# yanqinJiang/Animate3D

Hardware: AMD Instinct MI355X
Metric: UNet denoise-steps/sec, 4view×16frame×512² MV-VDM @1/2/4/8 GPU (higher is better)
Workload: dtype bf16; 1 GPU; BASELINE config 2: 4 views x 16 frames x 512^2 px (64x64 latent), CFG-doubled batch V=8 videos, one MVUNetMotionModel.forward per step, SD1.5 MV-VDM UNet 1.53 B params, seeded synthetic weights; parallelism=single GPU

## Files before the change

### animate3d_amd/csrc/gemm_common.h

```cpp
#pragma once
#include "common.h"

struct GemmParams {
  const uint16_t* X; int64_t ldx;
  const uint16_t* W; int64_t ldw;
  const float* bias;
  const uint16_t* rowbias; int64_t rb_div;
  const uint16_t* R; int64_t ldr;
  uint16_t* Y; int64_t ldy;
  int64_t M, N, K;
  float alpha, beta;
  int vec16;
  int out_f32;
  int B, H, Wd, Cin, Ho, Wo, stride, up, He, We;
  int64_t tiles_n, tiles_m;
  int ksplit, nk_item;
  float* ws; int64_t ws_bytes;
  const uint16_t* X2; int64_t ldx2; int64_t K1;
};

constexpr int EPI_LINEAR = 0, EPI_GEGLU = 1;

static inline int a3d_gemm_kernel_of(int flags) { return flags & A3D_GEMM_KERNEL_MASK; }
static inline int a3d_gemm_reserved_cus_of(int flags) { return flags & A3D_GEMM_RESERVED_CUS_MASK; }

A3D_DEV float epi_scale(float v, float alpha) { return __fmul_rn(v, alpha); }
A3D_DEV float epi_axpy(float v, float beta, float r) { return __fmaf_rn(beta, r, v); }

A3D_DEV float gelu_erf(float gte) {
  const float x = fabsf(gte) * 0.70710678118654752f;
  const float t = __builtin_amdgcn_rcpf(fmaf(0.3275911f, x, 1.0f));
  float poly = fmaf(1.061405429f, t, -1.453152027f);
  poly = fmaf(poly, t, 1.421413741f);
  poly = fmaf(poly, t, -0.284496736f);
  poly = fmaf(poly, t, 0.254829592f);
  poly *= t;
  const float e = __builtin_amdgcn_exp2f(-x * x * 1.4426950408889634f);
  const float erfx = fmaf(-poly, e, 1.0f);
  const float hg = __fmul_rn(0.5f, gte);
  return __fmaf_rn(fabsf(hg), erfx, hg);
}

A3D_DEV f32x2_t splat2(float v) { return f32x2_t{v, v}; }
A3D_DEV f32x2_t gelu_erf2(f32x2_t g) {
  const f32x2_t x = __builtin_elementwise_abs(g) * 0.70710678118654752f;
  const f32x2_t den = __builtin_elementwise_fma(splat2(0.3275911f), x, splat2(1.0f));
  const f32x2_t t = {__builtin_amdgcn_rcpf(den[0]), __builtin_amdgcn_rcpf(den[1])};
  f32x2_t poly = __builtin_elementwise_fma(splat2(1.061405429f), t, splat2(-1.453152027f));
  poly = __builtin_elementwise_fma(poly, t, splat2(1.421413741f));
  poly = __builtin_elementwise_fma(poly, t, splat2(-0.284496736f));
  poly = __builtin_elementwise_fma(poly, t, splat2(0.254829592f));
  poly = poly * t;
  const f32x2_t a = (-x) * x * 1.4426950408889634f;
  const f32x2_t e = {__builtin_amdgcn_exp2f(a[0]), __builtin_amdgcn_exp2f(a[1])};
  const f32x2_t erfx = __builtin_elementwise_fma(-poly, e, splat2(1.0f));
  const f32x2_t hg = g * 0.5f;
  return __builtin_elementwise_fma(__builtin_elementwise_abs(hg), erfx, hg);
}
A3D_DEV void geglu8(const float (&hv)[8], const float (&gv)[8], const float (&bh)[8], const float (&bg)[8], float (&y)[8]) {
#pragma unroll
  for (int e = 0; e < 4; ++e) {
    const f32x2_t gg = f32x2_t{gv[2 * e], gv[2 * e + 1]} + f32x2_t{bg[2 * e], bg[2 * e + 1]};
    const f32x2_t hh = f32x2_t{hv[2 * e], hv[2 * e + 1]} + f32x2_t{bh[2 * e], bh[2 * e + 1]};
    const f32x2_t yy = hh * gelu_erf2(gg);
    y[2 * e] = yy[0]; y[2 * e + 1] = yy[1];
  }
}

static __device__ u32x4_t g_zero_page[4];

A3D_DEV uint32_t lds_addr(const void* p) {
  return (uint32_t)(uintptr_t)(__attribute__((address_space(3))) const void*)p;
}
A3D_DEV void glds16_v(const void* gsrc, uint32_t lds_dst) {
  unsigned keep;
  asm volatile("s_mov_b32 %0, m0\n\ts_mov_b32 m0, %2\n\ts_nop 0\n\tglobal_load_lds_dwordx4 %1, off\n\ts_mov_b32 m0, %0"
               : "=&s"(keep) : "v"(gsrc), "s"(__builtin_amdgcn_readfirstlane(lds_dst)) : "memory");
}
A3D_DEV void glds16_s(uint32_t voff, const void* sbase, uint32_t lds_dst) {
  unsigned keep;
  asm volatile("s_mov_b32 %0, m0\n\ts_mov_b32 m0, %3\n\ts_nop 0\n\tglobal_load_lds_dwordx4 %1, %2\n\ts_mov_b32 m0, %0"
               : "=&s"(keep) : "v"(voff), "s"(sbase), "s"(__builtin_amdgcn_readfirstlane(lds_dst)) : "memory");
}
A3D_DEV const uint16_t* scalar_ptr(const uint16_t* ptr) {
  const uint64_t a = (uint64_t)(uintptr_t)ptr;
  return (const uint16_t*)(uintptr_t)(((uint64_t)(uint32_t)__builtin_amdgcn_readfirstlane((int)(a >> 32)) << 32) |
                                      (uint32_t)__builtin_amdgcn_readfirstlane((int)(uint32_t)a));
}
A3D_DEV u32x4_t lds_vload128(const void* p) {
  return *(const volatile __attribute__((address_space(3))) u32x4_t*)(uintptr_t)lds_addr(p);
}
A3D_DEV u32x2_t lds_vload64(const void* p) {
  return *(const volatile __attribute__((address_space(3))) u32x2_t*)(uintptr_t)lds_addr(p);
}
A3D_DEV void wave_lds_fence() {
  __builtin_amdgcn_fence(__ATOMIC_RELEASE, "wavefront");
  __builtin_amdgcn_wave_barrier();
  __builtin_amdgcn_fence(__ATOMIC_ACQUIRE, "wavefront");
}

A3D_DEV void tile_barrier() {
  asm volatile("s_barrier" ::: "memory");
  __builtin_amdgcn_sched_barrier(0);
}

template <int NB> struct WaveCols {
  static constexpr int PASSES = (NB + 1) / 2;
  int first, last;
  __device__ __forceinline__ explicit WaveCols(int wn) : first(NB == 5 ? wn * 4 : wn * NB), last(NB == 5 ? 8 + wn : wn * NB + NB - 1) {}
  __device__ __forceinline__ int block(int tn) const { return tn < NB - 1 ? first + tn : last; }
  A3D_DEV int pass_width(int ps) { return 2 * ps + 1 < NB ? 64 : 32; }
  __device__ __forceinline__ int pass_col0(int ps) const { return block(2 * ps) * 32; }
};

constexpr int BIAS_IMG_STRIDE = 2048;
constexpr int BIAS_IMG_ROWBIAS = 1280;
constexpr int BIAS_IMG_DMA = 1024;
A3D_DEV const float* bias_image(const char* img, int par) { return reinterpret_cast<const float*>(img + par * BIAS_IMG_STRIDE); }
A3D_DEV const uint16_t* rowbias_image(const char* img, int par) {
  return reinterpret_cast<const uint16_t*>(img + par * BIAS_IMG_STRIDE + BIAS_IMG_ROWBIAS);
}
template <int THREADS> A3D_DEV void zero_absent_bias_images(char* img, const float* bias, const uint16_t* rowbias, int tid) {
  if (!bias || !rowbias) {
    uint32_t* const bz = reinterpret_cast<uint32_t*>(img);
    for (int i = tid; i < 2 * BIAS_IMG_STRIDE / 4; i += THREADS) {
      const int o = (i * 4) % BIAS_IMG_STRIDE;
      if ((o < BIAS_IMG_ROWBIAS && !bias) || (o >= BIAS_IMG_ROWBIAS && !rowbias)) bz[i] = 0u;
    }
    asm volatile("s_waitcnt lgkmcnt(0)" ::: "memory");
    tile_barrier();
  }
}

template <int NB> A3D_DEV void read_frags(const char* stage, uint32_t xrd, uint32_t wrd, uint32_t wrd_last, uint32_t ko, u32x4_t (&fx)[2],
                                          u32x4_t (&fw)[NB]) {
  const char* xs = stage + xrd;
  const char* ws = stage + wrd;
  const char* wl = stage + wrd_last;
#pragma unroll
  for (int tm = 0; tm < 2; ++tm) fx[tm] = *reinterpret_cast<const u32x4_t*>(xs + tm * 4096 + ko);
#pragma unroll
  for (int tn = 0; tn < NB - 1; ++tn) fw[tn] = *reinterpret_cast<const u32x4_t*>(ws + tn * 4096 + ko);
  fw[NB - 1] = *reinterpret_cast<const u32x4_t*>(wl + ko);
}

template <int EPI, int NB>
A3D_DEV void epilogue_rounded(const GemmParams& p, f32x16_t (&acc)[NB][2], float* const stg, const float* const bias_lds,
                              const uint16_t* const rowbias_lds, const int64_t m0, const int64_t n0, const int wm, const WaveCols<NB> wc,
                              const int lane) {
  const int wblk = wc.first, wblk_last = wc.last;
  auto pass_cols = [&](int ps) { return (2 * ps + 1 < NB) ? 64 : 32; };
  auto pass_col0 = [&](int ps) { return ((2 * ps + 1 < NB) ? wblk + 2 * ps : wblk_last) * 32; };
  const int l31 = lane & 31, g = lane >> 5;
  constexpr int NP = (NB + 1) / 2;
  constexpr int RS = (EPI == EPI_GEGLU) ? 64 : 128;
  char* const stg16 = reinterpret_cast<char*>(stg);
  const int wsw = (EPI == EPI_GEGLU) ? ((l31 >> 1) & 3) : (l31 & 7);
  const int whalf = 8 * (g ^ ((l31 >> 3) & 1));
  auto unswap = [](u32x4_t o, int row) {
    const bool sw = row & 8;
    u32x4_t r;
    r[0] = sw ? o[2] : o[0]; r[1] = sw ? o[3] : o[1]; r[2] = sw ? o[0] : o[2]; r[3] = sw ? o[1] : o[3];
    return r;
  };
  constexpr int BUF2 = 32 * RS;
#pragma unroll
  for (int pi = 0; pi < 2 * NP; ++pi) {
    const int tm = pi / NP, ps = pi % NP;
    const int ncol = pass_cols(ps);
    const int64_t mbase = m0 + wm * 64 + tm * 32;
    const int64_t nbase = n0 + pass_col0(ps);
    char* const sb = stg16 + (pi & 1) * BUF2;
    if constexpr (EPI == EPI_GEGLU) {
      u32x4_t bq[2][4];
      auto fetch = [&](int q2, int slot) __attribute__((always_inline)) {
#pragma unroll
        for (int h = 0; h < 2; ++h) {
          const int c0 = 8 * (2 * q2 + h) + 4 * g;
          bq[slot][2 * h] = lds_vload128(bias_lds + pass_col0(ps) + c0);
          bq[slot][2 * h + 1] = lds_vload128(bias_lds + pass_col0(ps) + 32 + c0);
        }
      };
      fetch(0, 0);
#pragma unroll
      for (int q2 = 0; q2 < 2; ++q2) {
        if (q2 + 1 < 2) fetch(q2 + 1, (q2 + 1) & 1);
        __builtin_amdgcn_sched_barrier(0);
        float hv[8], gv[8], bh[8], bg[8], y[8];
#pragma unroll
        for (int h = 0; h < 2; ++h) {
          const u32x4_t b0 = bq[q2 & 1][2 * h], b1 = bq[q2 & 1][2 * h + 1];
#pragma unroll
          for (int j = 0; j < 4; ++j) { bh[4 * h + j] = __uint_as_float(b0[j]); bg[4 * h + j] = __uint_as_float(b1[j]); }
#pragma unroll
          for (int j = 0; j < 4; ++j) { hv[4 * h + j] = acc[2 * ps][tm][4 * (2 * q2 + h) + j]; gv[4 * h + j] = acc[2 * ps + 1][tm][4 * (2 * q2 + h) + j]; }
        }
        geglu8(hv, gv, bh, bg, y);
#pragma unroll
        for (int h = 0; h < 2; ++h) {
          u32x2_t o;
          o[0] = pack16(y[4 * h], y[4 * h + 1]);
          o[1] = pack16(y[4 * h + 2], y[4 * h + 3]);
          *reinterpret_cast<u32x2_t*>(sb + l31 * RS + 16 * ((2 * q2 + h) ^ wsw) + whalf) = o;
        }
      }
      wave_lds_fence();
      const int cc = lane & 3;
      const int64_t oc = nbase / 2 + 8 * cc;
      u32x4_t ob[2];
#pragma unroll
      for (int j = 0; j < 2; ++j) {
        const int row = 16 * j + (lane >> 2);
        ob[j] = *reinterpret_cast<const u32x4_t*>(sb + row * RS + 16 * (cc ^ ((row >> 1) & 3)));
      }
#pragma unroll
      for (int j = 0; j < 2; ++j) {
        const int row = 16 * j + (lane >> 2);
        const int64_t m = mbase + row;
        const u32x4_t o = unswap(ob[j], row);
        *reinterpret_cast<u32x4_t*>(p.Y + m * p.ldy + oc) = o;
      }
    } else {
      constexpr int NQ = 8;
      const int nq = (2 * ps + 1 < NB) ? 8 : 4;
      u32x4_t bq[3];
      u32x2_t tq[3];
      auto fetch = [&](int idx, int slot) __attribute__((always_inline)) {
        const int c0 = (idx >> 2) * 32 + 8 * (idx & 3) + 4 * g;
        bq[slot] = lds_vload128(bias_lds + pass_col0(ps) + c0);
        tq[slot] = lds_vload64(rowbias_lds + pass_col0(ps) + c0);
      };
      auto quads = [&](auto with_c) __attribute__((always_inline)) {
        constexpr bool WITH = decltype(with_c)::value;
        if constexpr (WITH) { fetch(0, 0); fetch(1, 1); }
#pragma unroll
        for (int idx = 0; idx < NQ; ++idx) {
          if (idx >= nq) continue;
          const int tl = idx >> 2, q = idx & 3;
          const int tn = 2 * ps + tl;
          if constexpr (WITH) {
            if (idx + 2 < nq) fetch(idx + 2, (idx + 2) % 3);
            __builtin_amdgcn_sched_barrier(0);
          }
          float v[4] = {acc[tn][tm][4 * q], acc[tn][tm][4 * q + 1], acc[tn][tm][4 * q + 2], acc[tn][tm][4 * q + 3]};
          if constexpr (WITH) {
            const u32x4_t b = bq[idx % 3];
            v[0] += __uint_as_float(b[0]); v[1] += __uint_as_float(b[1]); v[2] += __uint_as_float(b[2]); v[3] += __uint_as_float(b[3]);
            const u32x2_t tb = tq[idx % 3];
            v[0] += lo16(tb[0]); v[1] += hi16(tb[0]); v[2] += lo16(tb[1]); v[3] += hi16(tb[1]);
          }
#pragma unroll
          for (int e = 0; e < 4; ++e) v[e] = epi_scale(v[e], p.alpha);
          u32x2_t o;
          o[0] = pack16(v[0], v[1]);
          o[1] = pack16(v[2], v[3]);
          *reinterpret_cast<u32x2_t*>(sb + l31 * RS + 16 * ((4 * tl + q) ^ wsw) + whalf) = o;
          if constexpr (WITH) __builtin_amdgcn_sched_barrier(0);
        }
      };
      if (p.bias || p.rowbias) quads(std::true_type{});
      else quads(std::false_type{});
      wave_lds_fence();
      const int lpr = ncol / 8;
      const int cc = lane & (lpr - 1);
      u32x4_t ob[4];
#pragma unroll
      for (int j = 0; j < 4; ++j) {
        if (j * (64 / lpr) >= 32) continue;
        const int row = (64 / lpr) * j + lane / lpr;
        ob[j] = *reinterpret_cast<const u32x4_t*>(sb + row * RS + 16 * (cc ^ (row & 7)));
      }
#pragma unroll
      for (int j = 0; j < 4; ++j) {
        if (j * (64 / lpr) >= 32) continue;
        const int row = (64 / lpr) * j + lane / lpr;
        const int64_t m = mbase + row;
        const u32x4_t o = unswap(ob[j], row);
        *reinterpret_cast<u32x4_t*>(p.Y + m * p.ldy + nbase + 8 * cc) = o;
      }
    }
  }
}

template <int NB>
A3D_DEV void epilogue_residual(const GemmParams& p, f32x16_t (&acc)[NB][2], float* const stg, const float* const bias_lds,
                               const uint16_t* const rowbias_lds, const int64_t m0, const int64_t n0, const int wm, const WaveCols<NB> wc,
                               const int lane) {
  const int l31 = lane & 31, g = lane >> 5;
  constexpr int SROW = 68;
  constexpr int NP = WaveCols<NB>::PASSES;
  u32x4_t rres[2][4];
  auto load_res = [&](int pi, int slot) {
    const int tm = pi / NP, ps = pi % NP;
    const int64_t mbase = m0 + wm * 64 + tm * 32;
    const int64_t nbase = n0 + wc.pass_col0(ps);
    if (WaveCols<NB>::pass_width(ps) == 64) {
#pragma unroll
      for (int j = 0; j < 4; ++j) {
        const int64_t m = mbase + 8 * j + (lane >> 3);
        rres[slot][j] = *reinterpret_cast<const u32x4_t*>(p.R + m * p.ldr + nbase + 8 * (lane & 7));
      }
    } else {
#pragma unroll
      for (int j = 0; j < 2; ++j) {
        const int64_t m = mbase + 16 * j + (lane >> 2);
        rres[slot][j] = *reinterpret_cast<const u32x4_t*>(p.R + m * p.ldr + nbase + 8 * (lane & 3));
      }
    }
  };
  load_res(0, 0);
#pragma unroll
  for (int pi = 0; pi < 2 * NP; ++pi) {
    const int tm = pi / NP, ps = pi % NP;
    const int ncol = WaveCols<NB>::pass_width(ps);
    if (pi + 1 < 2 * NP) load_res(pi + 1, (pi + 1) & 1);
#pragma unroll
    for (int tl = 0; tl < 2; ++tl) {
      const int tn = 2 * ps + tl;
      if (tn < NB) {
#pragma unroll
        for (int q = 0; q < 4; ++q) {
          float4 v;
          v.x = acc[tn][tm][4 * q]; v.y = acc[tn][tm][4 * q + 1]; v.z = acc[tn][tm][4 * q + 2]; v.w = acc[tn][tm][4 * q + 3];
          *reinterpret_cast<float4*>(stg + l31 * SROW + tl * 32 + 8 * q + 4 * g) = v;
        }
      }
    }
    wave_lds_fence();
    const int64_t mbase = m0 + wm * 64 + tm * 32;
    const int64_t nbase = n0 + wc.pass_col0(ps);

    const int lpr = ncol / 8;
    const int cc = lane & (lpr - 1);
    const int64_t n = nbase + 8 * cc;
    const int ncl = wc.pass_col0(ps) + 8 * cc;
    float bv[8];
#pragma unroll
    for (int e = 0; e < 8; ++e) bv[e] = bias_lds[ncl + e];
    const u32x4_t tb = *reinterpret_cast<const u32x4_t*>(rowbias_lds + ncl);
#pragma unroll
    for (int j = 0; j < 4; ++j) {
      if (j * (64 / lpr) >= 32) continue;
      const int row = (64 / lpr) * j + lane / lpr;
      const int64_t m = mbase + row;
      const float4 a0 = *reinterpret_cast<const float4*>(stg + row * SROW + 8 * cc);
      const float4 a1 = *reinterpret_cast<const float4*>(stg + row * SROW + 8 * cc + 4);
      float v[8] = {a0.x, a0.y, a0.z, a0.w, a1.x, a1.y, a1.z, a1.w};
#pragma unroll
      for (int e = 0; e < 8; ++e) v[e] += bv[e];
#pragma unroll
      for (int e = 0; e < 4; ++e) { v[2 * e] += lo16(tb[e]); v[2 * e + 1] += hi16(tb[e]); }
#pragma unroll
      for (int e = 0; e < 8; ++e) v[e] = epi_scale(v[e], p.alpha);
      const u32x4_t tr = rres[pi & 1][j];
#pragma unroll
      for (int e = 0; e < 4; ++e) { v[2 * e] = epi_axpy(v[2 * e], p.beta, lo16(tr[e])); v[2 * e + 1] = epi_axpy(v[2 * e + 1], p.beta, hi16(tr[e])); }
      u32x4_t o;
#pragma unroll
      for (int e = 0; e < 4; ++e) o[e] = pack16(v[2 * e], v[2 * e + 1]);
      *reinterpret_cast<u32x4_t*>(p.Y + m * p.ldy + n) = o;
    }
    wave_lds_fence();
  }
}


__attribute__((visibility("hidden"))) int A3D_FN(a3d_launch_gemm_pp)(int conv, int epi, int nb, hipStream_t stream, const GemmParams& p, int cus);
__attribute__((visibility("hidden"))) int A3D_FN(a3d_launch_gemm_ring)(int nb, hipStream_t stream, const GemmParams& p, int cus);
```

### animate3d_amd/csrc/gemm_conv.hip

```cpp
#include "gemm_common.h"

namespace {

constexpr int BM = 128, BN = 128;
template <int BKT> struct TileCfg {
  static constexpr int LROW = BKT + 8;
  static constexpr int TILE_ELEMS = 128 * LROW;
  static constexpr int STAGE_BYTES = 2 * 2 * TILE_ELEMS * 2;
  static constexpr int EPI_BYTES = 4 * 32 * 68 * 4;
  static constexpr int SMEM_BYTES = STAGE_BYTES > EPI_BYTES ? STAGE_BYTES : EPI_BYTES;
  static constexpr int CPR = BKT / 8;
  static constexpr int RPT = 256 / CPR;
  static constexpr int NPASS = 128 / RPT;
};



template <int CONV, int EPI, int BKT, bool RES>
__global__ __launch_bounds__(256, (BKT == 64 ? 2 : 3)) void gemm_kernel(const GemmParams p) {
  using TC = TileCfg<BKT>;
  constexpr int LROW = TC::LROW, TILE_ELEMS = TC::TILE_ELEMS, NPASS = TC::NPASS, RPT = TC::RPT, BK = BKT;
  extern __shared__ __attribute__((aligned(16))) uint16_t smem[];
  const int tid = threadIdx.x;
  const int lane = tid & 63, wid = tid >> 6;
  const int wm = wid >> 1, wn = wid & 1;
  const int l31 = lane & 31, g = lane >> 5;

  const int64_t nblk = p.tiles_n * p.tiles_m;
  const int64_t lid = xcd_remap(blockIdx.x, nblk);
  const int64_t tile_n = lid % p.tiles_n, tile_m = lid / p.tiles_n;
  const int64_t m0 = tile_m * BM, n0 = tile_n * BN;

  const int kc = tid % TC::CPR;
  const int srow = tid / TC::CPR;

  const uint16_t* a_ptr[NPASS];
  int a_b[CONV == 2 ? NPASS : 1], a_y[CONV == 2 ? NPASS : 1], a_x[CONV == 2 ? NPASS : 1];
  bool a_ok[NPASS];
  int a_mask[NPASS];
#pragma unroll
  for (int i = 0; i < NPASS; ++i) {
    int64_t m = m0 + srow + RPT * i;
    a_ok[i] = m < p.M;
    if (m >= p.M) m = p.M - 1;
    if constexpr (CONV != 0) {
      const int hw = p.Ho * p.Wo;
      const int b = (int)(m / hw);
      const int rem = (int)(m - (int64_t)b * hw);
      const int oy = rem / p.Wo, ox = rem - oy * p.Wo;
      if constexpr (CONV == 2) {
        a_b[i] = b; a_y[i] = oy; a_x[i] = ox;
        a_ptr[i] = nullptr; a_mask[i] = 0;
      } else {
        const int y0 = oy * p.stride - 1, x0 = ox * p.stride - 1;
        a_ptr[i] = p.X + (((int64_t)b * p.H + y0) * p.Wd + x0) * p.Cin + kc * 8;
        int mask = 0;
#pragma unroll
        for (int t = 0; t < 9; ++t) {
          const int yy = y0 + t / 3, xx = x0 + t % 3;
          if (a_ok[i] && yy >= 0 && yy < p.H && xx >= 0 && xx < p.Wd) mask |= 1 << t;
        }
        a_mask[i] = mask;
      }
    } else {
      a_ptr[i] = p.X + m * p.ldx + kc * 8;
      a_mask[i] = 0;
    }
  }
  const uint16_t* w_ptr[NPASS];
#pragma unroll
  for (int i = 0; i < NPASS; ++i) {
    int64_t n = n0 + srow + RPT * i;
    if (n >= p.N) n = p.N - 1;
    w_ptr[i] = p.W + n * p.ldw + kc * 8;
  }

  struct RegTile { u32x4_t a[NPASS], w[NPASS]; };
  RegTile rt0, rt1;
  auto load_tile = [&](int64_t k0, RegTile& rt) {
    u32x4_t (&ra)[NPASS] = rt.a; u32x4_t (&rw)[NPASS] = rt.w;
    if constexpr (CONV != 0) {
      {
        const int kt64 = (int)(k0 >> 6);
        const int c64 = kt64 / 9, t = kt64 - 9 * c64;
        k0 = (int64_t)t * p.Cin + c64 * 64 + (k0 & 63);
      }
      const int tap = (int)(k0 / p.Cin);
      const int ci0 = (int)(k0 - (int64_t)tap * p.Cin);
      const int ky = tap / 3, kx = tap - ky * 3;
      if constexpr (CONV == 1) {
        const int64_t toff = ((int64_t)ky * p.Wd + kx) * p.Cin + ci0;
#pragma unroll
        for (int i = 0; i < NPASS; ++i) {
          if ((a_mask[i] >> tap) & 1) ra[i] = *reinterpret_cast<const u32x4_t*>(a_ptr[i] + toff);
          else ra[i] = u32x4_t{0u, 0u, 0u, 0u};
        }
      } else {
        const int He = p.He, We = p.We;
#pragma unroll
        for (int i = 0; i < NPASS; ++i) {
          const int yy = a_y[i] + ky - 1, xx = a_x[i] + kx - 1;
          const bool ok = a_ok[i] && yy >= 0 && yy < He && xx >= 0 && xx < We;
          if (ok) {
            const uint16_t* src = p.X + (((int64_t)a_b[i] * p.H + (yy >> 1)) * p.Wd + (xx >> 1)) * p.Cin + ci0 + kc * 8;
            ra[i] = *reinterpret_cast<const u32x4_t*>(src);
          } else {
            ra[i] = u32x4_t{0u, 0u, 0u, 0u};
          }
        }
      }
    } else {
#pragma unroll
      for (int i = 0; i < NPASS; ++i) ra[i] = *reinterpret_cast<const u32x4_t*>(a_ptr[i] + k0);
    }
#pragma unroll
    for (int i = 0; i < NPASS; ++i) rw[i] = *reinterpret_cast<const u32x4_t*>(w_ptr[i] + k0);
  };
  auto store_tile = [&](int buf, const RegTile& rt) {
    const u32x4_t (&ra)[NPASS] = rt.a; const u32x4_t (&rw)[NPASS] = rt.w;
    uint16_t* As = smem + (buf * 2 + 0) * TILE_ELEMS;
    uint16_t* Ws = smem + (buf * 2 + 1) * TILE_ELEMS;
#pragma unroll
    for (int i = 0; i < NPASS; ++i) {
      *reinterpret_cast<u32x4_t*>(As + (srow + RPT * i) * LROW + kc * 8) = ra[i];
      *reinterpret_cast<u32x4_t*>(Ws + (srow + RPT * i) * LROW + kc * 8) = rw[i];
    }
  };

  f32x16_t acc[2][2];
#pragma unroll
  for (int a = 0; a < 2; ++a)
#pragma unroll
    for (int b = 0; b < 2; ++b)
#pragma unroll
      for (int r = 0; r < 16; ++r) acc[a][b][r] = 0.f;

  u32x4_t rres[RES ? 4 : 1];
  const int ecc = lane & 7;
  const int64_t en = n0 + wn * 64 + 8 * ecc;
  const bool epf = RES && (EPI == EPI_LINEAR) && p.R != nullptr && p.vec16 && en + 8 <= p.N;
  auto prefetch_residual = [&](int tm) {
    if constexpr (RES) {
#pragma unroll
      for (int j = 0; j < 4; ++j) {
        int64_t m = m0 + wm * 64 + tm * 32 + 8 * j + (lane >> 3);
        if (m >= p.M) m = p.M - 1;
        rres[j] = *reinterpret_cast<const u32x4_t*>(p.R + m * p.ldr + en);
      }
    }
  };

  const int64_t nk = p.K / BK;
  auto compute = [&](int cur) {
    const uint16_t* As = smem + (cur * 2 + 0) * TILE_ELEMS;
    const uint16_t* Ws = smem + (cur * 2 + 1) * TILE_ELEMS;
    u32x4_t fw[2][2], fa[2][2];
    auto load_frags = [&](int slot, int ks) {
#pragma unroll
      for (int t = 0; t < 2; ++t) {
        fw[slot][t] = *reinterpret_cast<const u32x4_t*>(Ws + (wn * 64 + t * 32 + l31) * LROW + ks * 16 + g * 8);
        fa[slot][t] = *reinterpret_cast<const u32x4_t*>(As + (wm * 64 + t * 32 + l31) * LROW + ks * 16 + g * 8);
      }
    };
    load_frags(0, 0);
#pragma unroll
    for (int ks = 0; ks < BK / 16; ++ks) {
      if (ks + 1 < BK / 16) load_frags((ks + 1) & 1, ks + 1);
#pragma unroll
      for (int tn = 0; tn < 2; ++tn)
#pragma unroll
        for (int tm = 0; tm < 2; ++tm) acc[tn][tm] = mfma32(fw[ks & 1][tn], fa[ks & 1][tm], acc[tn][tm]);
    }
  };

  load_tile(0, rt0);
  store_tile(0, rt0);
  if (nk > 1) load_tile(1 * BK, rt0);
  if (nk > 2) load_tile(2 * BK, rt1);
  __syncthreads();
  for (int64_t kt = 0;;) {
    if (kt + 1 >= nk && epf) prefetch_residual(0);
    compute(0);
    if (kt + 1 < nk) store_tile(1, rt0);
    if (kt + 3 < nk) load_tile((kt + 3) * BK, rt0);
    __syncthreads();
    if (++kt >= nk) break;
    if (kt + 1 >= nk && epf) prefetch_residual(0);
    compute(1);
    if (kt + 1 < nk) store_tile(0, rt1);
    if (kt + 3 < nk) load_tile((kt + 3) * BK, rt1);
    __syncthreads();
    if (++kt >= nk) break;
  }

  constexpr int SROW = 68;
  float* const stg = reinterpret_cast<float*>(smem) + wid * (32 * SROW);
#pragma unroll
  for (int tm = 0; tm < 2; ++tm) {
  if (tm == 1) __syncthreads();
#pragma unroll
  for (int tn = 0; tn < 2; ++tn)
#pragma unroll
    for (int q = 0; q < 4; ++q) {
      float4 v;
      v.x = acc[tn][tm][4 * q]; v.y = acc[tn][tm][4 * q + 1]; v.z = acc[tn][tm][4 * q + 2]; v.w = acc[tn][tm][4 * q + 3];
      *reinterpret_cast<float4*>(stg + l31 * SROW + tn * 32 + 8 * q + 4 * g) = v;
    }
  __syncthreads();
  const int64_t mbase = m0 + wm * 64 + tm * 32;

  if constexpr (EPI == EPI_GEGLU) {
    const int cc = lane & 3;
    const int64_t nh = n0 + wn * 64 + 8 * cc;
    const int64_t oc = (n0 + wn * 64) / 2 + 8 * cc;
    if (nh + 32 < p.N + 0 && oc + 8 <= p.N / 2) {
      float bh[8], bg[8];
#pragma unroll
      for (int e = 0; e < 8; ++e) { bh[e] = p.bias ? p.bias[nh + e] : 0.f; bg[e] = p.bias ? p.bias[nh + 32 + e] : 0.f; }
#pragma unroll
      for (int j = 0; j < 2; ++j) {
        const int row = 16 * j + (lane >> 2);
        const int64_t m = mbase + row;
        if (m >= p.M) continue;
        const float4 h0 = *reinterpret_cast<const float4*>(stg + row * SROW + 8 * cc);
        const float4 h1 = *reinterpret_cast<const float4*>(stg + row * SROW + 8 * cc + 4);
        const float4 g0 = *reinterpret_cast<const float4*>(stg + row * SROW + 32 + 8 * cc);
        const float4 g1 = *reinterpret_cast<const float4*>(stg + row * SROW + 32 + 8 * cc + 4);
        const float hv[8] = {h0.x, h0.y, h0.z, h0.w, h1.x, h1.y, h1.z, h1.w};
        const float gv[8] = {g0.x, g0.y, g0.z, g0.w, g1.x, g1.y, g1.z, g1.w};
        float y[8];
        geglu8(hv, gv, bh, bg, y);
        u32x4_t o;
#pragma unroll
        for (int e = 0; e < 4; ++e) o[e] = pack16(y[2 * e], y[2 * e + 1]);
        *reinterpret_cast<u32x4_t*>(p.Y + m * p.ldy + oc) = o;
      }
    }
  } else {
    const int cc = lane & 7;
    const int64_t n = n0 + wn * 64 + 8 * cc;
    if (n < p.N) {
      const bool full = (n + 8 <= p.N) && p.vec16;
      float bv[8];
#pragma unroll
      for (int e = 0; e < 8; ++e) bv[e] = (p.bias && n + e < p.N) ? p.bias[n + e] : 0.f;
#pragma unroll
      for (int j = 0; j < 4; ++j) {
        const int row = 8 * j + (lane >> 3);
        const int64_t m = mbase + row;
        if (m >= p.M) continue;
        const float4 a0 = *reinterpret_cast<const float4*>(stg + row * SROW + 8 * cc);
        const float4 a1 = *reinterpret_cast<const float4*>(stg + row * SROW + 8 * cc + 4);
        float v[8] = {a0.x, a0.y, a0.z, a0.w, a1.x, a1.y, a1.z, a1.w};
#pragma unroll
        for (int e = 0; e < 8; ++e) v[e] += bv[e];
        const uint16_t* rb = p.rowbias ? p.rowbias + (m / p.rb_div) * p.N + n : nullptr;
        const uint16_t* rr = p.R ? p.R + m * p.ldr + n : nullptr;
        uint16_t* yy = p.Y + m * p.ldy + n;
        if (full) {
          if (rb) {
            const u32x4_t t = *reinterpret_cast<const u32x4_t*>(rb);
#pragma unroll
            for (int e = 0; e < 4; ++e) { v[2 * e] += lo16(t[e]); v[2 * e + 1] += hi16(t[e]); }
          }
#pragma unroll
          for (int e = 0; e < 8; ++e) v[e] = epi_scale(v[e], p.alpha);
          if constexpr (RES) {
            if (rr) {
              const u32x4_t t = rres[j];
#pragma unroll
              for (int e = 0; e < 4; ++e) { v[2 * e] = epi_axpy(v[2 * e], p.beta, lo16(t[e])); v[2 * e + 1] = epi_axpy(v[2 * e + 1], p.beta, hi16(t[e])); }
            }
          }
          if (p.out_f32) {
            float* yf = reinterpret_cast<float*>(p.Y) + m * p.ldy + n;
            *reinterpret_cast<float4*>(yf) = float4{v[0], v[1], v[2], v[3]};
            *reinterpret_cast<float4*>(yf + 4) = float4{v[4], v[5], v[6], v[7]};
          } else {
            u32x4_t o;
#pragma unroll
            for (int e = 0; e < 4; ++e) o[e] = pack16(v[2 * e], v[2 * e + 1]);
            *reinterpret_cast<u32x4_t*>(yy) = o;
          }
        } else {
#pragma unroll
          for (int hh = 0; hh < 2; ++hh) {
            if (n + 4 * hh + 4 > p.N) continue;
            float w[4] = {v[4 * hh], v[4 * hh + 1], v[4 * hh + 2], v[4 * hh + 3]};
            if (rb) {
              const u32x2_t t = *reinterpret_cast<const u32x2_t*>(rb + 4 * hh);
              w[0] += lo16(t[0]); w[1] += hi16(t[0]); w[2] += lo16(t[1]); w[3] += hi16(t[1]);
            }
#pragma unroll
            for (int e = 0; e < 4; ++e) w[e] = epi_scale(w[e], p.alpha);
            if (rr) {
              const u32x2_t t = *reinterpret_cast<const u32x2_t*>(rr + 4 * hh);
              w[0] = epi_axpy(w[0], p.beta, lo16(t[0])); w[1] = epi_axpy(w[1], p.beta, hi16(t[0]));
              w[2] = epi_axpy(w[2], p.beta, lo16(t[1])); w[3] = epi_axpy(w[3], p.beta, hi16(t[1]));
            }
            u32x2_t o;
            o[0] = pack16(w[0], w[1]);
            o[1] = pack16(w[2], w[3]);
            *reinterpret_cast<u32x2_t*>(yy + 4 * hh) = o;
          }
        }
      }
    }
  }
  if (tm == 0 && epf) prefetch_residual(1);
  }
}


constexpr int PBM = 256;
constexpr int NOT_ELIGIBLE = -1000;

inline bool gemm_flags_ok(int flags) {
  return !(flags & ~(A3D_GEMM_RESERVED_CUS_MASK | A3D_GEMM_KERNEL_MASK)) && a3d_gemm_kernel_of(flags) <= A3D_GEMM_RING;
}

inline int device_cus() {
  static int cus_of[64] = {0};
  const int dev = a3d_current_device();
  if (cus_of[dev] == 0) {
    int n = 0;
    if (hipDeviceGetAttribute(&n, hipDeviceAttributeMultiprocessorCount, dev) != hipSuccess) return 0;
    cus_of[dev] = n > 0 ? n : 256;
  }
  return cus_of[dev];
}

constexpr int PERSIST_MIN_FILL = 50;
struct PPPlan { int nb, S, cus; int64_t tiles_m, tiles_n; };
constexpr int SPLITK_MAX = 16;
constexpr int SPLITK_MINK = 9;
template <int CONV, int EPI>
bool plan_persist(const GemmParams& p, int flags, bool allow_split, PPPlan& out) {
  if (a3d_gemm_kernel_of(flags) == A3D_GEMM_TILE128 || p.out_f32) return false;
  const int cus_dev = device_cus();
  if (cus_dev == 0) return false;
  const int reserved = a3d_gemm_reserved_cus_of(flags);
  const int cus = cus_dev - reserved > 32 ? cus_dev - reserved : 32;
  if (!p.vec16 || p.K % 64 != 0 || p.M % PBM != 0 || (p.rowbias && p.rb_div % PBM != 0)) return false;
  if (p.ldw % 64 != 0 || (CONV == 0 && p.ldx % 64 != 0)) return false;
  if (CONV == 0 && (uint64_t)p.ldx * 16u >= (1ull << 31)) return false;
  if ((uint64_t)p.ldw * 16u >= (1ull << 31)) return false;
  if (CONV != 0 && ((uint64_t)p.B * p.H * p.Wd + 2u * p.Wd + 2u) * (uint64_t)p.Cin * 2u >= (1ull << 32)) return false;
  const int64_t tm = (p.M + PBM - 1) / PBM;
  const int nk = (int)(p.K / 64);
  const int unit = CONV ? 9 : 1;
  const int cus_plan = cus_dev;
  constexpr int OVH = 12;
  int64_t best = -1, best1 = -1;
  int bnb = 0, bS = 1, bnb1 = 0;
  for (int nb = 5; nb >= 4; --nb) {
    if (EPI == EPI_GEGLU && nb == 5) continue;
    if (p.N % (nb * 64) != 0) continue;
    const int64_t tiles = tm * (p.N / (nb * 64));
    for (int S = 1; S <= (allow_split && EPI == EPI_LINEAR ? SPLITK_MAX : 1); ++S) {
      if ((nk / unit) % S != 0 || (S > 1 && nk / S < SPLITK_MINK)) continue;
      const int64_t items = tiles * S;
      const int64_t rounds = (items + cus_plan - 1) / cus_plan;
      if (items * 100 < rounds * cus_plan * PERSIST_MIN_FILL) continue;
      if (S > 1 && p.ws != nullptr && items * nb * 65536 > p.ws_bytes) continue;
      const int64_t cost = rounds * (nk / S + OVH) * nb * (nb == 4 ? 108 : 100) + (S > 1 ? 100 * nb : 0);
      if (S == 1 && (best1 < 0 || cost < best1)) { best1 = cost; bnb1 = nb; }
      if (best < 0 || cost < best) { best = cost; bnb = nb; bS = S; }
    }
  }
  if (best < 0) return false;
  if (bS > 1 && best1 >= 0 && best * 100 > best1 * 85) { bnb = bnb1; bS = 1; }
  out.nb = bnb; out.S = bS; out.cus = cus;
  out.tiles_m = tm; out.tiles_n = p.N / (bnb * 64);
  return true;
}

struct RingPlan { int nb, cus, cus_plan; int64_t cost; };
constexpr int RING_VS_PP_PCT = 75;
inline bool plan_ring(const GemmParams& p, int flags, RingPlan& out) {
  if (a3d_gemm_kernel_of(flags) == A3D_GEMM_TILE128 || p.out_f32 || !p.vec16 || p.X2 != nullptr) return false;
  if (p.M % 128 != 0 || p.K % 64 != 0 || p.K < 256 || p.ldx % 64 != 0 || p.ldw % 64 != 0) return false;
  if ((uint64_t)p.ldx * 64u >= (1ull << 32) || (uint64_t)p.ldw * 256u >= (1ull << 32)) return false;
  if (p.rowbias && p.rb_div % 128 != 0) return false;
  const int n = device_cus() ? device_cus() : 256;
  const int reserved = a3d_gemm_reserved_cus_of(flags);
  out.cus_plan = n;
  out.cus = n - reserved > 32 ? n - reserved : 32;
  out.nb = 0; out.cost = 0;
  for (int nb : {5, 4, 2}) {
    if (p.N % (64 * nb) != 0) continue;
    const int64_t tiles = (p.M / 128) * (p.N / (64 * nb));
    const int64_t rounds = (tiles + out.cus - 1) / out.cus;
    const int64_t cost = rounds * (128 + 64 * nb);
    if (out.nb == 0 || cost < out.cost) { out.nb = nb; out.cost = cost; }
  }
  return out.nb != 0;
}

template <int CONV, int EPI>
int try_launch_persist(hipStream_t stream, GemmParams& p, int flags) {
  PPPlan pl;
  if (!plan_persist<CONV, EPI>(p, flags, p.ws != nullptr, pl)) return NOT_ELIGIBLE;
  p.tiles_m = pl.tiles_m; p.tiles_n = pl.tiles_n;
  p.ksplit = pl.S; p.nk_item = (int)(p.K / 64) / pl.S;
  return A3D_FN(a3d_launch_gemm_pp)(CONV, EPI, pl.nb, stream, p, pl.cus);
}


template <int CONV, int EPI, int BKT, bool RES>
int launch_res(hipStream_t stream, GemmParams& p, int64_t nblk) {
  using TC = TileCfg<BKT>;
  static uint64_t attr_done = 0;
  if (int rc = a3d_once_per_device(attr_done, [] {
        return (int)hipFuncSetAttribute(reinterpret_cast<const void*>(&gemm_kernel<CONV, EPI, BKT, RES>),
                                        hipFuncAttributeMaxDynamicSharedMemorySize, TC::SMEM_BYTES); })) return rc;
  gemm_kernel<CONV, EPI, BKT, RES><<<dim3((unsigned)nblk), dim3(256), TC::SMEM_BYTES, stream>>>(p);
  return a3d_launch_status();
}

template <int CONV, int EPI, int BKT>
int launch_bk(hipStream_t stream, GemmParams& p, int64_t nblk) {
  if constexpr (EPI == EPI_LINEAR) {
    if (p.R != nullptr) return launch_res<CONV, EPI, BKT, true>(stream, p, nblk);
  }
  return launch_res<CONV, EPI, BKT, false>(stream, p, nblk);
}

template <int CONV, int EPI = EPI_LINEAR>
int launch(hipStream_t stream, GemmParams& p, int flags) {
  if (!gemm_flags_ok(flags)) return A3D_EINVAL;
  if constexpr (CONV == 0 && EPI == EPI_LINEAR) {
    RingPlan rp;
    if (plan_ring(p, flags, rp)) {
      PPPlan pl;
      bool ring = true;
      if (a3d_gemm_kernel_of(flags) != A3D_GEMM_RING && plan_persist<CONV, EPI>(p, flags, p.ws != nullptr, pl)) {
        const int64_t tiles = pl.tiles_m * pl.tiles_n * pl.S;
        const int64_t pp_cost = ((tiles + rp.cus_plan - 1) / rp.cus_plan) * (256 + 64 * pl.nb) * RING_VS_PP_PCT;
        ring = pl.S == 1 && rp.cost * 100 < pp_cost;
      }
      if (ring) {
        p.tiles_m = p.M / 128; p.tiles_n = p.N / (64 * rp.nb);
        return A3D_FN(a3d_launch_gemm_ring)(rp.nb, stream, p, rp.cus);
      }
    }
  }
  {
    const int rc = try_launch_persist<CONV, EPI>(stream, p, flags);
    if (rc != NOT_ELIGIBLE) return rc;
  }
  p.tiles_m = (p.M + BM - 1) / BM;
  p.tiles_n = (p.N + BN - 1) / BN;
  const int64_t nblk = p.tiles_m * p.tiles_n;
  if (nblk <= 0 || nblk > 0x7fffffffLL) return A3D_EINVAL;
  const bool small = (CONV == 0 && p.K <= 640) || nblk < 768;
  if (small) return launch_bk<CONV, EPI, 32>(stream, p, nblk);
  return launch_bk<CONV, EPI, 64>(stream, p, nblk);
}

template <int CONV>
int64_t splitk_ws_bytes(const GemmParams& p, int flags) {
  PPPlan pl;
  GemmParams q = p;
  q.ws = nullptr; q.ws_bytes = 0;
  if (!gemm_flags_ok(flags)) return 0;
  if (!plan_persist<CONV, EPI_LINEAR>(q, flags, true, pl) || pl.S <= 1) return 0;
  return pl.tiles_m * pl.tiles_n * pl.S * pl.nb * 65536;
}

void attach_workspace(GemmParams& p, void* ws, int64_t ws_bytes) {
  if (ws && ws_bytes > 0 && a3d_aligned(16, ws)) { p.ws = (float*)ws; p.ws_bytes = ws_bytes; }
}

GemmParams dense_params(const void* X, int64_t ldx, const void* W, int64_t ldw, const float* bias, const void* rowbias, int64_t rb_div,
                        const void* R, int64_t ldr, void* Y, int64_t ldy, int64_t M, int64_t N, int64_t K, float alpha, float beta,
                        bool out_f32 = false) {
  GemmParams p{};
  p.X = (const uint16_t*)X; p.ldx = ldx; p.W = (const uint16_t*)W; p.ldw = ldw;
  p.bias = bias; p.rowbias = (const uint16_t*)rowbias; p.rb_div = rowbias ? rb_div : 1;
  p.R = (const uint16_t*)R; p.ldr = ldr; p.Y = (uint16_t*)Y; p.ldy = ldy;
  p.M = M; p.N = N; p.K = K; p.alpha = alpha; p.beta = beta; p.out_f32 = out_f32;
  p.vec16 = (ldy * (out_f32 ? 4 : 2) % 16 == 0) && a3d_aligned(16, Y) && (!R || (ldr % 8 == 0 && a3d_aligned(16, R))) &&
            (!rowbias || (N % 8 == 0 && a3d_aligned(16, rowbias)));
  return p;
}

bool dense_args_ok(const GemmParams& p, uintptr_t y_align, int n_div, int ldy_div) {
  if (!p.X || !p.W || !p.Y || p.M <= 0 || p.N <= 0 || p.K <= 0) return false;
  if (p.K % 64 != 0 || p.N % n_div != 0) return false;
  if (p.ldx % 8 != 0 || p.ldw % 8 != 0 || p.ldy % ldy_div != 0 || (p.R && p.ldr % 4 != 0)) return false;
  if (!a3d_aligned(16, p.X, p.W) || !a3d_aligned(16, p.bias) || !a3d_aligned(y_align, p.Y) || !a3d_aligned(8, p.R, p.rowbias)) return false;
  return !p.rowbias || p.rb_div > 0;
}

int gemm_entry(a3d_stream_t stream, const void* X, int64_t ldx, const void* W, int64_t ldw,
               const float* bias, const void* rowbias, int64_t rb_div, const void* R, int64_t ldr,
               void* Y, int64_t ldy, int64_t M, int64_t N, int64_t K, float alpha, float beta, int flags,
               void* ws, int64_t ws_bytes, int64_t* ws_needed) {
  GemmParams p = dense_params(X, ldx, W, ldw, bias, rowbias, rb_div, R, ldr, Y, ldy, M, N, K, alpha, beta);
  if (!dense_args_ok(p, 8, 4, 4)) return A3D_EINVAL;
  if (ws_needed) { *ws_needed = splitk_ws_bytes<0>(p, flags); return 0; }
  attach_workspace(p, ws, ws_bytes);
  return launch<0>((hipStream_t)stream, p, flags);
}

}

extern "C" int A3D_FN(a3d_gemm)(a3d_stream_t stream, const void* X, int64_t ldx, const void* W, int64_t ldw,
                             const float* bias, const void* rowbias, int64_t rb_div, const void* R, int64_t ldr,
                             void* Y, int64_t ldy, int64_t M, int64_t N, int64_t K, float alpha, float beta, int flags) {
  return gemm_entry(stream, X, ldx, W, ldw, bias, rowbias, rb_div, R, ldr, Y, ldy, M, N, K, alpha, beta, flags, nullptr, 0, nullptr);
}

extern "C" int A3D_FN(a3d_gemm_ws)(a3d_stream_t stream, const void* X, int64_t ldx, const void* W, int64_t ldw,
                                const float* bias, const void* rowbias, int64_t rb_div, const void* R, int64_t ldr,
                                void* Y, int64_t ldy, int64_t M, int64_t N, int64_t K, float alpha, float beta, int flags,
                                void* ws, int64_t ws_bytes, int64_t* ws_needed) {
  return gemm_entry(stream, X, ldx, W, ldw, bias, rowbias, rb_div, R, ldr, Y, ldy, M, N, K, alpha, beta, flags, ws, ws_bytes, ws_needed);
}

extern "C" int A3D_FN(a3d_gemm2)(a3d_stream_t stream, const void* X, int64_t ldx, const void* X2, int64_t ldx2, int64_t K1,
                              const void* W, int64_t ldw, const float* bias, void* Y, int64_t ldy, int64_t M, int64_t N, int64_t K, int flags) {
  GemmParams p = dense_params(X, ldx, W, ldw, bias, nullptr, 1, nullptr, 0, Y, ldy, M, N, K, 1.f, 0.f);
  p.X2 = (const uint16_t*)X2; p.ldx2 = ldx2; p.K1 = K1;
  if (!dense_args_ok(p, 16, 8, 8) || !X2 || K1 <= 0 || K1 >= K || K1 % 64 != 0 || ldx2 % 8 != 0 || !a3d_aligned(16, X2)) return A3D_EINVAL;
  if (!gemm_flags_ok(flags)) return A3D_EINVAL;
  if (ldx2 % 64 != 0 || (uint64_t)ldx2 * 16u >= (1ull << 31)) return A3D_EUNSUPPORTED;
  const int rc = try_launch_persist<0, EPI_LINEAR>((hipStream_t)stream, p, flags);
  return rc == NOT_ELIGIBLE ? A3D_EUNSUPPORTED : rc;
}

extern "C" int A3D_FN(a3d_gemm_f32out)(a3d_stream_t stream, const void* X, int64_t ldx, const void* W, int64_t ldw,
                                    const float* bias, float* Y, int64_t ldy, int64_t M, int64_t N, int64_t K, float alpha) {
  GemmParams p = dense_params(X, ldx, W, ldw, bias, nullptr, 1, nullptr, 0, Y, ldy, M, N, K, alpha, 0.f, true);
  if (!dense_args_ok(p, 16, 8, 4)) return A3D_EINVAL;
  return launch<0>((hipStream_t)stream, p, 0);
}

static int conv_entry(a3d_stream_t stream, const void* X, const void* Wp, const float* bias,
                      const void* rowbias, int64_t rb_div, const void* R, void* Y,
                      int B, int H, int W, int Cin, int Cout, int stride, int up2x, int flags,
                      void* ws, int64_t ws_bytes, int64_t* ws_needed) {
  if (!X || !Wp || !Y || B <= 0 || H <= 0 || W <= 0) return A3D_EINVAL;
  if (Cin % 64 != 0 || Cout % 4 != 0 || (stride != 1 && stride != 2)) return A3D_EINVAL;
  if (up2x < 0 || up2x > 7 || (up2x > 1 && !(up2x & 1)) || (up2x && stride != 1)) return A3D_EINVAL;
  if (!a3d_aligned(16, X, Wp) || !a3d_aligned(16, bias) || !a3d_aligned(8, Y)) return A3D_EINVAL;
  if (rowbias && rb_div <= 0) return A3D_EINVAL;
  const int He = up2x ? 2 * H - ((up2x >> 1) & 1) : H, We = up2x ? 2 * W - ((up2x >> 2) & 1) : W;
  if (He <= 0 || We <= 0) return A3D_EINVAL;
  GemmParams p{};
  p.X = (const uint16_t*)X; p.ldx = Cin; p.W = (const uint16_t*)Wp; p.ldw = (int64_t)9 * Cin;
  p.bias = bias; p.rowbias = (const uint16_t*)rowbias; p.rb_div = rowbias ? rb_div : 1;
  p.R = (const uint16_t*)R; p.ldr = Cout; p.Y = (uint16_t*)Y; p.ldy = Cout;
  p.B = B; p.H = H; p.Wd = W; p.Cin = Cin; p.stride = stride; p.up = up2x ? 1 : 0; p.He = He; p.We = We;
  p.Ho = (He + 2 - 3) / stride + 1; p.Wo = (We + 2 - 3) / stride + 1;
  p.M = (int64_t)B * p.Ho * p.Wo; p.N = Cout; p.K = (int64_t)9 * Cin;
  p.alpha = 1.f; p.beta = 1.f;
  p.vec16 = (Cout % 8 == 0) && a3d_aligned(16, Y, R, rowbias);
  if (ws_needed) { *ws_needed = up2x ? splitk_ws_bytes<2>(p, flags) : splitk_ws_bytes<1>(p, flags); return 0; }
  attach_workspace(p, ws, ws_bytes);
  return up2x ? launch<2>((hipStream_t)stream, p, flags) : launch<1>((hipStream_t)stream, p, flags);
}

extern "C" int A3D_FN(a3d_conv3x3)(a3d_stream_t stream, const void* X, const void* Wp, const float* bias,
                                const void* rowbias, int64_t rb_div, const void* R, void* Y,
                                int B, int H, int W, int Cin, int Cout, int stride, int up2x, int flags) {
  return conv_entry(stream, X, Wp, bias, rowbias, rb_div, R, Y, B, H, W, Cin, Cout, stride, up2x, flags, nullptr, 0, nullptr);
}

extern "C" int A3D_FN(a3d_conv3x3_ws)(a3d_stream_t stream, const void* X, const void* Wp, const float* bias,
                                   const void* rowbias, int64_t rb_div, const void* R, void* Y,
                                   int B, int H, int W, int Cin, int Cout, int stride, int up2x, int flags,
                                   void* ws, int64_t ws_bytes, int64_t* ws_needed) {
  return conv_entry(stream, X, Wp, bias, rowbias, rb_div, R, Y, B, H, W, Cin, Cout, stride, up2x, flags, ws, ws_bytes, ws_needed);
}

extern "C" int A3D_FN(a3d_gemm_geglu)(a3d_stream_t stream, const void* X, int64_t ldx, const void* W, int64_t ldw,
                                   const float* bias, void* Y, int64_t ldy, int64_t M, int64_t N2, int64_t K, int flags) {
  GemmParams p = dense_params(X, ldx, W, ldw, bias, nullptr, 1, nullptr, 0, Y, ldy, M, N2, K, 1.f, 0.f);
  if (!dense_args_ok(p, 16, 64, 8)) return A3D_EINVAL;
  return launch<0, EPI_GEGLU>((hipStream_t)stream, p, flags);
}
```

### animate3d_amd/csrc/gemm_pp.hip

```cpp
#include "gemm_common.h"

namespace {

constexpr int PBM = 256;
template <int NB> struct PPCfg {
  static constexpr int BN = NB * 64;
  static constexpr int XBYTES = PBM * 128;
  static constexpr int WBYTES = BN * 128;
  static constexpr int EPI_BYTES = 8 * 32 * 68 * 4;
  static constexpr int STAGE = (XBYTES + WBYTES) > EPI_BYTES ? (XBYTES + WBYTES) : EPI_BYTES;
  static constexpr int BIAS_OFF = 2 * STAGE;
  static constexpr int SMEM = BIAS_OFF + 2 * BIAS_IMG_STRIDE;
};

constexpr int PP_GM = 8;
A3D_DEV void pp_tile_coords(int64_t t, int64_t tiles_m, int64_t tiles_n, int64_t& tile_m, int64_t& tile_n) {
  const int64_t gsz = PP_GM * tiles_n;
  const int64_t blk = t / gsz;
  const int64_t first = blk * PP_GM;
  const int64_t gm = tiles_m - first < PP_GM ? tiles_m - first : PP_GM;
  const int64_t within = t - blk * gsz;
  tile_n = within / gm;
  tile_m = first + (within - tile_n * gm);
}

template <int CONV, int EPI, int NB, bool RES, bool SPLIT = false, bool TWO = false>
__global__ __launch_bounds__(512, 1) void gemm_pp_kernel(const GemmParams p) {
  static_assert(!TWO || CONV == 0, "the two-source A operand is a dense-GEMM feature");
  using PC = PPCfg<NB>;
  constexpr int PH = 1, NPH = 4;
  constexpr int NP = 4 + NB;
  extern __shared__ __attribute__((aligned(16))) uint16_t smem[];
  char* const smem_b = reinterpret_cast<char*>(smem);
  const int tid = threadIdx.x, lane = tid & 63;
  const int wid = __builtin_amdgcn_readfirstlane(tid >> 6);
  const int wm = wid >> 1, wn = wid & 1;
  const int grp = wid >> 2;
  const int l31 = lane & 31, g = lane >> 5;
  const int lr = lane >> 3, pos = lane & 7;
  const uint32_t lds0 = lds_addr(smem);

  const int S = SPLIT ? p.ksplit : 1;
  const int64_t ntiles = p.tiles_m * p.tiles_n * S;
  const int64_t G = gridDim.x;
  int64_t t = xcd_remap(blockIdx.x, G);
  if (t >= ntiles) return;
  const int nk = SPLIT ? p.nk_item : (int)(p.K / 64);

  const uint32_t koff0 = (uint32_t)((g ^ ((l31 >> 1) & 7)) << 4);
  const uint32_t xrd = (uint32_t)(wm * 64 + l31) * 128u;
  const WaveCols<NB> wc(wn);
  const uint32_t wrd = (uint32_t)PC::XBYTES + (uint32_t)(wc.first * 32 + l31) * 128u;
  const uint32_t wrd_last = (uint32_t)PC::XBYTES + (uint32_t)(wc.last * 32 + l31) * 128u;

  const uint32_t vx0 = (uint32_t)(lr * p.ldx * 2 + ((pos ^ (lr >> 1)) << 4));
  const uint32_t vw0 = (uint32_t)(lr * p.ldw * 2 + ((pos ^ (lr >> 1)) << 4));
  uint32_t aoff[CONV ? 4 : 1];
  uint32_t amask[CONV ? 2 : 1];
  uint32_t sok[CONV ? 2 : 1];
  const int64_t cbias = CONV ? ((int64_t)p.Wd + 1) * p.Cin : 0;
  int64_t ld_m0 = 0, ld_n0 = 0;
  int ld_par = 0;
  int ik0 = 0, itap = 0, ikx = 0, iky = 0;
  uint64_t xck = 0;
  uint64_t zpage = 0;
  if constexpr (CONV != 0) {
    zpage = (uint64_t)(uintptr_t)g_zero_page;
    asm volatile("" : "+s"(zpage));
  }
  uint64_t xk = 0, wk = 0, rbk = 0;
  const uint32_t sx8 = (uint32_t)(p.ldx * 16), sw8 = (uint32_t)(p.ldw * 16);
  uint64_t xk2 = 0;
  const uint32_t vx0b = TWO ? (uint32_t)(lr * p.ldx2 * 2 + ((pos ^ (lr >> 1)) << 4)) : 0u;
  const uint32_t sx8b = TWO ? (uint32_t)(p.ldx2 * 16) : 0u;
  auto setup_tile = [&](int64_t tt) {
    int64_t tile_n, tile_m;
    const int64_t tile_id = SPLIT ? (int64_t)((uint32_t)tt / (uint32_t)S) : tt;
    const int64_t kofs = SPLIT ? (CONV ? ((int64_t)(tt - tile_id * S) * nk / 9) * 64 : (int64_t)(tt - tile_id * S) * nk * 64) : 0;
    pp_tile_coords(tile_id, p.tiles_m, p.tiles_n, tile_m, tile_n);
    ld_m0 = tile_m * PBM; ld_n0 = tile_n * PC::BN;
    ik0 = 0; itap = 0; ikx = 0; iky = 0;
    ld_par ^= 1;
    if constexpr (CONV != 0) xck = (uint64_t)(uintptr_t)p.X - (uint64_t)cbias * 2u + (uint64_t)kofs * 2u;
    if constexpr (CONV == 0) xk = (uint64_t)(uintptr_t)(p.X + (ld_m0 + wid * 32) * p.ldx + kofs);
    if constexpr (TWO) xk2 = (uint64_t)(uintptr_t)(p.X2 + (ld_m0 + wid * 32) * p.ldx2);
    wk = (uint64_t)(uintptr_t)(p.W + (ld_n0 + wid * (NB * 8)) * p.ldw + kofs);
    if (EPI == EPI_LINEAR && p.rowbias) rbk = (uint64_t)(uintptr_t)(p.rowbias + (ld_m0 / p.rb_div) * p.N + ld_n0);
    if constexpr (CONV != 0) {
      amask[0] = 0; amask[1] = 0;
#pragma unroll
      for (int i = 0; i < 4; ++i) {
        const int r = (wid * 4 + i) * 8 + lr;
        const int slot = pos ^ ((r >> 1) & 7);
        const uint32_t m = (uint32_t)ld_m0 + (uint32_t)r;
        const uint32_t hw = (uint32_t)(p.Ho * p.Wo);
        const int b = (int)(m / hw);
        const int rem = (int)(m - (uint32_t)b * hw);
        const int oy = (int)((uint32_t)rem / (uint32_t)p.Wo), ox = rem - oy * p.Wo;
        uint32_t mask = 0;
        if constexpr (CONV == 2) {
          const int sy0 = (oy - 1) >> 1, sx0 = (ox - 1) >> 1;
          aoff[i] = (uint32_t)(((((int64_t)b * p.H + sy0) * p.Wd + sx0) * p.Cin + cbias) * 2 + slot * 16);
#pragma unroll
          for (int tp = 0; tp < 9; ++tp) {
            const int yy = oy + tp / 3 - 1, xx = ox + tp % 3 - 1;
            if (yy >= 0 && yy < p.He && xx >= 0 && xx < p.We) mask |= 1u << tp;
          }
          amask[i >> 1] |= (mask << (9 * (i & 1))) | ((uint32_t)(~oy & 1) << (18 + 2 * (i & 1))) | ((uint32_t)(~ox & 1) << (19 + 2 * (i & 1)));
        } else {
          const int y0 = oy * p.stride - 1, x0 = ox * p.stride - 1;
          aoff[i] = (uint32_t)(((((int64_t)b * p.H + y0) * p.Wd + x0) * p.Cin + cbias) * 2 + slot * 16);
#pragma unroll
          for (int tp = 0; tp < 9; ++tp) {
            const int yy = y0 + tp / 3, xx = x0 + tp % 3;
            if (yy >= 0 && yy < p.H && xx >= 0 && xx < p.Wd) mask |= 1u << tp;
          }
          amask[i >> 1] |= mask << (9 * (i & 1));
        }
      }
      sok[0] = 0; sok[1] = 0;
#pragma unroll
      for (int bit = 0; bit < 18; ++bit) {
        if (__builtin_amdgcn_ballot_w64(((amask[0] >> bit) & 1u) != 0u) == ~0ull) sok[0] |= 1u << bit;
        if (__builtin_amdgcn_ballot_w64(((amask[1] >> bit) & 1u) != 0u) == ~0ull) sok[1] |= 1u << bit;
      }
    }
  };
  auto issue_pieces = [&](int buf, auto a_c, auto b_c) __attribute__((always_inline)) {
    constexpr int A = decltype(a_c)::value, B = decltype(b_c)::value;
    if constexpr (A >= B) return;
    const uint32_t dst = lds0 + (uint32_t)buf * PC::STAGE;
    if constexpr (A == 0) {
      if (ik0 == 0) {
        const uint32_t bdst = lds0 + (uint32_t)PC::BIAS_OFF + (uint32_t)ld_par * BIAS_IMG_STRIDE;
        if (p.bias) {
          if (wid == 0) glds16_s((uint32_t)lane * 16u, p.bias + ld_n0, bdst);
          if (NB == 5 && wid == 1) { if (lane < 16) glds16_s((uint32_t)lane * 16u, p.bias + ld_n0 + BIAS_IMG_DMA / 4, bdst + (uint32_t)BIAS_IMG_DMA); }
        }
        if (EPI == EPI_LINEAR && p.rowbias && wid == 2) {
          if (lane < PC::BN / 8) glds16_s((uint32_t)lane * 16u, (const void*)(uintptr_t)rbk, bdst + (uint32_t)BIAS_IMG_ROWBIAS);
        }
      }
    }
    if constexpr (CONV != 0) {
      const int ky = iky, kx = ikx;
      const uint32_t rowb = (uint32_t)(p.Wd * p.Cin * 2), colb = (uint32_t)(p.Cin * 2);
      const uint32_t yE = (uint32_t)((ky + 1) >> 1) * rowb, yO = (uint32_t)(ky >> 1) * rowb;
      const uint32_t xE = (uint32_t)((kx + 1) >> 1) * colb, xO = (uint32_t)(kx >> 1) * colb;
#pragma unroll
      for (int i = 0; i < 4; ++i) {
        if (i < A || i >= B) continue;
        const uint32_t d = dst + (uint32_t)(wid * 4 + i) * 1024u;
        const uint32_t mk = amask[i >> 1];
        uint32_t vo = aoff[i];
        if constexpr (CONV == 2) vo += (((mk >> (18 + 2 * (i & 1))) & 1u) ? yE : yO) + (((mk >> (19 + 2 * (i & 1))) & 1u) ? xE : xO);
        const int bit = itap + 9 * (i & 1);
        if ((sok[i >> 1] >> bit) & 1u) {
          glds16_s(vo, (const void*)(uintptr_t)xck, d);
        } else {
          const uint64_t src = ((mk >> bit) & 1u) ? xck + vo : zpage;
          glds16_v((const void*)(uintptr_t)src, d);
        }
      }
    } else {
      const bool sec = TWO && ik0 >= (int)p.K1;
      const uint32_t vxs = sec ? vx0b : vx0, sxs = sec ? sx8b : sx8;
      const uint64_t xks = sec ? xk2 : xk;
#pragma unroll
      for (int i = 0; i < 4; ++i) {
        if (i < A || i >= B) continue;
        const int pc = wid * 4 + i;
        glds16_s(vxs ^ (uint32_t)((i & 1) << 6), (const void*)(uintptr_t)(xks + (uint64_t)(uint32_t)(i * sxs)), dst + (uint32_t)pc * 1024u);
      }
    }
#pragma unroll
    for (int i = 0; i < NB; ++i) {
      if (4 + i < A || 4 + i >= B) continue;
      const int pc = wid * NB + i;
      glds16_s(vw0 ^ (uint32_t)((pc & 1) << 6), (const void*)(uintptr_t)(wk + (uint64_t)(uint32_t)(i * sw8)), dst + (uint32_t)PC::XBYTES + (uint32_t)pc * 1024u);
    }
    if constexpr (B == NP) {
      if constexpr (CONV != 0) {
        const uint64_t cin2 = (uint64_t)(uint32_t)p.Cin * 2u;
        wk += cin2;
        ++itap;
        if (++ikx == 3) { ikx = 0; ++iky; }
        if (itap == 9) {
          itap = 0; iky = 0; wk -= 9u * cin2 - 128u;
          if constexpr (CONV == 1) xck -= (2u * (uint64_t)(uint32_t)p.Wd + 2u) * cin2;
          xck += 128u;
        } else if constexpr (CONV == 1) {
          xck += ikx == 0 ? ((uint64_t)(uint32_t)p.Wd - 2u) * cin2 : cin2;
        }
      } else {
        if (TWO && ik0 >= (int)p.K1) xk2 += 128; else xk += 128;
        wk += 128;
      }
      ik0 += 64;
    }
  };
  auto issue_phase = [&](int buf, auto ph_c, bool late) __attribute__((always_inline)) {
    constexpr int ph = decltype(ph_c)::value;
    using I0 = std::integral_constant<int, 0>;
    using I3 = std::integral_constant<int, 3>;
    using I5 = std::integral_constant<int, 5>;
    using I6 = std::integral_constant<int, 6>;
    using IN = std::integral_constant<int, NP>;
    if (!late) {
      if constexpr (ph == 0) issue_pieces(buf, I0{}, I3{});
      if constexpr (ph == 1) issue_pieces(buf, I3{}, I6{});
      if constexpr (ph == 2) issue_pieces(buf, I6{}, IN{});
    } else {
      if constexpr (ph == 1) issue_pieces(buf, I0{}, I5{});
      if constexpr (ph == 2) issue_pieces(buf, I5{}, IN{});
    }
  };

  f32x16_t acc[NB][2];
  u32x4_t fx[PH][2], fw[PH][NB];
  auto load_frags = [&](int buf, int ks0) __attribute__((always_inline)) {
#pragma unroll
    for (int s = 0; s < PH; ++s) read_frags<NB>(smem_b + buf * PC::STAGE, xrd, wrd, wrd_last, koff0 ^ (uint32_t)((ks0 + s) << 5), fx[s], fw[s]);
  };
  auto mfma_phase = [&]() __attribute__((always_inline)) {
#pragma unroll
    for (int s = 0; s < PH; ++s)
#pragma unroll
      for (int tn = 0; tn < NB; ++tn)
#pragma unroll
        for (int tm = 0; tm < 2; ++tm) acc[tn][tm] = mfma32(fw[s][tn], fx[s][tm], acc[tn][tm]);
  };

  zero_absent_bias_images<512>(smem_b + PC::BIAS_OFF, p.bias, EPI == EPI_LINEAR ? p.rowbias : nullptr, tid);
  setup_tile(t);
  issue_pieces(0, std::integral_constant<int, 0>{}, std::integral_constant<int, NP>{});
  asm volatile("s_waitcnt vmcnt(0)" ::: "memory");
  tile_barrier();
  int buf = 0;
  for (;;) {
    int64_t tile_n, tile_m;
    pp_tile_coords(SPLIT ? (int64_t)((uint32_t)t / (uint32_t)S) : t, p.tiles_m, p.tiles_n, tile_m, tile_n);
    const int64_t m0 = tile_m * PBM, n0 = tile_n * PC::BN;
    const int64_t tnext = t + G;
#pragma unroll
    for (int a = 0; a < NB; ++a)
#pragma unroll
      for (int b = 0; b < 2; ++b)
#pragma unroll
        for (int r = 0; r < 16; ++r) acc[a][b][r] = 0.f;
    const int cur_par = ld_par;
    if (grp) tile_barrier();
    for (int kt = 0; kt < nk; ++kt) {
      const bool last = kt + 1 >= nk;
      const bool more = !last || tnext < ntiles;
      const bool late = kt == 0;
      static_for<NPH>([&](auto ph_c) __attribute__((always_inline)) {
        constexpr int ph = decltype(ph_c)::value;
        load_frags(buf, ph * PH);
        if (more) {
          if constexpr (ph == 0 || ph == 1) {
            if (last && (late ? ph == 1 : ph == 0)) setup_tile(tnext);
          }
          issue_phase(buf ^ 1, ph_c, late);
          if constexpr (ph == NPH - 1) { if (grp) asm volatile("s_waitcnt vmcnt(0)" ::: "memory"); }
        }
        asm volatile("s_waitcnt lgkmcnt(0)" ::: "memory");
        tile_barrier();
        __builtin_amdgcn_s_setprio(1);
        mfma_phase();
        __builtin_amdgcn_s_setprio(0);
        __builtin_amdgcn_sched_barrier(0);
        if constexpr (ph == NPH - 1) { if (more && !grp) asm volatile("s_waitcnt vmcnt(0)" ::: "memory"); }
        tile_barrier();
      });
      buf ^= 1;
    }
    if (!grp) tile_barrier();

    if constexpr (SPLIT) {
      float* const wsi = p.ws + ((t * 8 + wid) * (NB * 8)) * 256 + lane * 4;
#pragma unroll
      for (int tn = 0; tn < NB; ++tn)
#pragma unroll
        for (int tm = 0; tm < 2; ++tm)
#pragma unroll
          for (int q = 0; q < 4; ++q)
            *reinterpret_cast<float4*>(wsi + ((tn * 2 + tm) * 4 + q) * 256) =
                float4{acc[tn][tm][4 * q], acc[tn][tm][4 * q + 1], acc[tn][tm][4 * q + 2], acc[tn][tm][4 * q + 3]};
    } else {
      float* const stg = reinterpret_cast<float*>(smem_b + (buf ^ 1) * PC::STAGE) + wid * (32 * 68);
      const float* const bias_lds = bias_image(smem_b + PC::BIAS_OFF, cur_par);
      const uint16_t* const rowbias_lds = rowbias_image(smem_b + PC::BIAS_OFF, cur_par);
      if constexpr (EPI == EPI_GEGLU || !RES) epilogue_rounded<EPI, NB>(p, acc, stg, bias_lds, rowbias_lds, m0, n0, wm, wc, lane);
      else epilogue_residual<NB>(p, acc, stg, bias_lds, rowbias_lds, m0, n0, wm, wc, lane);
    }
    if (tnext >= ntiles) break;
    t = tnext;
  }
}

template <int NB>
__global__ __launch_bounds__(512) void splitk_reduce_kernel(const GemmParams p) {
  using PC = PPCfg<NB>;
  const int tid = threadIdx.x, lane = tid & 63, wid = tid >> 6;
  const int wm = wid >> 1, wn = wid & 1, l31 = lane & 31, g = lane >> 5;
  const WaveCols<NB> wc(wn);
  const int S = p.ksplit;
  int64_t tile_n, tile_m;
  pp_tile_coords(blockIdx.x, p.tiles_m, p.tiles_n, tile_m, tile_n);
  const int64_t m0 = tile_m * PBM, n0 = tile_n * PC::BN;
  const float* const w0 = p.ws + (((int64_t)blockIdx.x * S * 8 + wid) * (NB * 8)) * 256 + lane * 4;
  const int64_t item_stride = (int64_t)8 * NB * 8 * 256;
  const int tn = blockIdx.y;
#pragma unroll
    for (int tm = 0; tm < 2; ++tm) {
      const int64_t m = m0 + wm * 64 + tm * 32 + l31;
      const int64_t nb0 = n0 + wc.block(tn) * 32 + 4 * g;
#pragma unroll
      for (int q = 0; q < 4; ++q) {
        const float* src = w0 + ((tn * 2 + tm) * 4 + q) * 256;
        float4 a = *reinterpret_cast<const float4*>(src);
        for (int s = 1; s < S; ++s) {
          const float4 b = *reinterpret_cast<const float4*>(src + s * item_stride);
          a.x += b.x; a.y += b.y; a.z += b.z; a.w += b.w;
        }
        const int64_t n = nb0 + 8 * q;
        float v[4] = {a.x, a.y, a.z, a.w};
        if (p.bias) {
          const float4 b = *reinterpret_cast<const float4*>(p.bias + n);
          v[0] += b.x; v[1] += b.y; v[2] += b.z; v[3] += b.w;
        }
        if (p.rowbias) {
          const u32x2_t tb = *reinterpret_cast<const u32x2_t*>(p.rowbias + (m / p.rb_div) * p.N + n);
          v[0] += lo16(tb[0]); v[1] += hi16(tb[0]); v[2] += lo16(tb[1]); v[3] += hi16(tb[1]);
        }
#pragma unroll
        for (int e = 0; e < 4; ++e) v[e] = epi_scale(v[e], p.alpha);
        if (p.R) {
          const u32x2_t tr = *reinterpret_cast<const u32x2_t*>(p.R + m * p.ldr + n);
          v[0] = epi_axpy(v[0], p.beta, lo16(tr[0])); v[1] = epi_axpy(v[1], p.beta, hi16(tr[0]));
          v[2] = epi_axpy(v[2], p.beta, lo16(tr[1])); v[3] = epi_axpy(v[3], p.beta, hi16(tr[1]));
        }
        u32x2_t o;
        o[0] = pack16(v[0], v[1]);
        o[1] = pack16(v[2], v[3]);
        *reinterpret_cast<u32x2_t*>(p.Y + m * p.ldy + n) = o;
      }
    }
}

template <int CONV, int EPI, int NB, bool RES, bool SPLIT = false, bool TWO = false>
int launch_pp(hipStream_t stream, const GemmParams& p, int cus) {
  using PC = PPCfg<NB>;
  static uint64_t attr_done = 0;
  if (int rc = a3d_once_per_device(attr_done, [] {
        return (int)hipFuncSetAttribute(reinterpret_cast<const void*>(&gemm_pp_kernel<CONV, EPI, NB, RES, SPLIT, TWO>),
                                        hipFuncAttributeMaxDynamicSharedMemorySize, PC::SMEM); })) return rc;
  const int64_t ntiles = p.tiles_m * p.tiles_n * (SPLIT ? p.ksplit : 1);
  const unsigned grid = (unsigned)(ntiles < cus ? ntiles : cus);
  gemm_pp_kernel<CONV, EPI, NB, RES, SPLIT, TWO><<<dim3(grid), dim3(512), PC::SMEM, stream>>>(p);
  if (int rc = a3d_launch_status()) return rc;
  if constexpr (SPLIT) {
    splitk_reduce_kernel<NB><<<dim3((unsigned)(p.tiles_m * p.tiles_n), NB), dim3(512), 0, stream>>>(p);
    return a3d_launch_status();
  }
  return 0;
}

template <int CONV>
int launch_pp_conv(int epi, int nb, hipStream_t stream, const GemmParams& p, int cus) {
  if (epi == EPI_GEGLU) {
    if constexpr (CONV == 0) { if (nb == 4) return launch_pp<0, EPI_GEGLU, 4, false>(stream, p, cus); }
    return A3D_EUNSUPPORTED;
  }
  if constexpr (CONV == 0) {
    if (p.X2 != nullptr) {
      if (p.R || p.ksplit > 1) return A3D_EUNSUPPORTED;
      if (nb == 5) return launch_pp<0, EPI_LINEAR, 5, false, false, true>(stream, p, cus);
      if (nb == 4) return launch_pp<0, EPI_LINEAR, 4, false, false, true>(stream, p, cus);
      return A3D_EUNSUPPORTED;
    }
  }
  if (p.ksplit > 1) {
    if (nb == 5) return launch_pp<CONV, EPI_LINEAR, 5, false, true>(stream, p, cus);
    if (nb == 4) return launch_pp<CONV, EPI_LINEAR, 4, false, true>(stream, p, cus);
    return A3D_EUNSUPPORTED;
  }
  if (nb == 5) return p.R ? launch_pp<CONV, EPI_LINEAR, 5, true>(stream, p, cus) : launch_pp<CONV, EPI_LINEAR, 5, false>(stream, p, cus);
  if (nb == 4) return p.R ? launch_pp<CONV, EPI_LINEAR, 4, true>(stream, p, cus) : launch_pp<CONV, EPI_LINEAR, 4, false>(stream, p, cus);
  return A3D_EUNSUPPORTED;
}

}

int A3D_FN(a3d_launch_gemm_pp)(int conv, int epi, int nb, hipStream_t stream, const GemmParams& p, int cus) {
  if (conv == 0) return launch_pp_conv<0>(epi, nb, stream, p, cus);
  if (conv == 1) return launch_pp_conv<1>(epi, nb, stream, p, cus);
  return launch_pp_conv<2>(epi, nb, stream, p, cus);
}
```

### animate3d_amd/hip_ops.py

```python
from __future__ import annotations

import ctypes
import os
from dataclasses import dataclass
from typing import Optional

import torch

_LIB_PATH = os.path.join(os.path.dirname(os.path.abspath(__file__)), "lib", "libanimate3d_hip.so")
_lib = None

c_i64, c_int, c_f32, c_f64, c_vp = ctypes.c_int64, ctypes.c_int, ctypes.c_float, ctypes.c_double, ctypes.c_void_p


class _RowMapC(ctypes.Structure):
    _fields_ = [("gdiv", c_i64), ("ga", c_i64), ("gb", c_i64), ("seg_len", c_i64), ("seg_stride", c_i64), ("ld", c_i64)]


@dataclass(frozen=True)
class RowMap:
    gdiv: int
    ga: int
    gb: int
    seg_len: int
    seg_stride: int

    def c(self, ld: int) -> _RowMapC:
        return _RowMapC(self.gdiv, self.ga, self.gb, self.seg_len, self.seg_stride, ld)


def rowmap_rows(m: RowMap, groups: int, step: int, length: int, device="cpu") -> torch.Tensor:
    g = torch.arange(0, groups, step, device=device).view(-1, 1)
    s = torch.arange(length, device=device).view(1, -1)
    return ((g // m.gdiv) * m.ga + (g % m.gdiv) * m.gb + (s // m.seg_len) * m.seg_stride + s % m.seg_len).reshape(-1)


def rowmap_covers(m: RowMap, groups: int, step: int, length: int, rows: int, device="cpu") -> bool:
    if (groups + step - 1) // step * length != rows:
        return False
    idx = rowmap_rows(m, groups, step, length, device)
    return bool(int(idx.min()) >= 0 and int(idx.max()) < rows and torch.unique(idx).numel() == rows)


_SIGNATURES = {
    "a3d_version": (ctypes.c_char_p, []),
    "a3d_gemm_bf16": (c_int, [c_vp, c_vp, c_i64, c_vp, c_i64, c_vp, c_vp, c_i64, c_vp, c_i64, c_vp, c_i64, c_i64, c_i64, c_i64, c_f32, c_f32, c_int]),
    "a3d_gemm_ws_bf16": (c_int, [c_vp, c_vp, c_i64, c_vp, c_i64, c_vp, c_vp, c_i64, c_vp, c_i64, c_vp, c_i64, c_i64, c_i64, c_i64, c_f32, c_f32, c_int,
                                 c_vp, c_i64, ctypes.POINTER(c_i64)]),
    "a3d_gemm2_bf16": (c_int, [c_vp, c_vp, c_i64, c_vp, c_i64, c_i64, c_vp, c_i64, c_vp, c_vp, c_i64, c_i64, c_i64, c_i64, c_int]),
    "a3d_gemm_geglu_bf16": (c_int, [c_vp, c_vp, c_i64, c_vp, c_i64, c_vp, c_vp, c_i64, c_i64, c_i64, c_i64, c_int]),
    "a3d_conv3x3_bf16": (c_int, [c_vp, c_vp, c_vp, c_vp, c_vp, c_i64, c_vp, c_vp, c_int, c_int, c_int, c_int, c_int, c_int, c_int, c_int]),
    "a3d_conv3x3_ws_bf16": (c_int, [c_vp, c_vp, c_vp, c_vp, c_vp, c_i64, c_vp, c_vp, c_int, c_int, c_int, c_int, c_int, c_int, c_int, c_int,
                                    c_vp, c_i64, ctypes.POINTER(c_i64)]),
    "a3d_flash_attn_bf16": (c_int, [c_vp, c_vp, c_vp, c_vp, c_vp, ctypes.POINTER(_RowMapC), ctypes.POINTER(_RowMapC), ctypes.POINTER(_RowMapC),
                                    c_int, c_int, c_int, c_i64, c_i64, c_f32, c_f32, c_int]),
    "a3d_flash_attn_counted_bf16": (c_int, [c_vp, c_vp, c_vp, c_vp, c_vp, ctypes.POINTER(_RowMapC), ctypes.POINTER(_RowMapC), ctypes.POINTER(_RowMapC),
                                            c_int, c_int, c_int, c_i64, c_i64, c_f32, c_f32, c_int, c_vp]),
    "a3d_flash_attn2_bf16": (c_int, [c_vp, c_vp, c_vp, c_vp, c_vp, c_vp, c_vp, ctypes.POINTER(_RowMapC), ctypes.POINTER(_RowMapC), ctypes.POINTER(_RowMapC),
                                     ctypes.POINTER(_RowMapC), c_int, c_int, c_int, c_i64, c_i64, c_i64, c_f32, c_f32, c_f32, c_int]),
    "a3d_temporal_attn_bf16": (c_int, [c_vp, c_vp, c_vp, c_vp, c_i64, c_vp, c_i64, c_int, c_int, c_i64, c_int, c_int, c_f32]),
    "a3d_temporal_attn_sharded_bf16": (c_int, [c_vp, c_vp, c_i64, c_vp, c_vp, c_i64, c_vp, c_i64, c_int, c_int, c_i64, c_int, c_int, c_f32,
                                               c_int, c_int, c_int, c_i64]),
    "a3d_group_norm_ws_floats": (c_i64, [c_int, c_i64, c_int]),
    "a3d_group_norm_plan": (c_int, [c_i64, c_int, c_int, ctypes.POINTER(c_int)]),
    "a3d_group_norm_bf16": (c_int, [c_vp, c_vp, c_vp, c_vp, c_vp, c_vp, c_int, c_i64, c_int, c_int, c_f32, c_int]),
    "a3d_group_norm2_bf16": (c_int, [c_vp, c_vp, c_int, c_vp, c_int, c_vp, c_vp, c_vp, c_vp, c_int, c_i64, c_int, c_f32, c_int]),
    "a3d_group_norm_sums_bf16": (c_int, [c_vp, c_vp, c_vp, c_vp, c_int, c_i64, c_int, c_int]),
    "a3d_group_norm_apply_bf16": (c_int, [c_vp, c_vp, c_vp, c_vp, c_vp, c_vp, c_int, c_i64, c_int, c_int, c_int]),
    "a3d_layer_norm_bf16": (c_int, [c_vp, c_vp, c_vp, c_vp, c_vp, c_vp, c_i64, c_int, c_f32, c_vp, c_i64, c_i64, c_vp, c_i64, c_i64]),
    "a3d_geglu_bf16": (c_int, [c_vp, c_vp, c_i64, c_vp, c_i64, c_i64, c_i64]),
    "a3d_silu_bf16": (c_int, [c_vp, c_vp, c_vp, c_i64]),
    "a3d_activation_bf16": (c_int, [c_vp, c_vp, c_vp, c_i64, c_int]),
    "a3d_concat_bf16": (c_int, [c_vp, c_vp, c_i64, c_vp, c_i64, c_vp, c_i64]),
    "a3d_timestep_embed_bf16": (c_int, [c_vp, c_vp, c_vp, c_int, c_int]),
    "a3d_im2col_in": (c_int, [c_vp, c_vp, c_int, c_vp, c_int, c_int, c_int, c_int, c_int]),
    "a3d_unpack_out": (c_int, [c_vp, c_vp, c_vp, c_int, c_int, c_int, c_int, c_int, c_int]),
    "a3d_gemm_f32out_bf16": (c_int, [c_vp, c_vp, c_i64, c_vp, c_i64, c_vp, c_vp, c_i64, c_i64, c_i64, c_i64, c_f32]),
    "a3d_softmax_rows_f32_bf16": (c_int, [c_vp, c_vp, c_i64, c_vp, c_i64, c_i64, c_i64]),
    "a3d_softmax_rows_bwd_bf16": (c_int, [c_vp, c_vp, c_i64, c_vp, c_i64, c_vp, c_i64, c_i64, c_i64, c_f32]),
    "a3d_im2col_in_bwd": (c_int, [c_vp, c_vp, c_vp, c_int, c_int, c_int, c_int, c_int, c_f32]),
    "a3d_channel_mix_f32": (c_int, [c_vp, c_vp, c_vp, c_vp, c_vp, c_int, c_int, c_int, c_i64, c_f32]),
    "a3d_cfg_ddim_step_f32": (c_int, [c_vp, c_vp, c_vp, c_vp, c_vp, c_i64, c_int, c_int, c_i64, c_f32, c_f32, c_f32]),
    "a3d_flash_attn_bwd_bf16": (c_int, [c_vp, c_vp, c_vp, c_vp, c_vp, c_vp, c_vp, c_vp, c_vp, c_vp,
                                        ctypes.POINTER(_RowMapC), ctypes.POINTER(_RowMapC), ctypes.POINTER(_RowMapC), ctypes.POINTER(_RowMapC),
                                        ctypes.POINTER(_RowMapC), c_int, c_int, c_int, c_i64, c_i64, c_int, c_f32, c_f32, c_int]),
    "a3d_flash_attn_lse_bf16": (c_int, [c_vp, c_vp, c_vp, c_vp, c_vp, ctypes.POINTER(_RowMapC), ctypes.POINTER(_RowMapC), ctypes.POINTER(_RowMapC),
                                        c_int, c_int, c_int, c_i64, c_i64, c_f32, c_f32, c_int, c_vp]),
    "a3d_attn_delta_bf16": (c_int, [c_vp, c_vp, c_vp, ctypes.POINTER(_RowMapC), ctypes.POINTER(_RowMapC), c_vp, c_int, c_int, c_int, c_i64]),
    "a3d_temporal_attn_bwd_bf16": (c_int, [c_vp, c_vp, c_vp, c_vp, c_i64, c_vp, c_i64, c_vp, c_vp, c_vp, c_i64, c_int, c_int, c_i64, c_int, c_int, c_f32]),
    "a3d_layer_norm_bwd_bf16": (c_int, [c_vp, c_vp, c_vp, c_vp, c_vp, c_vp, c_vp, c_i64, c_int, c_f32, c_int]),
    "a3d_group_norm_bwd_bf16": (c_int, [c_vp, c_vp, c_vp, c_vp, c_vp, c_vp, c_vp, c_vp, c_vp, c_vp, c_int, c_i64, c_int, c_int, c_int]),
    "a3d_geglu_bwd_bf16": (c_int, [c_vp, c_vp, c_i64, c_vp, c_i64, c_vp, c_i64, c_i64, c_i64]),
    "a3d_transpose_bf16": (c_int, [c_vp, c_vp, c_i64, c_vp, c_i64, c_i64, c_i64, c_i64]),
    "a3d_wgrad_ws_floats": (c_i64, [c_i64, c_i64, c_i64]),
    "a3d_wgrad_bf16": (c_int, [c_vp, c_vp, c_i64, c_vp, c_i64, c_vp, c_i64, c_vp, c_i64, c_i64, c_i64, c_f32, c_int]),
    "a3d_colsum_bf16": (c_int, [c_vp, c_vp, c_i64, c_i64, c_i64, c_vp, c_f32, c_int]),
    "a3d_axpby_bf16": (c_int, [c_vp, c_vp, c_vp, c_i64, c_f32, c_f32]),
    "a3d_zero_insert2x_bf16": (c_int, [c_vp, c_vp, c_vp, c_int, c_int, c_int, c_int]),
    "a3d_upsample2x_bwd_bf16": (c_int, [c_vp, c_vp, c_vp, c_int, c_int, c_int, c_int, c_int, c_int]),
    "a3d_sqnorm_f32": (c_int, [c_vp, c_vp, c_i64, c_vp, c_int]),
    "a3d_clip_ctrl_f32": (c_int, [c_vp, c_vp, c_f32, c_f32, c_vp]),
    "a3d_adamw_f32": (c_int, [c_vp, c_vp, c_vp, c_vp, c_vp, c_i64, c_f32, c_f32, c_f32, c_f32, c_f32, c_f32, c_f32, c_vp]),
    "a3d_gs_preprocess_f32": (c_int, [c_vp, c_int, c_int, c_vp, c_i64, c_vp, c_i64, c_vp, c_i64, c_vp, c_i64, c_vp, c_i64, c_int, c_int, c_vp, c_i64, c_vp, c_vp, c_vp, c_vp, c_vp, c_int, c_int, c_f32, c_vp, c_vp, c_vp, c_vp, c_vp, c_vp, c_vp]),
    "a3d_gs_duplicate_f32": (c_int, [c_vp, c_int, c_int, c_int, c_int, c_vp, c_vp, c_vp, c_vp, c_vp, c_vp]),
    "a3d_gs_tile_ranges_f32": (c_int, [c_vp, c_vp, c_i64, c_vp, c_i64]),
    "a3d_gs_render_f32": (c_int, [c_vp, c_int, c_int, c_int, c_int, c_vp, c_vp, c_vp, c_vp, c_vp, c_vp, c_vp, c_vp, c_vp, c_vp, c_vp, c_vp, c_vp]),
    "a3d_gs_render_bwd_f32": (c_int, [c_vp, c_int, c_int, c_int, c_int, c_vp, c_vp, c_vp, c_vp, c_vp, c_vp, c_vp, c_vp, c_vp, c_vp, c_vp,
                                      c_vp, c_vp, c_vp]),
    "a3d_gs_preprocess_bwd_f32": (c_int, [c_vp, c_int, c_int, c_vp, c_i64, c_vp, c_i64, c_vp, c_i64, c_vp, c_i64, c_vp, c_i64, c_int, c_int, c_vp, c_i64, c_vp, c_vp, c_vp, c_vp, c_vp, c_int, c_int, c_f32, c_vp, c_vp, c_vp, c_vp, c_vp, c_vp, c_vp, c_vp, c_vp, c_vp, c_vp, c_vp]),
    "a3d_gs_sum_batch_f32": (c_int, [c_vp, c_vp, c_vp, c_int, c_i64]),
    "a3d_dg_cells_f32": (c_int, [c_vp, c_int, c_vp, c_vp, c_vp]),
    "a3d_dg_mean_partials": (c_i64, [c_int]),
    "a3d_dg_forward_f32": (c_int, [c_vp, c_int, c_int, c_int, c_vp, c_vp, c_vp, c_vp, c_vp, c_vp, c_vp, c_int, c_vp, c_vp, c_vp, c_vp, c_vp, c_vp,
                                   c_vp, c_vp, c_vp]),
    "a3d_dg_backward_ws_floats": (c_i64, [c_int, c_int, c_vp]),
    "a3d_dg_backward_f32": (c_int, [c_vp, c_int, c_int, c_int, c_vp, c_vp, c_vp, c_vp, c_vp, c_vp, c_vp, c_int, c_vp, c_vp, c_vp, c_vp, c_vp,
                                    c_vp, c_vp, c_vp, c_vp, c_vp, c_vp, c_vp, c_vp, c_vp, c_vp]),
    "a3d_knn_f32": (c_int, [c_vp, c_int, c_vp, c_int, c_int, c_f32, c_vp, c_vp]),
    "a3d_arap_energy_f32": (c_int, [c_vp, c_int, c_int, c_int, c_int, c_vp, c_vp, c_i64, c_vp, c_vp, c_vp, c_vp, c_vp, c_vp, c_vp]),
    "a3d_arap_backward_f32": (c_int, [c_vp, c_int, c_int, c_int, c_int, c_vp, c_vp, c_i64, c_vp, c_vp, c_vp, c_vp, c_vp, c_vp, c_vp, c_vp, c_vp]),
    "a3d_mesh_sample_neighbours": (c_int, [c_vp, c_int, c_int, c_vp, c_vp, c_int, c_vp, c_vp]),
    "a3d_mesh_vertex_gaussians_f32": (c_int, [c_vp, c_int, c_int, c_int, c_vp, c_vp, c_vp, c_vp, c_vp, c_vp, c_vp, c_vp, c_int, c_int, c_vp,
                                              c_int, c_vp, c_vp, c_f64, c_f64, c_vp, c_vp, c_vp, c_vp, c_vp, c_vp]),
    "a3d_gaussians_rigid_f32": (c_int, [c_vp, c_int, c_vp, c_vp, c_vp, c_vp, c_vp, c_f64, c_vp, c_vp, c_vp]),
    "a3d_recon_loss_f32": (c_int, [c_vp, c_int, c_int, c_int, c_vp, c_vp, c_vp, c_vp, c_vp, c_f32, c_f64, c_f64, c_vp, c_i64, c_vp]),
    "a3d_recon_loss_bwd_f32": (c_int, [c_vp, c_int, c_int, c_int, c_vp, c_vp, c_vp, c_vp, c_vp, c_f32, c_f32, c_f32, c_vp, c_vp, c_vp]),
    "a3d_image_reg_f32": (c_int, [c_vp, c_int, c_int, c_int, c_vp, c_vp, c_vp, c_f64, c_f64, c_f64, c_vp, c_i64, c_vp]),
    "a3d_image_reg_bwd_f32": (c_int, [c_vp, c_int, c_int, c_int, c_vp, c_vp, c_vp, c_f32, c_f32, c_f32, c_f32, c_f32, c_vp, c_vp, c_vp, c_vp]),
    "a3d_gaussian_reg_f32": (c_int, [c_vp, c_int, c_int, c_vp, c_vp, c_i64, c_vp, c_vp, c_f64, c_f64, c_f64, c_vp, c_i64, c_vp]),
    "a3d_gaussian_reg_bwd_f32": (c_int, [c_vp, c_int, c_int, c_vp, c_vp, c_f32, c_f32, c_f32, c_vp, c_vp, c_vp, c_vp]),
    "a3d_clip_preprocess_lds_limit": (c_i64, []),
    "a3d_clip_preprocess": (c_int, [c_vp, c_vp, c_int, c_int, c_int, c_i64, c_i64, c_i64, c_i64, c_vp, c_int, c_int, c_vp, c_vp, c_int, c_int,
                                    c_vp, c_vp, c_int, c_int, c_int, c_int, c_vp, c_int, c_vp, c_vp, c_int, c_int, c_vp]),
}
_UNSUFFIXED_TWINS = ("a3d_im2col_in", "a3d_unpack_out", "a3d_im2col_in_bwd")
for _name in list(_SIGNATURES):
    if _name.endswith("_bf16"):
        _SIGNATURES[_name[:-5] + "_f16"] = _SIGNATURES[_name]
    elif _name in _UNSUFFIXED_TWINS:
        _SIGNATURES[_name + "_f16"] = _SIGNATURES[_name]
EXPORTED_SYMBOLS = tuple(_SIGNATURES)

_DTYPE_CODE = {torch.float32: 0, torch.bfloat16: 1, torch.float16: 2}
A3D_EUNSUPPORTED = -2


def lib_path() -> str:
    return _LIB_PATH


def load_library():
    global _lib
    if _lib is None:
        if not os.path.exists(_LIB_PATH):
            raise RuntimeError(f"{_LIB_PATH} is missing: run `python -m animate3d_amd.build` (or __graft_entry__.build()). "
                               "There is no CPU fallback for the MI355X kernels.")
        lib = ctypes.CDLL(_LIB_PATH)
        for name, (res, args) in _SIGNATURES.items():
            fn = getattr(lib, name)
            fn.restype, fn.argtypes = res, args
        _lib = lib
    return _lib


GN_PLAN_FIELDS = ("fused", "sg", "nx", "ny", "threads", "rmax", "stream")


def group_norm_plan(rows: int, C: int, groups: int) -> dict:
    out = (c_int * len(GN_PLAN_FIELDS))()
    _check(load_library().a3d_group_norm_plan(rows, C, groups, out), f"a3d_group_norm_plan rows={rows} C={C} groups={groups}")
    plan = dict(zip(GN_PLAN_FIELDS, out))
    plan["iters"] = -(-rows // plan["ny"]) if plan["fused"] else 0
    return plan


def _check(rc: int, what: str):
    if rc != 0:
        kind = {-1: "A3D_EINVAL (shape/alignment precondition)", -2: "A3D_EUNSUPPORTED"}.get(rc, f"hipError {rc}")
        raise RuntimeError(f"{what} failed: {kind}")


def _p(t: Optional[torch.Tensor]):
    return None if t is None else t.data_ptr()


def on_model_device(method):
    import functools

    @functools.wraps(method)
    def wrapper(self, *args, **kwargs):
        dev = self.device
        if dev.type == "cuda" and torch.cuda.current_device() != (dev.index if dev.index is not None else torch.cuda.current_device()):
            with torch.cuda.device(dev):
                return method(self, *args, **kwargs)
        return method(self, *args, **kwargs)
    return wrapper


class _Entry:

    def __init__(self, lib, f16: bool):
        self._lib, self._f16 = lib, f16

    def __getattr__(self, name):
        if self._f16:
            if name.endswith("_bf16"):
                name = name[:-5] + "_f16"
            elif name in _UNSUFFIXED_TWINS:
                name = name + "_f16"
        return getattr(self._lib, name)


class HipOps:

    has_attn_lse = True

    def __init__(self, device: Optional[torch.device] = None, act_dtype: torch.dtype = torch.bfloat16, split_k: bool = True):
        if not torch.cuda.is_available():
            raise RuntimeError("HipOps needs a visible MI355X (torch.cuda.is_available() is False); no CPU fallback exists")
        if act_dtype not in (torch.bfloat16, torch.float16):
            raise ValueError(f"storage type {act_dtype} is not supported (bfloat16 or float16)")
        self.raw_lib = load_library()
        self._kv_row_cache = {}
        self._kv_cover_cache = {}
        self.act_dtype = act_dtype
        self.lib = _Entry(self.raw_lib, act_dtype == torch.float16)
        self.device = torch.device(device) if device is not None else torch.device("cuda", torch.cuda.current_device())
        self.reserved_cus = 0
        self.split_k = bool(split_k)
        self.split_k_gemm = False
        self.attn_counters = None
        self._ws_plan = {}
        self._ws_bufs = {}

    def _workspace(self, need: int) -> torch.Tensor:
        if torch.cuda.is_current_stream_capturing():
            return torch.empty(max(need, 1 << 20), dtype=torch.uint8, device=self.device)
        stream = self._stream()
        buf = self._ws_bufs.get(stream)
        if buf is None or buf.numel() < need:
            buf = self._ws_bufs[stream] = torch.empty(max(need, 1 << 20), dtype=torch.uint8, device=self.device)
        return buf

    def _gemm_flags(self, tile128: bool, ring: bool = False) -> int:
        r = int(self.reserved_cus)
        if not 0 <= r <= 0xFF:
            raise ValueError(f"reserved_cus = {self.reserved_cus}: the flags word of a3d_gemm / a3d_conv3x3 carries 0..255 reserved compute units")
        return r | (0x100 if tile128 else (0x200 if ring else 0))

    def _stream(self):
        return torch.cuda.current_stream(self.device).cuda_stream

    def _act(self, t: torch.Tensor, name: str):
        if t.dtype != self.act_dtype or not t.is_cuda or t.dim() != 2 or t.stride(1) != 1:
            raise RuntimeError(f"{name}: expected a 2-D {self.act_dtype} CUDA tensor with contiguous rows, got {t.dtype} {tuple(t.shape)} {t.device} strides {t.stride()}")
        return t

    def split_cols(self, x, *bounds):
        return tuple(x[:, a:b] for a, b in zip(bounds[:-1], bounds[1:]))

    def empty(self, rows: int, cols: int) -> torch.Tensor:
        return torch.empty((rows, cols), dtype=self.act_dtype, device=self.device)

    def gemm(self, x, w, bias=None, *, residual=None, alpha: float = 1.0, beta: float = 1.0, rowbias=None, rb_div: int = 1, out=None,
             tile128: bool = False, ring: bool = False):
        x, w = self._act(x, "gemm.x"), self._act(w, "gemm.w")
        M, K = x.shape
        N = w.shape[0]
        assert w.shape[1] == K, (x.shape, w.shape)
        y = out if out is not None else self.empty(M, N)
        self._act(y, "gemm.out")
        if residual is not None:
            self._act(residual, "gemm.residual")
            assert residual.shape == (M, N)
        if rowbias is not None:
            self._act(rowbias, "gemm.rowbias")
            assert rowbias.is_contiguous() and rowbias.shape[1] == N
        if bias is not None:
            assert bias.dtype == torch.float32 and bias.numel() == N
        flags = self._gemm_flags(tile128, ring)
        args = (self._stream(), _p(x), x.stride(0), _p(w), w.stride(0), _p(bias), _p(rowbias), rb_div,
                _p(residual), residual.stride(0) if residual is not None else 0, _p(y), y.stride(0), M, N, K, alpha, beta, flags)
        if self.split_k and self.split_k_gemm and not tile128 and M <= 32768 and K >= 1152:
            key = ("gemm", M, N, K, x.stride(0), w.stride(0), y.stride(0), rb_div if rowbias is not None else 0, flags)
            need = self._ws_plan.get(key)
            if need is None:
                q = c_i64(0)
                _check(self.lib.a3d_gemm_ws_bf16(*args, None, 0, ctypes.byref(q)), f"a3d_gemm_ws_bf16 (query) M={M} N={N} K={K}")
                need = self._ws_plan[key] = int(q.value)
            if need > 0:
                ws = self._workspace(need)
                _check(self.lib.a3d_gemm_ws_bf16(*args, _p(ws), need, None), f"a3d_gemm_ws_bf16 M={M} N={N} K={K}")
                return y
        rc = self.lib.a3d_gemm_bf16(*args)
        _check(rc, f"a3d_gemm_bf16 M={M} N={N} K={K}")
        return y

    def gemm2(self, xa, xb, w, bias=None):
        xa, xb, w = self._act(xa, "gemm2.xa"), self._act(xb, "gemm2.xb"), self._act(w, "gemm2.w")
        M, K1 = xa.shape
        K = K1 + xb.shape[1]
        N = w.shape[0]
        assert xb.shape[0] == M and w.shape[1] == K
        if K1 % 64 or K % 64 or N % 8:
            return None
        y = self.empty(M, N)
        rc = self.lib.a3d_gemm2_bf16(self._stream(), _p(xa), xa.stride(0), _p(xb), xb.stride(0), K1, _p(w), w.stride(0), _p(bias), _p(y), y.stride(0),
                                     M, N, K, self._gemm_flags(False))
        if rc == A3D_EUNSUPPORTED:
            return None
        _check(rc, f"a3d_gemm2_bf16 M={M} N={N} K={K1}+{K - K1}")
        return y

    @staticmethod
    def interleave_geglu(w: torch.Tensor) -> torch.Tensor:
        n = w.shape[0] // 2
        assert n % 32 == 0
        h, g = w[:n].reshape(n // 32, 32, *w.shape[1:]), w[n:].reshape(n // 32, 32, *w.shape[1:])
        return torch.stack([h, g], dim=1).reshape(w.shape).contiguous()

    def gemm_geglu(self, x, w_il, bias_il, *, tile128: bool = False):
        x, w_il = self._act(x, "geglu.x"), self._act(w_il, "geglu.w")
        M, K = x.shape
        N2 = w_il.shape[0]
        y = self.empty(M, N2 // 2)
        rc = self.lib.a3d_gemm_geglu_bf16(self._stream(), _p(x), x.stride(0), _p(w_il), w_il.stride(0), _p(bias_il), _p(y), y.stride(0), M, N2, K,
                                          self._gemm_flags(tile128))
        _check(rc, f"a3d_gemm_geglu_bf16 M={M} N2={N2} K={K}")
        return y

    def conv3x3(self, x, B: int, H: int, W: int, w, bias, *, stride: int = 1, up2x: bool = False, rowbias=None, rb_div: int = 1, residual=None,
                up_size=None, tile128: bool = False):
        x, w = self._act(x, "conv.x"), self._act(w, "conv.w")
        Cin = x.shape[1]
        Cout = w.shape[0]
        assert x.is_contiguous() and w.is_contiguous() and x.shape[0] == B * H * W and w.shape[1] == 9 * Cin
        He, We = (2 * H, 2 * W) if up2x else (H, W)
        up_code = 1 if up2x else 0
        if up_size is not None:
            if not up2x or up_size[0] not in (2 * H, 2 * H - 1) or up_size[1] not in (2 * W, 2 * W - 1):
                raise ValueError(f"forced upsample size {tuple(up_size)} is not reachable from {(H, W)} (2x or 2x - 1 per axis)")
            He, We = int(up_size[0]), int(up_size[1])
            up_code |= (2 if He == 2 * H - 1 else 0) | (4 if We == 2 * W - 1 else 0)
        Ho, Wo = (He - 1) // stride + 1, (We - 1) // stride + 1
        y = self.empty(B * Ho * Wo, Cout)
        if residual is not None:
            assert residual.is_contiguous() and residual.shape == y.shape
        if rowbias is not None:
            assert rowbias.is_contiguous() and rowbias.shape[1] == Cout
        flags = self._gemm_flags(tile128)
        args = (self._stream(), _p(x), _p(w), _p(bias), _p(rowbias), rb_div, _p(residual), _p(y), B, H, W, Cin, Cout, stride, up_code, flags)
        if self.split_k and not tile128 and B * Ho * Wo <= 32768:
            key = ("conv", B, H, W, Cin, Cout, stride, up_code, rb_div if rowbias is not None else 0, flags)
            need = self._ws_plan.get(key)
            if need is None:
                q = c_i64(0)
                _check(self.lib.a3d_conv3x3_ws_bf16(*args, None, 0, ctypes.byref(q)), f"a3d_conv3x3_ws_bf16 (query) B={B} H={H} W={W} Cin={Cin} Cout={Cout}")
                need = self._ws_plan[key] = int(q.value)
            if need > 0:
                ws = self._workspace(need)
                _check(self.lib.a3d_conv3x3_ws_bf16(*args, _p(ws), need, None), f"a3d_conv3x3_ws_bf16 B={B} H={H} W={W} Cin={Cin} Cout={Cout}")
                return y, Ho, Wo
        rc = self.lib.a3d_conv3x3_bf16(*args)
        _check(rc, f"a3d_conv3x3_bf16 B={B} H={H} W={W} Cin={Cin} Cout={Cout} stride={stride} up={up2x}")
        return y, Ho, Wo

    def flash_attn(self, q, k, v, qmap: RowMap, kmap: RowMap, groups: int, heads: int, q_len: int, kv_len: int, *,
                   out=None, out_scale: float = 1.0, accumulate: bool = False, causal: bool = False, with_lse: bool = False,
                   accumulation_target: bool = False, exact: bool = False, plain: bool = False):
        q, k, v = self._act(q, "attn.q"), self._act(k, "attn.k"), self._act(v, "attn.v")
        C = q.shape[1]
        D = C // heads
        assert k.stride(0) == v.stride(0)
        o = out if out is not None else self.empty(q.shape[0], C)
        qm, km, om = qmap.c(q.stride(0)), kmap.c(k.stride(0)), qmap.c(o.stride(0))
        flags = (1 if accumulate else 0) | (2 if causal else 0) | (4 if exact else 0) | (8 if plain else 0)
        if with_lse:
            lse = torch.empty((groups, heads, q_len), dtype=torch.float32, device=self.device)
            rc = self.lib.a3d_flash_attn_lse_bf16(self._stream(), _p(q), _p(k), _p(v), _p(o), ctypes.byref(qm), ctypes.byref(km), ctypes.byref(om),
                                                  groups, heads, D, q_len, kv_len, float(D) ** -0.5, out_scale,
                                                  flags, _p(lse))
            _check(rc, f"a3d_flash_attn_lse_bf16 groups={groups} heads={heads} D={D} q_len={q_len} kv_len={kv_len}")
            return o, lse
        if self.attn_counters is not None:
            cnt = self.attn_counters
            assert cnt.dtype == torch.int32 and cnt.is_cuda and cnt.numel() >= 3 and cnt.is_contiguous()
            rc = self.lib.a3d_flash_attn_counted_bf16(self._stream(), _p(q), _p(k), _p(v), _p(o), ctypes.byref(qm), ctypes.byref(km), ctypes.byref(om),
                                                      groups, heads, D, q_len, kv_len, float(D) ** -0.5, out_scale, flags, _p(cnt))
            _check(rc, f"a3d_flash_attn_counted_bf16 groups={groups} heads={heads} D={D} q_len={q_len} kv_len={kv_len}")
            return o
        rc = self.lib.a3d_flash_attn_bf16(self._stream(), _p(q), _p(k), _p(v), _p(o), ctypes.byref(qm), ctypes.byref(km), ctypes.byref(om),
                                          groups, heads, D, q_len, kv_len, float(D) ** -0.5, out_scale, flags)
        _check(rc, f"a3d_flash_attn_bf16 groups={groups} heads={heads} D={D} q_len={q_len} kv_len={kv_len}")
        return o

    def flash_attn2(self, q, k, v, k2, v2, qmap: RowMap, kmap: RowMap, kmap2: RowMap, groups: int, heads: int, q_len: int, kv_len: int,
                    kv_len2: int, *, out_scale2: float = 1.0):
        D = q.shape[1] // heads
        if D not in (40, 80):
            return None
        q, k, v, k2, v2 = self._act(q, "attn.q"), self._act(k, "attn.k"), self._act(v, "attn.v"), self._act(k2, "attn.k2"), self._act(v2, "attn.v2")
        assert k.stride(0) == v.stride(0) and k2.stride(0) == v2.stride(0)
        o = self.empty(q.shape[0], q.shape[1])
        qm, km, km2, om = qmap.c(q.stride(0)), kmap.c(k.stride(0)), kmap2.c(k2.stride(0)), qmap.c(o.stride(0))
        rc = self.lib.a3d_flash_attn2_bf16(self._stream(), _p(q), _p(k), _p(v), _p(k2), _p(v2), _p(o), ctypes.byref(qm), ctypes.byref(km),
                                           ctypes.byref(km2), ctypes.byref(om), groups, heads, D, q_len, kv_len, kv_len2, float(D) ** -0.5,
                                           1.0, out_scale2, 0)
        _check(rc, f"a3d_flash_attn2_bf16 groups={groups} heads={heads} D={D} q_len={q_len} kv_len={kv_len} kv_len2={kv_len2}")
        return o

    def temporal_attn(self, q, k, v, videos: int, frames: int, L: int, heads: int, *, q_f0: int = 0, q_frames: Optional[int] = None,
                      out=None):
        q, k, v = self._act(q, "tattn.q"), self._act(k, "tattn.k"), self._act(v, "tattn.v")
        C = q.shape[1]
        D = C // heads
        assert k.stride(0) == v.stride(0)
        o = self._act(out, "tattn.out") if out is not None else self.empty(q.shape[0], C)
        assert o.shape == (q.shape[0], C)
        if q_frames is None or q_frames == frames:
            assert q.stride(0) == k.stride(0)
            rc = self.lib.a3d_temporal_attn_bf16(self._stream(), _p(q), _p(k), _p(v), q.stride(0), _p(o), o.stride(0),
                                                 videos, frames, L, heads, D, float(D) ** -0.5)
        else:
            assert q.shape[0] == videos * q_frames * L and k.shape[0] == videos * frames * L
            rc = self.lib.a3d_temporal_attn_sharded_bf16(self._stream(), _p(q), q.stride(0), _p(k), _p(v), k.stride(0), _p(o), o.stride(0),
                                                         videos, frames, L, heads, D, float(D) ** -0.5, q_f0, q_frames, q_frames,
                                                         videos * q_frames * L)
        _check(rc, f"a3d_temporal_attn_bf16 videos={videos} frames={frames} L={L} D={D} q_f0={q_f0} q_frames={q_frames}")
        return o

    def group_norm(self, x, B: int, rows: int, gamma, beta, groups: int, eps: float, silu: bool):
        x = self._act(x, "gn.x")
        assert x.is_contiguous() and x.shape[0] == B * rows
        C = x.shape[1]
        y = self.empty(x.shape[0], C)
        ws = torch.empty(int(self.lib.a3d_group_norm_ws_floats(B, rows, groups)), dtype=torch.float32, device=self.device)
        rc = self.lib.a3d_group_norm_bf16(self._stream(), _p(x), _p(y), _p(gamma), _p(beta), _p(ws), B, rows, C, groups, eps, 1 if silu else 0)
        _check(rc, f"a3d_group_norm_bf16 B={B} rows={rows} C={C}")
        return y

    def group_norm2(self, xa, xb, B: int, rows: int, gamma, beta, groups: int, eps: float, silu: bool):
        xa, xb = self._act(xa, "gn2.xa"), self._act(xb, "gn2.xb")
        assert xa.is_contiguous() and xb.is_contiguous() and xa.shape[0] == B * rows == xb.shape[0]
        Ca, Cb = xa.shape[1], xb.shape[1]
        y = self.empty(xa.shape[0], Ca + Cb)
        ws = torch.empty(int(self.lib.a3d_group_norm_ws_floats(B, rows, groups)), dtype=torch.float32, device=self.device)
        rc = self.lib.a3d_group_norm2_bf16(self._stream(), _p(xa), Ca, _p(xb), Cb, _p(y), _p(gamma), _p(beta), _p(ws), B, rows, groups, eps, 1 if silu else 0)
        _check(rc, f"a3d_group_norm2_bf16 B={B} rows={rows} C={Ca}+{Cb}")
        return y

    def group_norm_sums(self, x, B: int, rows: int, groups: int) -> torch.Tensor:
        x = self._act(x, "gn.x")
        assert x.is_contiguous() and x.shape[0] == B * rows
        ws = torch.empty(int(self.lib.a3d_group_norm_ws_floats(B, rows, groups)), dtype=torch.float32, device=self.device)
        sums = torch.empty((B, groups, 2), dtype=torch.float64, device=self.device)
        _check(self.lib.a3d_group_norm_sums_bf16(self._stream(), _p(x), _p(ws), _p(sums), B, rows, x.shape[1], groups),
               f"a3d_group_norm_sums_bf16 B={B} rows={rows} C={x.shape[1]}")
        return sums

    def group_norm_apply(self, x, B: int, rows: int, gamma, beta, groups: int, stats: torch.Tensor, silu: bool):
        x = self._act(x, "gn.x")
        assert x.is_contiguous() and x.shape[0] == B * rows
        assert stats.dtype == torch.float32 and stats.is_contiguous() and stats.shape == (B, groups, 2)
        y = self.empty(x.shape[0], x.shape[1])
        _check(self.lib.a3d_group_norm_apply_bf16(self._stream(), _p(x), _p(y), _p(gamma), _p(beta), _p(stats), B, rows, x.shape[1], groups,
                                                  1 if silu else 0), f"a3d_group_norm_apply_bf16 B={B} rows={rows} C={x.shape[1]}")
        return y

    def layer_norm(self, x, gamma, beta, eps: float, pe1=None, pe1_div: int = 1, pe2=None, pe2_div: int = 1, two: bool = False):
        x = self._act(x, "ln.x")
        assert x.is_contiguous()
        M, C = x.shape
        y1 = self.empty(M, C)
        y2 = self.empty(M, C) if two else None
        for pe in (pe1, pe2):
            if pe is not None:
                self._act(pe, "ln.pe")
                assert pe.is_contiguous() and pe.shape[1] == C
        rc = self.lib.a3d_layer_norm_bf16(self._stream(), _p(x), _p(y1), _p(y2), _p(gamma), _p(beta), M, C, eps,
                                          _p(pe1), pe1_div, pe1.shape[0] if pe1 is not None else 1,
                                          _p(pe2), pe2_div, pe2.shape[0] if pe2 is not None else 1)
        _check(rc, f"a3d_layer_norm_bf16 M={M} C={C}")
        return (y1, y2) if two else y1

    def geglu(self, x):
        x = self._act(x, "geglu.x")
        M, N2 = x.shape
        y = self.empty(M, N2 // 2)
        _check(self.lib.a3d_geglu_bf16(self._stream(), _p(x), x.stride(0), _p(y), y.stride(0), M, N2 // 2), "a3d_geglu_bf16")
# ... 286 lines not shown
```

### animate3d_amd/unet.py

```python
from __future__ import annotations

import math
import os
import re
from types import SimpleNamespace
from typing import Any, Dict, Optional, Tuple, Union

import torch
import torch.nn as nn

from . import modules as M
from .config import UNetConfig
from .embeddings import sine_pos_2d, sinusoidal_pos_1d
from .hip_ops import RowMap, on_model_device


class UNet3DConditionOutput:

    def __init__(self, sample: torch.Tensor):
        self.sample = sample

    def __getitem__(self, i):
        return (self.sample,)[i]

# ... 300 lines not shown
        return self

    def _invalidate(self):
        self._packed = None
        self._packed_frozen = None
        if self._train_ops is not None:
            self._train_ops._persistent.clear()

    @property
    def ops(self):
        if self._active_ops is not None:
            return self._active_ops
        return self._base_ops()

    def _base_ops(self):
        if self._ops is None:
            from .hip_ops import HipOps
            self._ops = HipOps(self.device, torch.float16 if self.dtype == torch.float16 else torch.bfloat16)
            self._ops_auto = True
        return self._ops

    def _d(self, t: torch.Tensor) -> torch.Tensor:
        return t if (self._pack_grad and t.requires_grad) else t.detach()

    def _w(self, t: torch.Tensor) -> torch.Tensor:
        if self._pack_grad and t.requires_grad and t.is_leaf:
            return self._wcat([t])
        return self._d(t).to(self.ops.act_dtype).contiguous()

    def _wcat(self, ws, interleave: bool = False) -> torch.Tensor:
        if self._pack_grad and any(w.requires_grad for w in ws):
            from .autograd_ops import pack_weight
            return pack_weight(self.ops.act_dtype, list(ws), interleave)
        w = ws[0].detach() if len(ws) == 1 else torch.cat([w.detach() for w in ws], 0)
        if interleave:
            w = self.ops.interleave_geglu(w)
        return w.to(self.ops.act_dtype).contiguous()

    def _f(self, t: Optional[torch.Tensor]) -> Optional[torch.Tensor]:
        return None if t is None else self._d(t).float().contiguous()

    def _conv_w(self, conv: nn.Conv2d) -> torch.Tensor:
        w = self._d(conv.weight)
        return self._w(w.permute(0, 2, 3, 1).reshape(w.shape[0], -1))

    def _fold(self, a: torch.Tensor, b_t: torch.Tensor) -> torch.Tensor:
        ops = self._base_ops()
        dt = ops.act_dtype
        a, b_t = a.detach().float().contiguous(), b_t.detach().float().contiguous()
        ah, bh = a.to(dt), b_t.to(dt)
        al, bl = (a - ah.float()).to(dt), (b_t - bh.float()).to(dt)
        return ops.gemm_f32out(ah, bh) + ops.gemm_f32out(ah, bl) + ops.gemm_f32out(al, bh)

    def _pack_resnet(self, r: M.ResnetBlock2D):
        return SimpleNamespace(
            n1=(self._f(r.norm1.weight), self._f(r.norm1.bias)), eps=r.norm1.eps,
            c1=(self._conv_w(r.conv1), self._f(r.conv1.bias)),
            temb=(self._w(r.time_emb_proj.weight), self._f(r.time_emb_proj.bias)),
            n2=(self._f(r.norm2.weight), self._f(r.norm2.bias)),
            c2=(self._conv_w(r.conv2), self._f(r.conv2.bias)),
            sc=None if r.conv_shortcut is None else (self._conv_w(r.conv_shortcut), self._f(r.conv_shortcut.bias)))

    def _pack_ff(self, tb):
        return SimpleNamespace(n3=(self._f(tb.norm3.weight), self._f(tb.norm3.bias)),
                               ff1=(self._wcat([tb.ff.net[0].proj.weight], interleave=True),
                                    self._f(self.ops.interleave_geglu(self._d(tb.ff.net[0].proj.bias)))),
                               ff2=(self._w(tb.ff.net[2].weight), self._f(tb.ff.net[2].bias)))

    def _pack_t2d(self, t: M.Transformer2DModel):
        tb = t.transformer_blocks[0]
        a1, a2 = tb.attn1, tb.attn2
        p1, p2 = a1.processor, a2.processor
        if p1.kind not in ("mvdream", "mvdream_i2v") or p2.kind != "ip_adapter":
            raise TypeError("Transformer2D layers need a MVDream(I2V) processor on attn1 and an IPAdapter processor on attn2")
        qkv = [a1.to_k.weight, a1.to_v.weight, a1.to_q.weight]
        i2v = p1.kind == "mvdream_i2v"
        if i2v:
            qkv.append(p1.to_q_i2v.weight)
        out = SimpleNamespace(
            heads=a1.heads, i2v=i2v,
            norm=(self._f(t.norm.weight), self._f(t.norm.bias)),
            pin=(self._conv_w(t.proj_in), self._f(t.proj_in.bias)),
            n1=(self._f(tb.norm1.weight), self._f(tb.norm1.bias)),
            qkv=self._wcat(qkv),
            oi2v=(self._w(p1.to_out_i2v.weight), self._f(p1.to_out_i2v.bias)) if i2v else None,
            o1=(self._w(a1.to_out[0].weight), self._f(a1.to_out[0].bias)),
            n2=(self._f(tb.norm2.weight), self._f(tb.norm2.bias)),
            q2=self._w(a2.to_q.weight),
            kv_text=self._wcat([a2.to_k.weight, a2.to_v.weight]),
            kv_ip=[self._wcat([k.weight, v.weight]) for k, v in zip(p2.to_k_ip, p2.to_v_ip)],
            ip_scale=list(p2.scale), ip_tokens=list(p2.num_tokens),
            o2=(self._w(a2.to_out[0].weight), self._f(a2.to_out[0].bias)),
            pout=(self._conv_w(t.proj_out), self._f(t.proj_out.bias)))
        out.o1m = None
        if i2v and not self._pack_grad:
            wo, wi = a1.to_out[0].weight.detach().float(), p1.to_out_i2v.weight.detach().float()
            bias = a1.to_out[0].bias.detach().float()
            if p1.to_out_i2v.bias is not None:
                bias = bias + self._fold(p1.to_out_i2v.bias.detach().float()[None, :], wo)[0]
            out.o1m = (self._w(torch.cat([wo, self._fold(wo, wi.t())], dim=1)), self._f(bias))
        out.ff = self._pack_ff(tb)
        return out

    def _pack_motion(self, m: M.TransformerTemporalModel):
        tb = m.transformer_blocks[0]
        attns = []
        for a, ln in ((tb.attn1, tb.norm1), (tb.attn2, tb.norm2)):
            pr = a.processor
            if pr.kind != "spatio_temporal":
                raise TypeError("motion-module attention layers need a SpatioTemporalI2VAttnProcessor")
            C = a.to_q.weight.shape[0]
            if hasattr(pr, "time_pos_embed"):
                pe = pr.time_pos_embed.pe[0]
            else:
                pe = sinusoidal_pos_1d(C, self.config.motion_max_seq_length)[0].to(a.to_q.weight.device)
            proc_pe = hasattr(pr, "time_pos_embed")
            ct, cs, ci = pr.blend_coefficients_t() if self._pack_grad else pr.blend_coefficients()
            if self._pack_grad:
                self._coef_tensors.extend(c for c in (ct, cs, ci) if torch.is_tensor(c))
            ns = SimpleNamespace(
                heads=a.heads, spatial=pr.use_spatial_attn, image=pr.use_image_attn,
                spatial_pe=pr.use_spatial_attn and pr.use_spatial_encoding, camera_pe=pr.use_spatial_attn and pr.use_camera_encoding,
                n=(self._f(ln.weight), self._f(ln.bias)),
                qkv=self._wcat([a.to_q.weight, a.to_k.weight, a.to_v.weight]),
                o=(self._w(a.to_out[0].weight), self._f(a.to_out[0].bias)),
                pe_t=self._w(pe), coef=(ct, cs, ci), proc=pr,
                block_pe=not proc_pe)
            if pr.use_spatial_attn:
                ns.qkv_sp = self._wcat([pr.to_k_sp.weight, pr.to_v_sp.weight, pr.to_q_sp.weight])
                ns.osp = (self._w(pr.to_out_sp.weight), self._f(pr.to_out_sp.bias))
            if pr.use_image_attn:
                ns.qkv_img = self._wcat([pr.to_k_i2v.weight, pr.to_v_i2v.weight, pr.to_q_i2v.weight])
                ns.oimg = (self._w(pr.to_out_i2v.weight), self._f(pr.to_out_i2v.bias))
            ns.om = None
            if not self._pack_grad and (pr.use_spatial_attn or pr.use_image_attn):
                parts = [(ct, a.to_out[0])]
                if pr.use_spatial_attn:
                    parts.append((cs, pr.to_out_sp))
                if pr.use_image_attn:
                    parts.append((ci, pr.to_out_i2v))
                bias = None
                for c, lin in parts:
                    if lin.bias is not None:
                        bias = float(c) * lin.bias.detach().float() if bias is None else bias + float(c) * lin.bias.detach().float()
                ns.om = (self._w(torch.cat([float(c) * lin.weight.detach().float() for c, lin in parts], dim=1)), self._f(bias))
            attns.append(ns)
        out = SimpleNamespace(norm=(self._f(m.norm.weight), self._f(m.norm.bias)),
                              pin=(self._w(m.proj_in.weight), self._f(m.proj_in.bias)),
                              attns=attns,
                              pout=(self._w(m.proj_out.weight), self._f(m.proj_out.bias)))
        out.ff = self._pack_ff(tb)
        return out

    def _pack_block(self, blk: M.MotionBlock):
        return SimpleNamespace(
            resnets=[self._pack_resnet(r) for r in blk.resnets],
            t2d=[self._pack_t2d(t) for t in blk.attentions] if blk.has_cross_attention else None,
            motion=[self._pack_motion(m) for m in blk.motion_modules],
            down=None if blk.downsamplers is None else (self._conv_w(blk.downsamplers[0].conv), self._f(blk.downsamplers[0].conv.bias)),
            up=None if blk.upsamplers is None else (self._conv_w(blk.upsamplers[0].conv), self._f(blk.upsamplers[0].conv.bias)))

    def _pack(self):
        cfg = self.config
        dev = self.device
        te, P = self.time_embedding, SimpleNamespace()
        P.time = (self._w(te.linear_1.weight), self._f(te.linear_1.bias), self._w(te.linear_2.weight), self._f(te.linear_2.bias))
        P.cam = None
        if cfg.camera_embedding_dim is not None:
            ce = self.camera_embedding
            w1 = torch.zeros(ce.linear_1.weight.shape[0], 64, device=dev, dtype=torch.float32)
            w1[:, : cfg.camera_embedding_dim] = ce.linear_1.weight.detach().float()
            P.cam = (self._w(w1), self._f(ce.linear_1.bias), self._w(ce.linear_2.weight), self._f(ce.linear_2.bias))
        P.ip = None
        if self.encoder_hid_proj is not None:
            ipl = self.encoder_hid_proj.image_projection_layers[0]
            P.ip = (self._w(ipl.image_embeds.weight), self._f(ipl.image_embeds.bias), self._f(ipl.norm.weight), self._f(ipl.norm.bias), ipl.norm.eps)
        wi = self.conv_in.weight.detach().float().permute(0, 2, 3, 1).reshape(self.conv_in.weight.shape[0], -1)
        wpad = torch.zeros(wi.shape[0], 64, device=dev, dtype=torch.float32)
        wpad[:, : wi.shape[1]] = wi
        P.conv_in = (self._w(wpad), self._f(self.conv_in.bias))
        P.down = [self._pack_block(b) for b in self.down_blocks]
        P.mid = self._pack_block(self.mid_block)
        P.up = [self._pack_block(b) for b in self.up_blocks]
        P.norm_out = (self._f(self.conv_norm_out.weight), self._f(self.conv_norm_out.bias))
        P.conv_out = (self._conv_w(self.conv_out), self._f(self.conv_out.bias))
        P.cond = self._pack_conditioning(P)
        self._packed = P
        return P

    def _pack_conditioning(self, P):
        blocks = [*P.down, P.mid, *P.up]
        res = [r for b in blocks for r in b.resnets]
        t2d = [t for b in blocks if b.t2d is not None for t in b.t2d]
        c = SimpleNamespace(temb=None, kv_text=None, kv_ip=None, perm={}, widths=[r.temb[0].shape[0] for r in res])
        if res:
            off = 0
            for r in res:
                r.temb_off = (off, r.temb[0].shape[0])
                off += r.temb[0].shape[0]
            c.temb = (torch.cat([r.temb[0] for r in res], 0).contiguous(), torch.cat([r.temb[1] for r in res], 0).contiguous(), off)
        if t2d:
            off = 0
            for t in t2d:
                t.kv_off = (off, t.kv_text.shape[0])
                off += t.kv_text.shape[0]
            c.kv_text = torch.cat([t.kv_text for t in t2d], 0).contiguous()
            if all(len(t.kv_ip) == 1 and t.kv_ip[0].shape[0] == t.kv_text.shape[0] for t in t2d):
                c.kv_ip = torch.cat([t.kv_ip[0] for t in t2d], 0).contiguous()
        return c

    def _project_conditioning(self, c, semb, text_rows, ip_rows):
        ops = self.ops
        out = SimpleNamespace(tp=None, M=0, kvt=None, kvi=None)
        if c.temb is not None:
            M = semb.shape[0]
            perm = c.perm.get(M)
            if perm is None:
                total = c.temb[2]
                idx = torch.arange(M * total, device=semb.device).view(M, total)
                parts, off = [], 0
                for w in c.widths:
                    parts.append(idx[:, off:off + w].reshape(-1))
                    off += w
                perm = c.perm[M] = torch.cat(parts).contiguous()
            out.tp = ops.gemm(semb, c.temb[0], c.temb[1]).reshape(-1).index_select(0, perm)
            out.M = M
        if c.kv_text is not None:
            out.kvt = ops.gemm(text_rows, c.kv_text)
            if c.kv_ip is not None and len(ip_rows) == 1:
                out.kvi = ops.gemm(ip_rows[0], c.kv_ip)
        return out


    def _pe_spatial(self, C: int, h: int, w: int) -> torch.Tensor:
        key = (C, h, w)
        if key not in self._pe_cache:
            self._pe_cache[key] = sine_pos_2d(C // 2, h, w).to(device=self.device, dtype=self.ops.act_dtype).contiguous()
        return self._pe_cache[key]

    def _pe_spatial_general(self, a, C: int, h: int, w: int, n: int, F: int, view0: int = 0):
        pr = a.proc
        L = h * w
        pe = None
        if self._active_ops is not None:
            learn = ([pr.spatial_pos_embed.row_embed.weight, pr.spatial_pos_embed.col_embed.weight]
                     if a.spatial_pe and pr.spatial_encoding_type == "learnable" else [])
            learn += [pr.camera_embed.embedding_table.weight] if a.camera_pe and pr.camera_encoding_type == "learnable" else []
            if any(t.requires_grad for t in learn):
                raise NotImplementedError("learnable positional / camera-encoding tables are not trainable on this path (the reference's "
                                          "training configuration uses the sinusoid encodings); freeze them (requires_grad_(False))")
        if a.spatial_pe:
            if pr.spatial_encoding_type == "learnable":
                sp = pr.spatial_pos_embed
                if h > sp.row_embed.weight.shape[0] or w > sp.col_embed.weight.shape[0]:
                    raise ValueError(f"feature map {(h, w)} exceeds the learnable positional tables "
                                     f"({sp.row_embed.weight.shape[0]} x {sp.col_embed.weight.shape[0]})")
                xe = sp.col_embed.weight.detach().float()[:w][None, :, :].expand(h, w, -1)
                ye = sp.row_embed.weight.detach().float()[:h][:, None, :].expand(h, w, -1)
                pe = torch.cat([xe, ye], dim=-1).reshape(L, C).to(self.device)
            else:
                pe = sine_pos_2d(C // 2, h, w).to(self.device)
        if not a.camera_pe:
            return pe.to(self.ops.act_dtype).contiguous(), 1
        cam = pr.camera_embed.embedding_table.weight if pr.camera_encoding_type == "learnable" else pr.camera_embed.pe[0]
        cam = cam.detach().float().to(self.device)[view0:view0 + n]
        if cam.shape[0] != n:
            raise ValueError(f"camera encoding holds {pr.camera_embed} vectors, the call has views {view0}..{view0 + n}")
        tab = cam[:, None, None, :].expand(n, F, L, C)
        if pe is not None:
            tab = tab + pe[None, None, :, :]
        return tab.reshape(n * F * L, C).to(self.ops.act_dtype).contiguous(), 1

    def _resnet(self, x, B2, H, W, pk, semb, rb_rows):
        ops, g = self.ops, self.config.norm_num_groups
        L = H * W
        sc = None
        if isinstance(x, tuple):
            xa, xb = x
            sc = ops.gemm2(xa, xb, pk.sc[0], pk.sc[1]) if pk.sc is not None else None
            if sc is None:
                x = ops.concat(xa, xb)
                h = ops.group_norm(x, B2, L, pk.n1[0], pk.n1[1], g, pk.eps, True)
            else:
                h = ops.group_norm2(xa, xb, B2, L, pk.n1[0], pk.n1[1], g, pk.eps, True)
        else:
            h = ops.group_norm(x, B2, L, pk.n1[0], pk.n1[1], g, pk.eps, True)
        c = self._cond
        if c is not None and c.tp is not None and hasattr(pk, "temb_off"):
            o, N = pk.temb_off
            tp = c.tp[c.M * o: c.M * (o + N)].view(c.M, N)
        else:
            tp = ops.gemm(semb, pk.temb[0], pk.temb[1])
        h, _, _ = ops.conv3x3(h, B2, H, W, pk.c1[0], pk.c1[1], rowbias=tp, rb_div=rb_rows * L)
        h = ops.group_norm(h, B2, L, pk.n2[0], pk.n2[1], g, pk.eps, True)
        if sc is None:
            sc = x if pk.sc is None else ops.gemm(x, pk.sc[0], pk.sc[1])
        out, _, _ = ops.conv3x3(h, B2, H, W, pk.c2[0], pk.c2[1], residual=sc)
        return out

    def _ff(self, h, pk):
        ops = self.ops
        n3 = ops.layer_norm(h, pk.n3[0], pk.n3[1], 1e-5)
        u = ops.gemm_geglu(n3, pk.ff1[0], pk.ff1[1])
        return ops.gemm(u, pk.ff2[0], pk.ff2[1], residual=h)

    def _mv_maps(self, n, F, L):
        qm = RowMap(gdiv=F, ga=n * F * L, gb=L, seg_len=L, seg_stride=F * L)
        k0 = RowMap(gdiv=F, ga=n * F * L, gb=0, seg_len=L, seg_stride=F * L)
        return qm, k0

    def _mv_attention(self, x, w_kvq, C, V, n, F, L, heads, i2v, overlap=None, out_a=None, out_ai=None):
        ops, par = self.ops, self.parallel
        if par is not None and par.world == 1:
# ... 334 lines not shown

    def _forward_impl(self, sample, timestep, encoder_hidden_states, *, packed, timestep_cond, attention_mask, cross_attention_kwargs,
                      added_cond_kwargs, down_block_additional_residuals, mid_block_additional_residual, return_dict, camera, num_views,
                      i2v_cond_time_zero):
        assert sample.shape[0] % num_views == 0, "[UNet] input batch size must be dividable by num_views!"
        if timestep_cond is not None:
            raise ValueError("timestep_cond needs a time_embedding.cond_proj, which this UNet (time_cond_proj_dim = None) does not have")
        if attention_mask is not None:
            self._reject_attention_mask(attention_mask, sample, num_views)
        if cross_attention_kwargs:
            extra = set(cross_attention_kwargs) - {"scale"}
            if extra:
                raise NotImplementedError(f"cross_attention_kwargs {sorted(extra)} are not supported (only the LoRA `scale`, a no-op here)")
        residuals = down_block_additional_residuals is not None or mid_block_additional_residual is not None
        if residuals and (torch.is_grad_enabled() and getattr(self, "_training_enabled", False)):
            raise NotImplementedError("ControlNet residuals are an inference input (:787-796, 816-817); the training path does not differentiate them")
        if residuals and self.parallel is not None and self.parallel.world > 1:
            raise NotImplementedError("ControlNet residuals with a sharded (shard_unet) model are not supported")
        cfg, ops = self.config, self.ops
        V, _, F, H, W = sample.shape
        n = self.num_views or num_views
        if V % n != 0:
            raise AssertionError("[UNet] input batch size must be dividable by the processors' num_views!")
        nlev = len(cfg.block_out_channels)
        if min(H, W) < (1 << (nlev - 1)):
            raise ValueError(f"latent size {(H, W)} is smaller than the {1 << (nlev - 1)}x total down-sampling")
        if F > cfg.motion_max_seq_length:
            raise ValueError(f"num_frames {F} exceeds motion_max_seq_length {cfg.motion_max_seq_length}")
        P = packed if packed is not None else (self._packed if self._packed is not None else self._pack())
        dev, adt = sample.device, ops.act_dtype
        img_embeds = None if added_cond_kwargs is None else added_cond_kwargs.get("image_embeds")
        if torch.is_tensor(timestep) and timestep.numel() not in (1, V):
            raise ValueError(f"timestep must be a scalar or have one entry per video, got {tuple(timestep.shape)}")
        par = self.parallel if (self.parallel is not None and self.parallel.world > 1) else None
        V_full, n_full, F_full, f0 = V, n, F, 0
        if par is not None:
            par.configure(V // n, n, F)
            idx = par.local_videos_on(V, n, dev)
            f0, F = par.frame_range(F)
            sample = sample.index_select(0, idx)[:, :, f0:f0 + F]
            encoder_hidden_states = encoder_hidden_states.to(dev).index_select(0, idx)
            camera = None if camera is None else camera.to(dev).index_select(0, idx)
            img_embeds = None if img_embeds is None else img_embeds.to(dev).index_select(0, idx)
            if torch.is_tensor(timestep) and timestep.numel() == V:
                timestep = timestep.to(dev).reshape(-1).index_select(0, idx)
            V, n = idx.numel(), n // par.view_shards
        self._frames = (F_full, f0)
        B2 = V * F

        if not torch.is_tensor(timestep):
            t = torch.full((V,), float(timestep), dtype=torch.float32, device=dev)
        else:
            t = timestep.to(device=dev, dtype=torch.float32).reshape(-1).expand(V).contiguous()

        def time_mlp(tt):
            e = ops.gemm(ops.timestep_embed(tt, cfg.block_out_channels[0]), P.time[0], P.time[1])
            return ops.gemm(ops.silu(e), P.time[2], P.time[3])

        emb = time_mlp(t)
        cond_emb = time_mlp(torch.zeros_like(t)) if i2v_cond_time_zero else None
        if camera is not None:
            assert camera.shape[0] == V
            if P.cam is None:
                raise ValueError("camera passed but the model has no camera_embedding")
            cam = torch.zeros((V, 64), dtype=adt, device=dev)
            cam[:, : camera.shape[1]] = camera.to(device=dev, dtype=adt)
            c1 = ops.silu(ops.gemm(cam, P.cam[0], P.cam[1]))
            emb = ops.gemm(c1, P.cam[2], P.cam[3], residual=emb)
            if cond_emb is not None:
                cond_emb = ops.gemm(c1, P.cam[2], P.cam[3], residual=cond_emb)
        if cond_emb is None:
            semb, rb_rows = ops.silu(emb), F
        else:
            per_img = emb[:, None, :].repeat(1, F, 1)
            if f0 == 0:
                per_img[:, 0] = cond_emb
            semb, rb_rows = ops.silu(per_img.reshape(B2, -1).contiguous()), 1

        T = encoder_hidden_states.shape[1]
        text_rows = encoder_hidden_states.to(device=dev, dtype=adt).reshape(V * T, -1).contiguous()
        ip_rows = []
        if self.encoder_hid_proj is not None and cfg.encoder_hid_dim_type == "ip_image_proj":
            if img_embeds is None:
                raise ValueError(f"{self.__class__} has the config param `encoder_hid_dim_type` set to 'ip_image_proj' which requires the "
                                 "keyword argument `image_embeds` to be passed in  `added_conditions`")
            img = img_embeds.to(device=dev, dtype=adt).reshape(V, -1).contiguous()
            pr = ops.gemm(img, P.ip[0], P.ip[1]).reshape(V * cfg.ip_num_tokens, cfg.cross_attention_dim)
            ip_rows.append(ops.layer_norm(pr, P.ip[2], P.ip[3], P.ip[4]))

        self._cond = None
        if self.stack_conditioning and self._active_ops is None and getattr(P, "cond", None) is not None and P is self._packed:
            self._cond = self._project_conditioning(P.cond, semb, text_rows, ip_rows)

        x = ops.gemm(ops.im2col_in(sample), P.conv_in[0], P.conv_in[1])
        h_, w_ = H, W
        skips = [x]
        sizes = [(H, W)]
        ckpt = bool(getattr(self, "_gradient_checkpointing", False)) and torch.is_grad_enabled() and self._active_ops is not None

        def layer(x_in, rp, tp, mp, hh, ww):
            aops = self._active_ops
            def run(xx):
                prev, self._active_ops = self._active_ops, aops
                try:
                    xx = self._resnet(xx, B2, hh, ww, rp, semb, rb_rows)
                    if tp is not None:
                        xx = self._t2d(xx, V, n, F, hh, ww, tp, text_rows, ip_rows, T)
                    return self._motion(xx, V, n, F, hh, ww, mp)
                finally:
                    self._active_ops = prev
            if ckpt:
                from torch.utils.checkpoint import checkpoint
                return checkpoint(run, x_in, use_reentrant=False, preserve_rng_state=False)
            return run(x_in)

        for pk in P.down:
            for j, rp in enumerate(pk.resnets):
                x = layer(x, rp, pk.t2d[j] if pk.t2d is not None else None, pk.motion[j], h_, w_)
                skips.append(x)
            if pk.down is not None:
                x, h_, w_ = ops.conv3x3(x, B2, h_, w_, pk.down[0], pk.down[1], stride=2)
                skips.append(x)
                sizes.append((h_, w_))
        def plus(x_rows, res, hh, ww):
            C = x_rows.shape[1]
            if tuple(res.shape) != (B2, C, hh, ww):
                raise ValueError(f"additional residual of shape {tuple(res.shape)}, expected {(B2, C, hh, ww)}")
            r = ops.empty(B2 * hh * ww, C)
            r.copy_(res.to(device=dev).permute(0, 2, 3, 1).reshape(B2 * hh * ww, C))
            return ops.axpby_(x_rows, r, 1.0, 1.0)

        if down_block_additional_residuals is not None:
            if len(down_block_additional_residuals) != len(skips):
                raise ValueError(f"{len(down_block_additional_residuals)} down-block residuals for {len(skips)} skip connections")
            geo = [sizes[0]]
            for bi, pkd in enumerate(P.down):
                geo += [sizes[bi]] * len(pkd.resnets) + ([sizes[bi + 1]] if pkd.down is not None else [])
            skips = [plus(s_, r_, *g_) for s_, r_, g_ in zip(skips, down_block_additional_residuals, geo)]
        pk = P.mid
        x = layer(x, pk.resnets[0], pk.t2d[0], pk.motion[0], h_, w_)
        x = self._resnet(x, B2, h_, w_, pk.resnets[1], semb, rb_rows)
        if mid_block_additional_residual is not None:
            x = plus(x, mid_block_additional_residual, h_, w_)
        lvl = len(sizes) - 1
        for bi, (blk, pk) in enumerate(zip(self.up_blocks, P.up)):
            for j, rp in enumerate(pk.resnets):
                skip = skips.pop()
                if getattr(self, "_freeu_factors", None) is not None:
                    x, skip = self._freeu(bi, x, skip, B2, h_, w_)
                pair = self._active_ops is None and hasattr(ops, "gemm2") and hasattr(ops, "group_norm2")
                x = layer((x, skip) if pair else ops.concat(x, skip), rp, pk.t2d[j] if pk.t2d is not None else None, pk.motion[j], h_, w_)
            if pk.up is not None:
                lvl -= 1
                x, h_, w_ = ops.conv3x3(x, B2, h_, w_, pk.up[0], pk.up[1], up2x=True, up_size=sizes[lvl])
        x = ops.group_norm(x, B2, h_ * w_, P.norm_out[0], P.norm_out[1], cfg.norm_num_groups, cfg.norm_eps, True)
        x, _, _ = ops.conv3x3(x, B2, h_, w_, P.conv_out[0], P.conv_out[1])
        out_dtype = sample.dtype if sample.dtype in (torch.float32, torch.bfloat16, torch.float16) else torch.float32
        out = ops.unpack_out(x, V, cfg.out_channels, F, H, W, out_dtype)
        if par is not None:
            out = par.all_gather_output(out, V_full, n_full, F_full)
        if not return_dict:
            return (out,)
        return UNet3DConditionOutput(sample=out)
```

### animate3d_amd/vae.py

```python
from __future__ import annotations

from dataclasses import dataclass
from types import SimpleNamespace
from typing import Optional, Tuple, Union

import torch
import torch.nn as nn

from .autograd_ops import AutogradOps
from .denoise import randn_like_reference
from .hip_ops import on_model_device


@dataclass
class VAEConfig:
    block_out_channels: Tuple[int, ...] = (128, 256, 512, 512)
    layers_per_block: int = 2
    norm_num_groups: int = 32
    latent_channels: int = 4
    out_channels: int = 3
    scaling_factor: float = 0.18215
    attention_head_dim: int = 512


# ... 68 lines not shown
    def __init__(self, cfg: VAEConfig):
        super().__init__()
        boc, g = cfg.block_out_channels, cfg.norm_num_groups
        self.conv_in = nn.Conv2d(cfg.out_channels, boc[0], 3, padding=1)
        self.down_blocks = nn.ModuleList()
        cout = boc[0]
        for i, c in enumerate(boc):
            cin, cout = cout, c
            self.down_blocks.append(_DownBlock(cin, cout, cfg.layers_per_block, g, downsample=i != len(boc) - 1))
        self.mid_block = _Mid(boc[-1], g)
        self.conv_norm_out = nn.GroupNorm(g, boc[-1], eps=1e-6)
        self.conv_out = nn.Conv2d(boc[-1], 2 * cfg.latent_channels, 3, padding=1)


def mid_attention(ops, x, B: int, L: int, pk, groups: int, keep: bool = False):
    C = x.shape[1]
    t = ops.group_norm(x, B, L, pk.gn[0], pk.gn[1], groups, 1e-6, False)
    q = ops.gemm(t, pk.q[0], pk.q[1])
    k = ops.gemm(t, pk.k[0], pk.k[1])
    a = ops.empty(B * L, C)
    Lp = -(-L // 64) * 64
    if Lp != L:
        p_pad, vt_pad = ops.empty(L, Lp).zero_(), ops.empty(C, Lp).zero_()
    for b in range(B):
        rows = slice(b * L, (b + 1) * L)
        s = ops.gemm_f32out(q[rows], k[rows], alpha=C ** -0.5)
        if Lp == L:
            p = ops.softmax_rows(s)
            vt = ops.gemm(pk.v[0], t[rows])
        else:
            ops.softmax_rows(s, out=p_pad[:, :L])
            ops.gemm(pk.v[0], t[rows], out=vt_pad[:, :L])
            p, vt = p_pad, vt_pad
        ops.gemm(p, vt, pk.v[1], out=a[rows])
    out = ops.gemm(a, pk.o[0], pk.o[1], residual=x)
    return (out, t, q, k) if keep else out


class _VAEHalf(nn.Module):

    def __init__(self, config: Optional[VAEConfig], ops):
        super().__init__()
        cfg = config or VAEConfig()
        if cfg.block_out_channels[-1] // cfg.attention_head_dim > 1:
            raise ValueError("only the single-head mid-block attention of the SD VAE is implemented")
        self.config = cfg
        self._ops = ops
        self._ops_auto = False
        self._packed = None

    @property
    def device(self):
        return next(self.parameters()).device

    @property
    def dtype(self):
        return next(self.parameters()).dtype

    @property
    def ops(self):
        if self._ops is None:
            from .hip_ops import HipOps
            self._ops = HipOps(self.device, torch.float16 if self.dtype == torch.float16 else torch.bfloat16)
            self._ops_auto = True
        return self._ops

    def load_state_dict(self, state_dict, strict: bool = True, **kw):
        self._packed = None
        return super().load_state_dict(state_dict, strict=strict, **kw)

    def _apply(self, fn, *a, **kw):
        self._packed = None
        if getattr(self, "_ops_auto", False):
            self._ops, self._ops_auto = None, False
        return super()._apply(fn, *a, **kw)

    def init_synthetic(self, seed: int = 0):
        g = torch.Generator(device=self.device).manual_seed(seed)
        with torch.no_grad():
            for name, p in self.named_parameters():
                if p.dim() >= 2:
                    p.copy_(((torch.rand(p.shape, generator=g, device=p.device) * 2 - 1) * p[0].numel() ** -0.5).to(p.dtype))
                elif "norm" in name and name.endswith("weight"):
                    p.copy_((1 + 0.1 * torch.randn(p.shape, generator=g, device=p.device)).to(p.dtype))
                else:
                    p.copy_((0.05 * torch.randn(p.shape, generator=g, device=p.device)).to(p.dtype))
        self._packed = None
        return self

    def _w(self, t):
        return t.detach().to(self.ops.act_dtype).contiguous()

    def _f(self, t):
        return None if t is None else t.detach().float().contiguous()

    def _conv_w(self, conv, pad_out_to: int = 0):
        w = conv.weight.detach().float().permute(0, 2, 3, 1).reshape(conv.weight.shape[0], -1)
        b = conv.bias.detach().float()
        if pad_out_to > w.shape[0]:
            w = torch.cat([w, w.new_zeros(pad_out_to - w.shape[0], w.shape[1])])
            b = torch.cat([b, b.new_zeros(pad_out_to - b.shape[0])])
        return self._w(w), b.contiguous()

    def _pack_resnet(self, r: _Resnet):
        sc = None
        if r.conv_shortcut is not None:
            sc = (self._w(r.conv_shortcut.weight.detach().reshape(r.conv_shortcut.weight.shape[0], -1)), self._f(r.conv_shortcut.bias))
        return SimpleNamespace(n1=(self._f(r.norm1.weight), self._f(r.norm1.bias)), c1=self._conv_w(r.conv1),
                               n2=(self._f(r.norm2.weight), self._f(r.norm2.bias)), c2=self._conv_w(r.conv2), sc=sc)

    def _resnet(self, x, B, H, W, pk, ops=None):
        ops, g = (self.ops if ops is None else ops), self.config.norm_num_groups
        h = ops.group_norm(x, B, H * W, pk.n1[0], pk.n1[1], g, 1e-6, True)
        h, _, _ = ops.conv3x3(h, B, H, W, pk.c1[0], pk.c1[1])
        h = ops.group_norm(h, B, H * W, pk.n2[0], pk.n2[1], g, 1e-6, True)
        sc = x if pk.sc is None else ops.gemm(x, pk.sc[0], pk.sc[1])
        out, _, _ = ops.conv3x3(h, B, H, W, pk.c2[0], pk.c2[1], residual=sc)
        return out

    def _mid_attention(self, x, B, H, W, pk, ops=None):
        ops = self.ops if ops is None else ops
        differentiable = getattr(ops, "vae_mid_attention", None)
        if differentiable is not None:
            return differentiable(x, B, H * W, pk, self.config.norm_num_groups)
        return mid_attention(ops, x, B, H * W, pk, self.config.norm_num_groups)


class AutoencoderKLDecoder(_VAEHalf):

    def __init__(self, config: Optional[VAEConfig] = None, ops=None, device: Optional[Union[str, torch.device]] = None):
        super().__init__(config, ops)
        cfg = self.config
        with (torch.device(device) if device is not None else torch.device("cpu")):
            self.post_quant_conv = nn.Conv2d(cfg.latent_channels, cfg.latent_channels, 1)
            self.decoder = _Decoder(cfg)

    def _pack(self):
        d, cfg = self.decoder, self.config
        P = SimpleNamespace()
        P.pq = (self.post_quant_conv.weight.detach().float().reshape(cfg.latent_channels, cfg.latent_channels).contiguous(),
                self._f(self.post_quant_conv.bias))
        wi = d.conv_in.weight.detach().float().permute(0, 2, 3, 1).reshape(d.conv_in.weight.shape[0], -1)
        wpad = wi.new_zeros(wi.shape[0], 64)
        wpad[:, : wi.shape[1]] = wi
        P.conv_in = (self._w(wpad), self._f(d.conv_in.bias))
        a = d.mid_block.attentions[0]
        P.mid = SimpleNamespace(
            r0=self._pack_resnet(d.mid_block.resnets[0]), r1=self._pack_resnet(d.mid_block.resnets[1]),
            gn=(self._f(a.group_norm.weight), self._f(a.group_norm.bias)),
            q=(self._w(a.to_q.weight), self._f(a.to_q.bias)), k=(self._w(a.to_k.weight), self._f(a.to_k.bias)),
            v=(self._w(a.to_v.weight), self._f(a.to_v.bias)), o=(self._w(a.to_out[0].weight), self._f(a.to_out[0].bias)))
        P.up = [SimpleNamespace(res=[self._pack_resnet(r) for r in b.resnets],
                                up=None if b.upsamplers is None else self._conv_w(b.upsamplers[0].conv)) for b in d.up_blocks]
        P.norm_out = (self._f(d.conv_norm_out.weight), self._f(d.conv_norm_out.bias))
        P.conv_out = self._conv_w(d.conv_out, pad_out_to=4)
        self._packed = P
        return P

    @torch.no_grad()
    @on_model_device
    def decode(self, z: torch.Tensor, scale: float = 1.0) -> torch.Tensor:
        ops, cfg = self.ops, self.config
        P = self._packed if self._packed is not None else self._pack()
        B, Cz, H, W = z.shape
        z = ops.channel_mix(z.to(device=self.device, dtype=torch.float32).contiguous(), P.pq[0], P.pq[1], scale)
        x = ops.gemm(ops.im2col_in(z.reshape(B, Cz, 1, H, W)), P.conv_in[0], P.conv_in[1])
        x = self._resnet(x, B, H, W, P.mid.r0)
        x = self._mid_attention(x, B, H, W, P.mid)
        x = self._resnet(x, B, H, W, P.mid.r1)
        for blk in P.up:
            for r in blk.res:
                x = self._resnet(x, B, H, W, r)
            if blk.up is not None:
                x, H, W = ops.conv3x3(x, B, H, W, blk.up[0], blk.up[1], up2x=True)
        x = ops.group_norm(x, B, H * W, P.norm_out[0], P.norm_out[1], cfg.norm_num_groups, 1e-6, True)
        x, _, _ = ops.conv3x3(x, B, H, W, P.conv_out[0], P.conv_out[1])
        img = ops.unpack_out(x, B, 4, 1, H, W, torch.float32)
        return img[:, : cfg.out_channels, 0].contiguous()

    @torch.no_grad()
    def decode_latents(self, latents: torch.Tensor) -> torch.Tensor:
        b, c, f, h, w = latents.shape
        z = latents.permute(0, 2, 1, 3, 4).reshape(b * f, c, h, w)
        image = self.decode(z, scale=1.0 / self.config.scaling_factor)
        return image[None, :].reshape((b, f, -1) + image.shape[2:]).permute(0, 2, 1, 3, 4).float()


class AutoencoderKLEncoder(_VAEHalf):

    def __init__(self, config: Optional[VAEConfig] = None, ops=None, device: Optional[Union[str, torch.device]] = None):
        super().__init__(config, ops)
        cfg = self.config
        with (torch.device(device) if device is not None else torch.device("cpu")):
            self.encoder = _Encoder(cfg)
            self.quant_conv = nn.Conv2d(2 * cfg.latent_channels, 2 * cfg.latent_channels, 1)
        self._gops = None

    def _pack(self):
        e, cfg = self.encoder, self.config
        P = SimpleNamespace()
        wi = e.conv_in.weight.detach().float().permute(0, 2, 3, 1).reshape(e.conv_in.weight.shape[0], -1)
        wpad = wi.new_zeros(wi.shape[0], 64)
        wpad[:, : wi.shape[1]] = wi
        P.conv_in = (self._w(wpad), self._f(e.conv_in.bias))
        P.down = []
        for b in e.down_blocks:
            dn = None
            if b.downsamplers is not None:
                conv = b.downsamplers[0].conv
                w = conv.weight.detach().float().flip(2, 3).permute(0, 2, 3, 1).reshape(conv.weight.shape[0], -1)
                dn = (self._w(w), self._f(conv.bias))
            P.down.append(SimpleNamespace(res=[self._pack_resnet(r) for r in b.resnets], down=dn))
        a = e.mid_block.attentions[0]
        P.mid = SimpleNamespace(
            r0=self._pack_resnet(e.mid_block.resnets[0]), r1=self._pack_resnet(e.mid_block.resnets[1]),
            gn=(self._f(a.group_norm.weight), self._f(a.group_norm.bias)),
            q=(self._w(a.to_q.weight), self._f(a.to_q.bias)), k=(self._w(a.to_k.weight), self._f(a.to_k.bias)),
            v=(self._w(a.to_v.weight), self._f(a.to_v.bias)), o=(self._w(a.to_out[0].weight), self._f(a.to_out[0].bias)))
        P.norm_out = (self._f(e.conv_norm_out.weight), self._f(e.conv_norm_out.bias))
        P.conv_out = self._conv_w(e.conv_out)
        c2 = 2 * cfg.latent_channels
        P.quant = (self.quant_conv.weight.detach().float().reshape(c2, c2).contiguous(), self._f(self.quant_conv.bias))
        self._packed = P
        return P

    def _downsample(self, x, B, H, W, pk, ops):
        if H % 2 or W % 2:
            raise ValueError(f"VAE encoder needs even feature maps at every level, got {H}x{W}")
        C = x.shape[1]
        xf = x.reshape(B, H, W, C).flip(1, 2).reshape(B * H * W, C).contiguous()
        y, Ho, Wo = ops.conv3x3(xf, B, H, W, pk[0], pk[1], stride=2)
        Co = y.shape[1]
        return y.reshape(B, Ho, Wo, Co).flip(1, 2).reshape(B * Ho * Wo, Co).contiguous(), Ho, Wo

    def _check_images(self, images: torch.Tensor):
        cfg = self.config
        B, Ci, H, W = images.shape
        levels = len(cfg.block_out_channels) - 1
        if Ci != cfg.out_channels or H % (1 << levels) or W % (1 << levels):
            raise ValueError(f"images must be [B, {cfg.out_channels}, H, W] with H, W multiples of {1 << levels}")

    def _moments(self, ops, images: torch.Tensor, unit_range: bool = False) -> torch.Tensor:
        cfg = self.config
        self._check_images(images)
        P = self._packed if self._packed is not None else self._pack()
        B, Ci, H, W = images.shape
        if unit_range:
            cols = ops.im2col_images(images, self.device)
        else:
            img = images.to(device=self.device, dtype=torch.float32).contiguous()
            cols = ops.im2col_in(img.reshape(B, Ci, 1, H, W))
        x = ops.gemm(cols, P.conv_in[0], P.conv_in[1])
        for blk in P.down:
            for r in blk.res:
                x = self._resnet(x, B, H, W, r, ops)
            if blk.down is not None:
                x, H, W = self._downsample(x, B, H, W, blk.down, ops)
        x = self._resnet(x, B, H, W, P.mid.r0, ops)
        x = self._mid_attention(x, B, H, W, P.mid, ops)
        x = self._resnet(x, B, H, W, P.mid.r1, ops)
        x = ops.group_norm(x, B, H * W, P.norm_out[0], P.norm_out[1], cfg.norm_num_groups, 1e-6, True)
        x, _, _ = ops.conv3x3(x, B, H, W, P.conv_out[0], P.conv_out[1])
        c2 = 2 * cfg.latent_channels
        moments = ops.unpack_out(x, B, c2, 1, H, W, torch.float32)[:, :, 0].contiguous()
        return ops.channel_mix(moments, P.quant[0], P.quant[1], 1.0)

    def _grad_ops(self):
        from .vae_grad import VaeGradOps
        base = self._plain_ops()
        if self._gops is None or self._gops.base is not base:
            self._gops = VaeGradOps(base)
        return self._gops

    def _plain_ops(self):
        return self.ops.base if isinstance(self.ops, AutogradOps) else self.ops

    @torch.no_grad()
    @on_model_device
    def encode(self, images: torch.Tensor) -> Tuple[torch.Tensor, torch.Tensor]:
        moments = self._moments(self.ops, images)
        lc = self.config.latent_channels
        mean, logvar = moments[:, :lc], moments[:, lc:]
        return mean.contiguous(), logvar.clamp(-30.0, 20.0).contiguous()

    @torch.no_grad()
    def encode_latents(self, images: torch.Tensor, generator: Optional[torch.Generator] = None) -> torch.Tensor:
        mean, logvar = self.encode(images)
        noise = randn_like_reference(mean.shape, generator, mean.device, mean.dtype)
        return (mean + torch.exp(0.5 * logvar) * noise) * self.config.scaling_factor

    @on_model_device
    def encode_images(self, imgs: torch.Tensor, generator: Optional[torch.Generator] = None,
                      noise: Optional[torch.Tensor] = None) -> torch.Tensor:
        if torch.is_grad_enabled() and imgs.requires_grad:
            moments = self._moments(self._grad_ops(), imgs, unit_range=True)
        else:
            with torch.no_grad():
                moments = self._moments(self._plain_ops(), imgs * 2 - 1)
        lc = self.config.latent_channels
        mean, logvar = moments[:, :lc].contiguous(), moments[:, lc:].clamp(-30.0, 20.0).contiguous()
        if noise is None:
            noise = randn_like_reference(mean.shape, generator, mean.device, mean.dtype)
        else:
            noise = noise.to(device=mean.device, dtype=mean.dtype)
        return ((mean + torch.exp(0.5 * logvar) * noise) * self.config.scaling_factor).to(imgs.dtype)
```

### include/animate3d_hip.h

```cpp
#ifndef ANIMATE3D_HIP_H
#define ANIMATE3D_HIP_H

#include <stdint.h>

#ifdef __cplusplus
extern "C" {
#endif

typedef void* a3d_stream_t;

enum {
  A3D_OK = 0,
  A3D_EINVAL = -1,
  A3D_EUNSUPPORTED = -2
};

enum { A3D_F32 = 0, A3D_BF16 = 1, A3D_F16 = 2 };

const char* a3d_version(void);

typedef struct a3d_rowmap {
  int64_t gdiv, ga, gb;
  int64_t seg_len, seg_stride;
  int64_t ld;
} a3d_rowmap;

#define A3D_GEMM_RESERVED_CUS_MASK 0xff
#define A3D_GEMM_KERNEL_MASK 0x300
#define A3D_GEMM_TILE128 0x100
#define A3D_GEMM_RING 0x200
int a3d_gemm_bf16(a3d_stream_t stream, const void* X, int64_t ldx, const void* W, int64_t ldw,
                  const float* bias, const void* rowbias, int64_t rb_div, const void* R, int64_t ldr,
                  void* Y, int64_t ldy, int64_t M, int64_t N, int64_t K, float alpha, float beta, int flags);

int a3d_gemm_ws_bf16(a3d_stream_t stream, const void* X, int64_t ldx, const void* W, int64_t ldw,
                     const float* bias, const void* rowbias, int64_t rb_div, const void* R, int64_t ldr,
                     void* Y, int64_t ldy, int64_t M, int64_t N, int64_t K, float alpha, float beta, int flags,
                     void* ws, int64_t ws_bytes, int64_t* ws_needed);

int a3d_gemm2_bf16(a3d_stream_t stream, const void* X, int64_t ldx, const void* X2, int64_t ldx2, int64_t K1,
                   const void* W, int64_t ldw, const float* bias, void* Y, int64_t ldy, int64_t M, int64_t N, int64_t K, int flags);

int a3d_gemm_f32out_bf16(a3d_stream_t stream, const void* X, int64_t ldx, const void* W, int64_t ldw,
                         const float* bias, float* Y, int64_t ldy, int64_t M, int64_t N, int64_t K, float alpha);

int a3d_gemm_geglu_bf16(a3d_stream_t stream, const void* X, int64_t ldx, const void* W, int64_t ldw,
                        const float* bias, void* Y, int64_t ldy, int64_t M, int64_t N2, int64_t K, int flags);

int a3d_conv3x3_bf16(a3d_stream_t stream, const void* X, const void* Wp, const float* bias,
                     const void* rowbias, int64_t rb_div, const void* R, void* Y,
                     int B, int H, int W, int Cin, int Cout, int stride, int up2x, int flags);

int a3d_conv3x3_ws_bf16(a3d_stream_t stream, const void* X, const void* Wp, const float* bias,
                        const void* rowbias, int64_t rb_div, const void* R, void* Y,
                        int B, int H, int W, int Cin, int Cout, int stride, int up2x, int flags,
                        void* ws, int64_t ws_bytes, int64_t* ws_needed);

#define A3D_ATTN_ACCUMULATE 1
#define A3D_ATTN_CAUSAL 2
#define A3D_ATTN_EXACT 4
#define A3D_ATTN_PLAIN 8
int a3d_flash_attn_bf16(a3d_stream_t stream, const void* Q, const void* K, const void* V, void* O,
                        const a3d_rowmap* qmap, const a3d_rowmap* kmap, const a3d_rowmap* omap,
                        int groups, int heads, int head_dim, int64_t q_len, int64_t kv_len,
                        float scale, float out_scale, int accumulate);

int a3d_flash_attn_counted_bf16(a3d_stream_t stream, const void* Q, const void* K, const void* V, void* O,
                                const a3d_rowmap* qmap, const a3d_rowmap* kmap, const a3d_rowmap* omap,
                                int groups, int heads, int head_dim, int64_t q_len, int64_t kv_len,
                                float scale, float out_scale, int accumulate, unsigned int* counters);

int a3d_flash_attn2_bf16(a3d_stream_t stream, const void* Q, const void* K, const void* V, const void* K2, const void* V2, void* O,
                         const a3d_rowmap* qmap, const a3d_rowmap* kmap, const a3d_rowmap* kmap2, const a3d_rowmap* omap,
                         int groups, int heads, int head_dim, int64_t q_len, int64_t kv_len, int64_t kv_len2,
                         float scale, float out_scale, float out_scale2, int accumulate);

int a3d_temporal_attn_bf16(a3d_stream_t stream, const void* Q, const void* K, const void* V, int64_t ldqkv,
                           void* O, int64_t ldo, int videos, int frames, int64_t L, int heads,
                           int head_dim, float scale);

int a3d_temporal_attn_sharded_bf16(a3d_stream_t stream, const void* Q, int64_t ldq, const void* K, const void* V, int64_t ldkv,
                                   void* O, int64_t ldo, int videos, int frames, int64_t L, int heads,
                                   int head_dim, float scale, int q_f0, int q_frames, int kv_frames_per_block,
                                   int64_t kv_block_stride);

int64_t a3d_group_norm_ws_floats(int B, int64_t rows, int groups);
int a3d_group_norm_bf16(a3d_stream_t stream, const void* X, void* Y, const float* gamma, const float* beta,
                        float* ws, int B, int64_t rows, int C, int groups, float eps, int silu);

int a3d_group_norm_plan(int64_t rows, int C, int groups, int* out);

int a3d_group_norm2_bf16(a3d_stream_t stream, const void* Xa, int Ca, const void* Xb, int Cb, void* Y, const float* gamma,
                         const float* beta, float* ws, int B, int64_t rows, int groups, float eps, int silu);

int a3d_group_norm_sums_bf16(a3d_stream_t stream, const void* X, float* ws, double* sums, int B, int64_t rows, int C, int groups);
int a3d_group_norm_apply_bf16(a3d_stream_t stream, const void* X, void* Y, const float* gamma, const float* beta,
                              const float* stats, int B, int64_t rows, int C, int groups, int silu);

int a3d_layer_norm_bf16(a3d_stream_t stream, const void* X, void* Y1, void* Y2, const float* gamma,
                        const float* beta, int64_t M, int C, float eps,
                        const void* pe1, int64_t pe1_div, int64_t pe1_mod,
                        const void* pe2, int64_t pe2_div, int64_t pe2_mod);

int a3d_geglu_bf16(a3d_stream_t stream, const void* X, int64_t ldx, void* Y, int64_t ldy, int64_t M, int64_t N);

int a3d_silu_bf16(a3d_stream_t stream, const void* X, void* Y, int64_t n);

int a3d_activation_bf16(a3d_stream_t stream, const void* X, void* Y, int64_t n, int mode);

int a3d_concat_bf16(a3d_stream_t stream, const void* A, int64_t Ca, const void* Bsrc, int64_t Cb, void* Y, int64_t M);

int a3d_timestep_embed_bf16(a3d_stream_t stream, const float* t, void* Y, int V, int dim);

int a3d_im2col_in(a3d_stream_t stream, const void* sample, int dtype, void* Y, int V, int C, int F, int H, int W);

int a3d_im2col_in_bwd(a3d_stream_t stream, const void* dCol, float* dX, int V, int C, int F, int H, int W, float scale);

int a3d_unpack_out(a3d_stream_t stream, const void* X, void* Y, int dtype, int V, int C, int F, int H, int W);

int a3d_softmax_rows_f32_bf16(a3d_stream_t stream, const float* X, int64_t ldx, void* Y, int64_t ldy, int64_t M, int64_t N);

int a3d_softmax_rows_bwd_bf16(a3d_stream_t stream, const void* P, int64_t ldp, const float* dP, int64_t lddp, void* dS, int64_t ldds,
                              int64_t M, int64_t N, float alpha);

int a3d_channel_mix_f32(a3d_stream_t stream, const float* X, const float* W, const float* bias, float* Y,
                        int B, int Cin, int Cout, int64_t HW, float scale);

int a3d_cfg_ddim_step_f32(a3d_stream_t stream, const float* eps_pair, const float* x, const float* first_frame,
                          float* x_prev, int64_t n, int C, int F, int64_t HW, float guidance,
                          float alpha_t, float alpha_prev);



int a3d_flash_attn_bwd_bf16(a3d_stream_t stream, const void* Q, const void* K, const void* V, const void* dO,
                            void* dQ, void* dK, void* dV, float* lse2, float* delta,
                            const a3d_rowmap* qmap, const a3d_rowmap* kmap, const a3d_rowmap* domap,
                            const a3d_rowmap* dqmap, const a3d_rowmap* dkmap,
                            int groups, int heads, int head_dim, int64_t q_len, int64_t kv_len, int q_per_kv,
                            float scale, float do_scale, int accumulate);

int a3d_flash_attn_lse_bf16(a3d_stream_t stream, const void* Q, const void* K, const void* V, void* O,
                            const a3d_rowmap* qmap, const a3d_rowmap* kmap, const a3d_rowmap* omap,
                            int groups, int heads, int head_dim, int64_t q_len, int64_t kv_len,
                            float scale, float out_scale, int accumulate, float* lse2);
int a3d_attn_delta_bf16(a3d_stream_t stream, const void* dO, const void* O, const a3d_rowmap* domap, const a3d_rowmap* omap,
                        float* delta, int groups, int heads, int head_dim, int64_t q_len);

int a3d_temporal_attn_bwd_bf16(a3d_stream_t stream, const void* Q, const void* K, const void* V, int64_t ldqkv,
                               const void* dO, int64_t lddo, void* dQ, void* dK, void* dV, int64_t ldd,
                               int videos, int frames, int64_t L, int heads, int head_dim, float scale);

int a3d_layer_norm_bwd_bf16(a3d_stream_t stream, const void* X, const void* dY, const float* gamma, void* dX,
                            float* dgamma, float* dbeta, int64_t M, int C, float eps, int accumulate);

int a3d_group_norm_bwd_bf16(a3d_stream_t stream, const void* X, const void* dY, const float* gamma, const float* beta,
                            const float* stats, void* dX, float* ws, float* dgamma, float* dbeta,
                            int B, int64_t rows, int C, int groups, int silu);

int a3d_geglu_bwd_bf16(a3d_stream_t stream, const void* P, int64_t ldp, const void* dY, int64_t lddy, void* dP, int64_t lddp,
                       int64_t M, int64_t N);

int a3d_transpose_bf16(a3d_stream_t stream, const void* X, int64_t ldx, void* Y, int64_t ldy, int64_t rows, int64_t cols,
                       int64_t rows_pad);

int64_t a3d_wgrad_ws_floats(int64_t M, int64_t N, int64_t K);
int a3d_wgrad_bf16(a3d_stream_t stream, const void* dY, int64_t lddy, const void* X, int64_t ldx, float* dW, int64_t lddw,
                   float* ws, int64_t M, int64_t N, int64_t K, float alpha, int accumulate);

int a3d_colsum_bf16(a3d_stream_t stream, const void* X, int64_t ldx, int64_t rows, int64_t cols, float* out, float alpha, int accumulate);

int a3d_axpby_bf16(a3d_stream_t stream, const void* X, void* Y, int64_t n, float a, float b);

int a3d_zero_insert2x_bf16(a3d_stream_t stream, const void* dY, void* Z, int B, int H, int W, int C);

int a3d_upsample2x_bwd_bf16(a3d_stream_t stream, const void* dU, void* dX, int B, int H, int W, int He, int We, int C);

int a3d_sqnorm_f32(a3d_stream_t stream, const float* g, int64_t n, float* out, int accumulate);
int a3d_clip_ctrl_f32(a3d_stream_t stream, const float* sqnorm, float max_norm, float inv_loss_scale, float* ctrl);
int a3d_adamw_f32(a3d_stream_t stream, float* p, const float* g, float* m, float* v, int64_t n, float lr, float beta1, float beta2,
                  float eps, float weight_decay, float bias_corr1, float bias_corr2, const float* ctrl);

int a3d_gs_preprocess_f32(a3d_stream_t stream, int B, int N, const float* means, int64_t means_bs, const float* scales, int64_t scales_bs,
                          const float* rots, int64_t rots_bs, const float* opac, int64_t opac_bs, const float* shs, int64_t shs_bs, int M,
                          int deg, const float* colors, int64_t colors_bs, const float* view, const float* proj, const float* campos,
                          const float* tanfovx, const float* tanfovy, int H, int W, float scale_mod, int* radii, float* xy, float* depth,
                          float* conic_o, float* rgb, int* clamped, int* tiles_touched);
int a3d_gs_duplicate_f32(a3d_stream_t stream, int B, int N, int H, int W, const float* xy, const float* depth, const int* radii,
                         const int64_t* offsets, int64_t* keys, int* vals);
int a3d_gs_tile_ranges_f32(a3d_stream_t stream, const int64_t* keys, int64_t L, int* ranges, int64_t n_tiles);
int a3d_gs_render_f32(a3d_stream_t stream, int B, int N, int H, int W, const int* ranges, const int64_t* perm, const int* vals,
                      const float* xy, const float* conic_o, const float* rgb, const float* depth, const float* bg,
                      float* out_img, float* out_depth, float* out_alpha, float* T_final, int* n_contrib);
int a3d_gs_render_bwd_f32(a3d_stream_t stream, int B, int N, int H, int W, const int* ranges, const int64_t* perm, const int* vals,
                          const float* xy, const float* conic_o, const float* rgb, const float* depth, const float* bg,
                          const float* T_final, const int* n_contrib, const float* d_img, const float* d_depth,
                          const float* d_alpha, float* rows);
int a3d_gs_preprocess_bwd_f32(a3d_stream_t stream, int B, int N, const float* means, int64_t means_bs, const float* scales, int64_t scales_bs,
                              const float* rots, int64_t rots_bs, const float* opac, int64_t opac_bs, const float* shs, int64_t shs_bs, int M,
                              int deg, const float* colors, int64_t colors_bs, const float* view, const float* proj, const float* campos,
                              const float* tanfovx, const float* tanfovy, int H, int W, float scale_mod, const int* radii,
                              const int* clamped, const int64_t* offsets, const int* tiles_touched, const float* rows,
                              float* d_means2d, float* d_means, float* d_scales, float* d_rots, float* d_opac, float* d_shs,
                              float* d_colors);
int a3d_gs_sum_batch_f32(a3d_stream_t stream, const float* src, float* dst, int B, int64_t M);

int a3d_dg_cells_f32(a3d_stream_t stream, int N, const float* xyz, const int64_t* plane_desc, int* cells);
int64_t a3d_dg_mean_partials(int N);
int a3d_dg_forward_f32(a3d_stream_t stream, int T, int N, int B, const float* xyz, const float* scaling, const float* rotation,
                       const float* timestamps, const float* grid, const int64_t* plane_desc, const float* weights, int flags,
                       const int* img_start, const int* img_list, float* sp, float* mpart, float* gmean, float* glob, float* means,
                       float* scales, float* rots);
int64_t a3d_dg_backward_ws_floats(int T, int N, const int64_t* plane_desc);
int a3d_dg_backward_f32(a3d_stream_t stream, int T, int N, int B, const float* xyz, const float* scaling, const float* rotation,
                        const float* timestamps, const float* grid, const int64_t* plane_desc, const float* weights, int flags,
                        const int* img_start, const int* img_list, const float* sp, const float* gmean, const float* glob,
                        const int* order, const int* starts, const float* d_means, const float* d_scales, const float* d_rots,
                        float* ws, float* d_grid, float* d_weights, float* d_scaling, float* d_rotation);

int a3d_knn_f32(a3d_stream_t stream, int N, const float* points, int K, int least_edge_num, float radius2, int* nn_idx, float* nn_dist);
int a3d_arap_energy_f32(a3d_stream_t stream, int F, int Nv, int K, int S, const float* source, const float* targets, int64_t targets_bs,
                        const int* nn_idx, const float* weight, const int* sample_idx, double* rot, float* rot_f32, double* energy,
                        float* loss);
int a3d_arap_backward_f32(a3d_stream_t stream, int F, int Nv, int K, int S, const float* source, const float* targets, int64_t targets_bs,
                          const int* nn_idx, const float* weight, const int* sample_idx, const double* rot, const int* order,
                          const int* starts, const float* grad_out, float* d_targets, float* d_source);
int a3d_mesh_sample_neighbours(a3d_stream_t stream, int Nv, int E, const int* row_start, const int* col, int K, const int64_t* seed,
                               int* nn_idx);

int a3d_mesh_vertex_gaussians_f32(a3d_stream_t stream, int Nv, int E, int C, const float* verts, const int* row_start, const int* col,
                                  const int* corner_order, const int* corner_start, const float* vertex_colors, const float* corner_colors,
                                  const float* texture, int Ht, int Wt, const float* uvs, int Nt, const int* corner_uv, const double* rot9,
                                  double scale_factor, double shrink, float* xyz, float* scaling, float* shs, float* colors,
                                  float* mean_edge, float* edge_length);
int a3d_gaussians_rigid_f32(a3d_stream_t stream, int N, const float* xyz_in, const float* scaling_in, const float* rotation_in,
                            const double* rot9, const double* quat4, double scale_factor, float* xyz, float* scaling, float* rotation);

int a3d_recon_loss_f32(a3d_stream_t stream, int B, int H, int W, const float* image, const float* alpha, const float* gt_rgb,
                       const uint8_t* gt_mask, const int* index, float bg, double lambda_rgb, double lambda_mask, float* partials,
                       int64_t n_partials, float* out);
int a3d_recon_loss_bwd_f32(a3d_stream_t stream, int B, int H, int W, const float* image, const float* alpha, const float* gt_rgb,
                           const uint8_t* gt_mask, const int* index, float bg, float coef_rgb, float coef_mask, const float* grad_out,
                           float* d_image, float* d_alpha);

int a3d_image_reg_f32(a3d_stream_t stream, int B, int H, int W, const float* image, const float* depth, const float* alpha, double lambda_tv,
                      double lambda_depth_tv, double lambda_sparsity, float* partials, int64_t n_partials, float* out);
int a3d_image_reg_bwd_f32(a3d_stream_t stream, int B, int H, int W, const float* image, const float* depth, const float* alpha,
                          float coef_tv_h, float coef_tv_w, float coef_depth_tv_h, float coef_depth_tv_w, float coef_sparsity,
                          const float* grad_out, float* d_image, float* d_depth, float* d_alpha);
int a3d_gaussian_reg_f32(a3d_stream_t stream, int B, int N, const float* means, const float* scales, int64_t scales_bs, const float* scaling,
                         const float* opacity, double lambda_position, double lambda_scales, double lambda_opacity, float* partials,
                         int64_t n_partials, float* out);
int a3d_gaussian_reg_bwd_f32(a3d_stream_t stream, int B, int N, const float* means, const float* scaling, float coef_position,
                             float coef_scales, float coef_opacity, const float* grad_out, float* d_means, float* d_scales,
                             float* d_opacity);

int64_t a3d_clip_preprocess_lds_limit(void);
int a3d_clip_preprocess(a3d_stream_t stream, const float* rgb, int n_src, int in_h, int in_w, int64_t s_img, int64_t s_y, int64_t s_x,
                        int64_t s_c, const int* image_index, int n_img, int crop, const int* coef_x, const int* bounds_x, int ksize_x,
                        int off_x, const int* coef_y, const int* bounds_y, int ksize_y, int off_y, int tile_rows, int max_rows,
                        const float* table, int dtype, void* pixel_values, void* patch_rows, int patch, int kp, uint8_t* u8);

int a3d_gemm_f16(a3d_stream_t stream, const void* X, int64_t ldx, const void* W, int64_t ldw,
                  const float* bias, const void* rowbias, int64_t rb_div, const void* R, int64_t ldr,
                  void* Y, int64_t ldy, int64_t M, int64_t N, int64_t K, float alpha, float beta, int flags);
int a3d_gemm_ws_f16(a3d_stream_t stream, const void* X, int64_t ldx, const void* W, int64_t ldw,
                    const float* bias, const void* rowbias, int64_t rb_div, const void* R, int64_t ldr,
                    void* Y, int64_t ldy, int64_t M, int64_t N, int64_t K, float alpha, float beta, int flags,
                    void* ws, int64_t ws_bytes, int64_t* ws_needed);
int a3d_gemm2_f16(a3d_stream_t stream, const void* X, int64_t ldx, const void* X2, int64_t ldx2, int64_t K1,
                  const void* W, int64_t ldw, const float* bias, void* Y, int64_t ldy, int64_t M, int64_t N, int64_t K, int flags);
int a3d_gemm_f32out_f16(a3d_stream_t stream, const void* X, int64_t ldx, const void* W, int64_t ldw,
                         const float* bias, float* Y, int64_t ldy, int64_t M, int64_t N, int64_t K, float alpha);
int a3d_gemm_geglu_f16(a3d_stream_t stream, const void* X, int64_t ldx, const void* W, int64_t ldw,
                        const float* bias, void* Y, int64_t ldy, int64_t M, int64_t N2, int64_t K, int flags);
int a3d_conv3x3_f16(a3d_stream_t stream, const void* X, const void* Wp, const float* bias,
                     const void* rowbias, int64_t rb_div, const void* R, void* Y,
                     int B, int H, int W, int Cin, int Cout, int stride, int up2x, int flags);
int a3d_conv3x3_ws_f16(a3d_stream_t stream, const void* X, const void* Wp, const float* bias,
                       const void* rowbias, int64_t rb_div, const void* R, void* Y,
                       int B, int H, int W, int Cin, int Cout, int stride, int up2x, int flags,
                       void* ws, int64_t ws_bytes, int64_t* ws_needed);
int a3d_flash_attn_f16(a3d_stream_t stream, const void* Q, const void* K, const void* V, void* O,
                        const a3d_rowmap* qmap, const a3d_rowmap* kmap, const a3d_rowmap* omap,
                        int groups, int heads, int head_dim, int64_t q_len, int64_t kv_len,
                        float scale, float out_scale, int accumulate);
int a3d_flash_attn_counted_f16(a3d_stream_t stream, const void* Q, const void* K, const void* V, void* O,
                               const a3d_rowmap* qmap, const a3d_rowmap* kmap, const a3d_rowmap* omap,
                               int groups, int heads, int head_dim, int64_t q_len, int64_t kv_len,
                               float scale, float out_scale, int accumulate, unsigned int* counters);
int a3d_flash_attn2_f16(a3d_stream_t stream, const void* Q, const void* K, const void* V, const void* K2, const void* V2, void* O,
                        const a3d_rowmap* qmap, const a3d_rowmap* kmap, const a3d_rowmap* kmap2, const a3d_rowmap* omap,
                        int groups, int heads, int head_dim, int64_t q_len, int64_t kv_len, int64_t kv_len2,
                        float scale, float out_scale, float out_scale2, int accumulate);
int a3d_temporal_attn_f16(a3d_stream_t stream, const void* Q, const void* K, const void* V, int64_t ldqkv,
                           void* O, int64_t ldo, int videos, int frames, int64_t L, int heads,
                           int head_dim, float scale);
int a3d_temporal_attn_sharded_f16(a3d_stream_t stream, const void* Q, int64_t ldq, const void* K, const void* V, int64_t ldkv,
                                   void* O, int64_t ldo, int videos, int frames, int64_t L, int heads,
                                   int head_dim, float scale, int q_f0, int q_frames, int kv_frames_per_block,
                                   int64_t kv_block_stride);
int a3d_group_norm_f16(a3d_stream_t stream, const void* X, void* Y, const float* gamma, const float* beta,
                        float* ws, int B, int64_t rows, int C, int groups, float eps, int silu);
int a3d_group_norm2_f16(a3d_stream_t stream, const void* Xa, int Ca, const void* Xb, int Cb, void* Y, const float* gamma,
                        const float* beta, float* ws, int B, int64_t rows, int groups, float eps, int silu);
int a3d_group_norm_sums_f16(a3d_stream_t stream, const void* X, float* ws, double* sums, int B, int64_t rows, int C, int groups);
int a3d_group_norm_apply_f16(a3d_stream_t stream, const void* X, void* Y, const float* gamma, const float* beta,
                              const float* stats, int B, int64_t rows, int C, int groups, int silu);
int a3d_layer_norm_f16(a3d_stream_t stream, const void* X, void* Y1, void* Y2, const float* gamma,
                        const float* beta, int64_t M, int C, float eps,
                        const void* pe1, int64_t pe1_div, int64_t pe1_mod,
                        const void* pe2, int64_t pe2_div, int64_t pe2_mod);
int a3d_geglu_f16(a3d_stream_t stream, const void* X, int64_t ldx, void* Y, int64_t ldy, int64_t M, int64_t N);
int a3d_silu_f16(a3d_stream_t stream, const void* X, void* Y, int64_t n);
int a3d_activation_f16(a3d_stream_t stream, const void* X, void* Y, int64_t n, int mode);
int a3d_concat_f16(a3d_stream_t stream, const void* A, int64_t Ca, const void* Bsrc, int64_t Cb, void* Y, int64_t M);
int a3d_timestep_embed_f16(a3d_stream_t stream, const float* t, void* Y, int V, int dim);
int a3d_im2col_in_f16(a3d_stream_t stream, const void* sample, int dtype, void* Y, int V, int C, int F, int H, int W);
int a3d_unpack_out_f16(a3d_stream_t stream, const void* X, void* Y, int dtype, int V, int C, int F, int H, int W);
int a3d_softmax_rows_f32_f16(a3d_stream_t stream, const float* X, int64_t ldx, void* Y, int64_t ldy, int64_t M, int64_t N);
int a3d_softmax_rows_bwd_f16(a3d_stream_t stream, const void* P, int64_t ldp, const float* dP, int64_t lddp, void* dS, int64_t ldds,
                             int64_t M, int64_t N, float alpha);
int a3d_im2col_in_bwd_f16(a3d_stream_t stream, const void* dCol, float* dX, int V, int C, int F, int H, int W, float scale);
int a3d_flash_attn_bwd_f16(a3d_stream_t stream, const void* Q, const void* K, const void* V, const void* dO,
                            void* dQ, void* dK, void* dV, float* lse2, float* delta,
                            const a3d_rowmap* qmap, const a3d_rowmap* kmap, const a3d_rowmap* domap,
                            const a3d_rowmap* dqmap, const a3d_rowmap* dkmap,
                            int groups, int heads, int head_dim, int64_t q_len, int64_t kv_len, int q_per_kv,
                            float scale, float do_scale, int accumulate);
int a3d_flash_attn_lse_f16(a3d_stream_t stream, const void* Q, const void* K, const void* V, void* O,
                           const a3d_rowmap* qmap, const a3d_rowmap* kmap, const a3d_rowmap* omap,
                           int groups, int heads, int head_dim, int64_t q_len, int64_t kv_len,
                           float scale, float out_scale, int accumulate, float* lse2);
int a3d_attn_delta_f16(a3d_stream_t stream, const void* dO, const void* O, const a3d_rowmap* domap, const a3d_rowmap* omap,
                       float* delta, int groups, int heads, int head_dim, int64_t q_len);
int a3d_temporal_attn_bwd_f16(a3d_stream_t stream, const void* Q, const void* K, const void* V, int64_t ldqkv,
                               const void* dO, int64_t lddo, void* dQ, void* dK, void* dV, int64_t ldd,
                               int videos, int frames, int64_t L, int heads, int head_dim, float scale);
int a3d_layer_norm_bwd_f16(a3d_stream_t stream, const void* X, const void* dY, const float* gamma, void* dX,
                            float* dgamma, float* dbeta, int64_t M, int C, float eps, int accumulate);
int a3d_group_norm_bwd_f16(a3d_stream_t stream, const void* X, const void* dY, const float* gamma, const float* beta,
                            const float* stats, void* dX, float* ws, float* dgamma, float* dbeta,
                            int B, int64_t rows, int C, int groups, int silu);
int a3d_geglu_bwd_f16(a3d_stream_t stream, const void* P, int64_t ldp, const void* dY, int64_t lddy, void* dP, int64_t lddp,
                       int64_t M, int64_t N);
int a3d_transpose_f16(a3d_stream_t stream, const void* X, int64_t ldx, void* Y, int64_t ldy, int64_t rows, int64_t cols,
                       int64_t rows_pad);
int a3d_colsum_f16(a3d_stream_t stream, const void* X, int64_t ldx, int64_t rows, int64_t cols, float* out, float alpha, int accumulate);
int a3d_axpby_f16(a3d_stream_t stream, const void* X, void* Y, int64_t n, float a, float b);
int a3d_zero_insert2x_f16(a3d_stream_t stream, const void* dY, void* Z, int B, int H, int W, int C);
int a3d_upsample2x_bwd_f16(a3d_stream_t stream, const void* dU, void* dX, int B, int H, int W, int He, int We, int C);
int a3d_wgrad_f16(a3d_stream_t stream, const void* dY, int64_t lddy, const void* X, int64_t ldx, float* dW, int64_t lddw,
                   float* ws, int64_t M, int64_t N, int64_t K, float alpha, int accumulate);

#ifdef __cplusplus
}
#endif
#endif
```

Before: 2.429 denoise-steps/s.

## Fold nearest-upsample into 3x3 conv as four 2x2 sub-pixel phase convolutions

Adds a folded up-sampling conv path (CONV==3) in which the nearest-2x upsample followed by a 3x3 conv is precomputed into four phase-specific 2x2 filters. Each output phase becomes a GEMM with K=4*Cin instead of 9*Cin, run on the low-resolution input, and the epilogue scatters rows into the interleaved high-resolution output. This cuts conv MACs in the UNet and VAE up blocks to roughly 4/9 of the original. In exchange it adds row-remap arithmetic in the epilogue, weights folded once at pack time (summed in fp32, then rounded back), and a path limited to bias-only, no-residual, no-split-K cases.

```diff
diff --git a/animate3d_amd/csrc/gemm_common.h b/animate3d_amd/csrc/gemm_common.h
--- a/animate3d_amd/csrc/gemm_common.h
+++ b/animate3d_amd/csrc/gemm_common.h
@@ -113,6 +113,27 @@
   __device__ __forceinline__ int pass_col0(int ps) const { return block(2 * ps) * 32; }
 };
 
+A3D_DEV uint32_t udiv_est(uint32_t x, uint32_t d, float rcp) {
+  uint32_t q = (uint32_t)((float)x * rcp);
+  const int32_t r = (int32_t)(x - q * d);
+  if (r < 0) --q;
+  else if (r >= (int32_t)d) ++q;
+  return q;
+}
+constexpr int UP2X_FOLD_MAX_HW = 1 << 20;
+struct Up2xRowMap {
+  int64_t m0, row0;
+  uint32_t rem0, hw, w;
+  float rcp_hw, rcp_w;
+  __device__ __forceinline__ int64_t operator()(int64_t m) const {
+    const uint32_t x = rem0 + (uint32_t)(m - m0);
+    const uint32_t bq = udiv_est(x, hw, rcp_hw);
+    const uint32_t rem = x - bq * hw;
+    const uint32_t i = udiv_est(rem, w, rcp_w), j = rem - i * w;
+    return row0 + (int64_t)bq * (4 * (int64_t)hw) + (int64_t)(4u * i * w + 2u * j);
+  }
+};
+
 constexpr int BIAS_IMG_STRIDE = 2048;
 constexpr int BIAS_IMG_ROWBIAS = 1280;
 constexpr int BIAS_IMG_DMA = 1024;
@@ -144,10 +165,11 @@
   fw[NB - 1] = *reinterpret_cast<const u32x4_t*>(wl + ko);
 }
 
-template <int EPI, int NB>
+struct IdentityRowMap { __device__ __forceinline__ int64_t operator()(int64_t m) const { return m; } };
+template <int EPI, int NB, class ROWMAP = IdentityRowMap>
 A3D_DEV void epilogue_rounded(const GemmParams& p, f32x16_t (&acc)[NB][2], float* const stg, const float* const bias_lds,
                               const uint16_t* const rowbias_lds, const int64_t m0, const int64_t n0, const int wm, const WaveCols<NB> wc,
-                              const int lane) {
+                              const int lane, const ROWMAP rowmap = ROWMAP{}) {
   const int wblk = wc.first, wblk_last = wc.last;
   auto pass_cols = [&](int ps) { return (2 * ps + 1 < NB) ? 64 : 32; };
   auto pass_col0 = [&](int ps) { return ((2 * ps + 1 < NB) ? wblk + 2 * ps : wblk_last) * 32; };
@@ -276,7 +298,7 @@
         const int row = (64 / lpr) * j + lane / lpr;
         const int64_t m = mbase + row;
         const u32x4_t o = unswap(ob[j], row);
-        *reinterpret_cast<u32x4_t*>(p.Y + m * p.ldy + nbase + 8 * cc) = o;
+        *reinterpret_cast<u32x4_t*>(p.Y + rowmap(m) * p.ldy + nbase + 8 * cc) = o;
       }
     }
   }
diff --git a/animate3d_amd/csrc/gemm_conv.hip b/animate3d_amd/csrc/gemm_conv.hip
--- a/animate3d_amd/csrc/gemm_conv.hip
+++ b/animate3d_amd/csrc/gemm_conv.hip
@@ -29,7 +29,14 @@
   const int64_t nblk = p.tiles_n * p.tiles_m;
   const int64_t lid = xcd_remap(blockIdx.x, nblk);
   const int64_t tile_n = lid % p.tiles_n, tile_m = lid / p.tiles_n;
-  const int64_t m0 = tile_m * BM, n0 = tile_n * BN;
+  int64_t m0 = tile_m * BM;
+  const int64_t n0 = tile_n * BN;
+  int phase = 0;
+  if constexpr (CONV == 3) {
+    const int64_t tpp = p.tiles_m >> 2;
+    phase = (int)(tile_m / tpp);
+    m0 = (tile_m - phase * tpp) * BM;
+  }
 
   const int kc = tid % TC::CPR;
   const int srow = tid / TC::CPR;
@@ -51,6 +58,16 @@
       if constexpr (CONV == 2) {
         a_b[i] = b; a_y[i] = oy; a_x[i] = ox;
         a_ptr[i] = nullptr; a_mask[i] = 0;
+      } else if constexpr (CONV == 3) {
+        const int y0 = oy - 1 + (phase >> 1), x0 = ox - 1 + (phase & 1);
+        a_ptr[i] = p.X + (((int64_t)b * p.H + y0) * p.Wd + x0) * p.Cin + kc * 8;
+        int mask = 0;
+#pragma unroll
+        for (int t = 0; t < 4; ++t) {
+          const int yy = y0 + (t >> 1), xx = x0 + (t & 1);
+          if (a_ok[i] && yy >= 0 && yy < p.H && xx >= 0 && xx < p.Wd) mask |= 1 << t;
+        }
+        a_mask[i] = mask;
       } else {
         const int y0 = oy * p.stride - 1, x0 = ox * p.stride - 1;
         a_ptr[i] = p.X + (((int64_t)b * p.H + y0) * p.Wd + x0) * p.Cin + kc * 8;
@@ -73,6 +90,7 @@
     int64_t n = n0 + srow + RPT * i;
     if (n >= p.N) n = p.N - 1;
     w_ptr[i] = p.W + n * p.ldw + kc * 8;
+    if constexpr (CONV == 3) w_ptr[i] += (int64_t)phase * p.N * p.ldw;
   }
 
   struct RegTile { u32x4_t a[NPASS], w[NPASS]; };
@@ -80,15 +98,16 @@
   auto load_tile = [&](int64_t k0, RegTile& rt) {
     u32x4_t (&ra)[NPASS] = rt.a; u32x4_t (&rw)[NPASS] = rt.w;
     if constexpr (CONV != 0) {
+      constexpr int NTAP = CONV == 3 ? 4 : 9, TAPW = CONV == 3 ? 2 : 3;
       {
         const int kt64 = (int)(k0 >> 6);
-        const int c64 = kt64 / 9, t = kt64 - 9 * c64;
+        const int c64 = kt64 / NTAP, t = kt64 - NTAP * c64;
         k0 = (int64_t)t * p.Cin + c64 * 64 + (k0 & 63);
       }
       const int tap = (int)(k0 / p.Cin);
       const int ci0 = (int)(k0 - (int64_t)tap * p.Cin);
-      const int ky = tap / 3, kx = tap - ky * 3;
-      if constexpr (CONV == 1) {
+      const int ky = tap / TAPW, kx = tap - ky * TAPW;
+      if constexpr (CONV == 1 || CONV == 3) {
         const int64_t toff = ((int64_t)ky * p.Wd + kx) * p.Cin + ci0;
 #pragma unroll
         for (int i = 0; i < NPASS; ++i) {
@@ -256,7 +275,15 @@
         for (int e = 0; e < 8; ++e) v[e] += bv[e];
         const uint16_t* rb = p.rowbias ? p.rowbias + (m / p.rb_div) * p.N + n : nullptr;
         const uint16_t* rr = p.R ? p.R + m * p.ldr + n : nullptr;
-        uint16_t* yy = p.Y + m * p.ldy + n;
+        int64_t orow = m;
+        if constexpr (CONV == 3) {
+          const int hw = p.H * p.Wd;
+          const int b = (int)(m / hw);
+          const int rem = (int)(m - (int64_t)b * hw);
+          const int i = rem / p.Wd, j = rem - i * p.Wd;
+          orow = ((int64_t)b * (2 * p.H) + 2 * i + (phase >> 1)) * (2 * p.Wd) + 2 * j + (phase & 1);
+        }
+        uint16_t* yy = p.Y + orow * p.ldy + n;
         if (full) {
           if (rb) {
             const u32x4_t t = *reinterpret_cast<const u32x4_t*>(rb);
@@ -346,9 +373,10 @@
   if (CONV == 0 && (uint64_t)p.ldx * 16u >= (1ull << 31)) return false;
   if ((uint64_t)p.ldw * 16u >= (1ull << 31)) return false;
   if (CONV != 0 && ((uint64_t)p.B * p.H * p.Wd + 2u * p.Wd + 2u) * (uint64_t)p.Cin * 2u >= (1ull << 32)) return false;
-  const int64_t tm = (p.M + PBM - 1) / PBM;
+  if (CONV == 3 && (int64_t)p.H * p.Wd > UP2X_FOLD_MAX_HW) return false;
+  const int64_t tm = (CONV == 3 ? 4 : 1) * ((p.M + PBM - 1) / PBM);
   const int nk = (int)(p.K / 64);
-  const int unit = CONV ? 9 : 1;
+  const int unit = CONV == 3 ? 4 : CONV ? 9 : 1;
   const int cus_plan = cus_dev;
   constexpr int OVH = 12;
   int64_t best = -1, best1 = -1;
@@ -420,7 +448,7 @@
 
 template <int CONV, int EPI, int BKT>
 int launch_bk(hipStream_t stream, GemmParams& p, int64_t nblk) {
-  if constexpr (EPI == EPI_LINEAR) {
+  if constexpr (EPI == EPI_LINEAR && CONV != 3) {
     if (p.R != nullptr) return launch_res<CONV, EPI, BKT, true>(stream, p, nblk);
   }
   return launch_res<CONV, EPI, BKT, false>(stream, p, nblk);
@@ -449,7 +477,7 @@
     const int rc = try_launch_persist<CONV, EPI>(stream, p, flags);
     if (rc != NOT_ELIGIBLE) return rc;
   }
-  p.tiles_m = (p.M + BM - 1) / BM;
+  p.tiles_m = (CONV == 3 ? 4 : 1) * ((p.M + BM - 1) / BM);
   p.tiles_n = (p.N + BN - 1) / BN;
   const int64_t nblk = p.tiles_m * p.tiles_n;
   if (nblk <= 0 || nblk > 0x7fffffffLL) return A3D_EINVAL;
@@ -575,6 +603,24 @@
   return conv_entry(stream, X, Wp, bias, rowbias, rb_div, R, Y, B, H, W, Cin, Cout, stride, up2x, flags, ws, ws_bytes, ws_needed);
 }
 
+extern "C" int A3D_FN(a3d_conv3x3_up2x_folded)(a3d_stream_t stream, const void* X, const void* Wf, const float* bias, void* Y,
+                                            int B, int H, int W, int Cin, int Cout, int flags) {
+  if (!X || !Wf || !Y || B <= 0 || H <= 0 || W <= 0) return A3D_EINVAL;
+  if (Cin <= 0 || Cin % 64 != 0 || Cout <= 0 || Cout % 4 != 0) return A3D_EINVAL;
+  if (!a3d_aligned(16, X, Wf) || !a3d_aligned(16, bias) || !a3d_aligned(8, Y)) return A3D_EINVAL;
+  if (!gemm_flags_ok(flags)) return A3D_EINVAL;
+  GemmParams p{};
+  p.X = (const uint16_t*)X; p.ldx = Cin; p.W = (const uint16_t*)Wf; p.ldw = (int64_t)4 * Cin;
+  p.bias = bias; p.rb_div = 1; p.ldr = Cout; p.Y = (uint16_t*)Y; p.ldy = Cout;
+  p.B = B; p.H = H; p.Wd = W; p.Cin = Cin; p.stride = 1; p.up = 1; p.He = 2 * H; p.We = 2 * W;
+  p.Ho = H; p.Wo = W;
+  p.M = (int64_t)B * H * W; p.N = Cout; p.K = (int64_t)4 * Cin;
+  p.alpha = 1.f; p.beta = 1.f;
+  p.vec16 = (Cout % 8 == 0) && a3d_aligned(16, Y);
+  if (4 * p.M > 0x7fffffffLL) return A3D_EINVAL;
+  return launch<3>((hipStream_t)stream, p, flags);
+}
+
 extern "C" int A3D_FN(a3d_gemm_geglu)(a3d_stream_t stream, const void* X, int64_t ldx, const void* W, int64_t ldw,
                                    const float* bias, void* Y, int64_t ldy, int64_t M, int64_t N2, int64_t K, int flags) {
   GemmParams p = dense_params(X, ldx, W, ldw, bias, nullptr, 1, nullptr, 0, Y, ldy, M, N2, K, 1.f, 0.f);
diff --git a/animate3d_amd/csrc/gemm_pp.hip b/animate3d_amd/csrc/gemm_pp.hip
--- a/animate3d_amd/csrc/gemm_pp.hip
+++ b/animate3d_amd/csrc/gemm_pp.hip
@@ -27,6 +27,8 @@
 template <int CONV, int EPI, int NB, bool RES, bool SPLIT = false, bool TWO = false>
 __global__ __launch_bounds__(512, 1) void gemm_pp_kernel(const GemmParams p) {
   static_assert(!TWO || CONV == 0, "the two-source A operand is a dense-GEMM feature");
+  static_assert(CONV != 3 || (EPI == EPI_LINEAR && !RES && !SPLIT), "the folded up-sampling conv: bias only, no split-K");
+  constexpr int NTAP = CONV == 3 ? 4 : 9;
   using PC = PPCfg<NB>;
   constexpr int PH = 1, NPH = 4;
   constexpr int NP = 4 + NB;
@@ -85,6 +87,7 @@
     if constexpr (CONV == 0) xk = (uint64_t)(uintptr_t)(p.X + (ld_m0 + wid * 32) * p.ldx + kofs);
     if constexpr (TWO) xk2 = (uint64_t)(uintptr_t)(p.X2 + (ld_m0 + wid * 32) * p.ldx2);
     wk = (uint64_t)(uintptr_t)(p.W + (ld_n0 + wid * (NB * 8)) * p.ldw + kofs);
+    if constexpr (CONV == 3) wk += (uint64_t)(tile_m / (p.tiles_m >> 2)) * (uint64_t)p.N * (uint64_t)p.ldw * 2u;
     if (EPI == EPI_LINEAR && p.rowbias) rbk = (uint64_t)(uintptr_t)(p.rowbias + (ld_m0 / p.rb_div) * p.N + ld_n0);
     if constexpr (CONV != 0) {
       amask[0] = 0; amask[1] = 0;
@@ -98,7 +101,17 @@
         const int rem = (int)(m - (uint32_t)b * hw);
         const int oy = (int)((uint32_t)rem / (uint32_t)p.Wo), ox = rem - oy * p.Wo;
         uint32_t mask = 0;
-        if constexpr (CONV == 2) {
+        if constexpr (CONV == 3) {
+          const int ph = (int)((uint32_t)b / (uint32_t)p.B);
+          const int y0 = oy - 1 + (ph >> 1), x0 = ox - 1 + (ph & 1);
+          aoff[i] = (uint32_t)(((((int64_t)(b - ph * p.B) * p.H + y0) * p.Wd + x0) * p.Cin + cbias) * 2 + slot * 16);
+#pragma unroll
+          for (int tp = 0; tp < 4; ++tp) {
+            const int yy = y0 + (tp >> 1), xx = x0 + (tp & 1);
+            if (yy >= 0 && yy < p.H && xx >= 0 && xx < p.Wd) mask |= 1u << tp;
+          }
+          amask[i >> 1] |= mask << (NTAP * (i & 1));
+        } else if constexpr (CONV == 2) {
           const int sy0 = (oy - 1) >> 1, sx0 = (ox - 1) >> 1;
           aoff[i] = (uint32_t)(((((int64_t)b * p.H + sy0) * p.Wd + sx0) * p.Cin + cbias) * 2 + slot * 16);
 #pragma unroll
@@ -120,7 +133,7 @@
       }
       sok[0] = 0; sok[1] = 0;
 #pragma unroll
-      for (int bit = 0; bit < 18; ++bit) {
+      for (int bit = 0; bit < 2 * NTAP; ++bit) {
         if (__builtin_amdgcn_ballot_w64(((amask[0] >> bit) & 1u) != 0u) == ~0ull) sok[0] |= 1u << bit;
         if (__builtin_amdgcn_ballot_w64(((amask[1] >> bit) & 1u) != 0u) == ~0ull) sok[1] |= 1u << bit;
       }
@@ -154,7 +167,7 @@
         const uint32_t mk = amask[i >> 1];
         uint32_t vo = aoff[i];
         if constexpr (CONV == 2) vo += (((mk >> (18 + 2 * (i & 1))) & 1u) ? yE : yO) + (((mk >> (19 + 2 * (i & 1))) & 1u) ? xE : xO);
-        const int bit = itap + 9 * (i & 1);
+        const int bit = itap + NTAP * (i & 1);
         if ((sok[i >> 1] >> bit) & 1u) {
           glds16_s(vo, (const void*)(uintptr_t)xck, d);
         } else {
@@ -184,13 +197,22 @@
         const uint64_t cin2 = (uint64_t)(uint32_t)p.Cin * 2u;
         wk += cin2;
         ++itap;
-        if (++ikx == 3) { ikx = 0; ++iky; }
-        if (itap == 9) {
-          itap = 0; iky = 0; wk -= 9u * cin2 - 128u;
-          if constexpr (CONV == 1) xck -= (2u * (uint64_t)(uint32_t)p.Wd + 2u) * cin2;
-          xck += 128u;
-        } else if constexpr (CONV == 1) {
-          xck += ikx == 0 ? ((uint64_t)(uint32_t)p.Wd - 2u) * cin2 : cin2;
+        if constexpr (CONV == 3) {
+          if (itap == 4) {
+            itap = 0; wk -= 4u * cin2 - 128u;
+            xck -= ((uint64_t)(uint32_t)p.Wd + 1u) * cin2 - 128u;
+          } else {
+            xck += itap == 2 ? ((uint64_t)(uint32_t)p.Wd - 1u) * cin2 : cin2;
+          }
+        } else {
+          if (++ikx == 3) { ikx = 0; ++iky; }
+          if (itap == 9) {
+            itap = 0; iky = 0; wk -= 9u * cin2 - 128u;
+            if constexpr (CONV == 1) xck -= (2u * (uint64_t)(uint32_t)p.Wd + 2u) * cin2;
+            xck += 128u;
+          } else if constexpr (CONV == 1) {
+            xck += ikx == 0 ? ((uint64_t)(uint32_t)p.Wd - 2u) * cin2 : cin2;
+          }
         }
       } else {
         if (TWO && ik0 >= (int)p.K1) xk2 += 128; else xk += 128;
@@ -291,8 +313,19 @@
       float* const stg = reinterpret_cast<float*>(smem_b + (buf ^ 1) * PC::STAGE) + wid * (32 * 68);
       const float* const bias_lds = bias_image(smem_b + PC::BIAS_OFF, cur_par);
       const uint16_t* const rowbias_lds = rowbias_image(smem_b + PC::BIAS_OFF, cur_par);
-      if constexpr (EPI == EPI_GEGLU || !RES) epilogue_rounded<EPI, NB>(p, acc, stg, bias_lds, rowbias_lds, m0, n0, wm, wc, lane);
-      else epilogue_residual<NB>(p, acc, stg, bias_lds, rowbias_lds, m0, n0, wm, wc, lane);
+      if constexpr (CONV == 3) {
+        const uint32_t hw = (uint32_t)(p.H * p.Wd);
+        const uint32_t bi = (uint32_t)m0 / hw, ph = bi / (uint32_t)p.B;
+        Up2xRowMap rm;
+        rm.m0 = m0; rm.rem0 = (uint32_t)m0 - bi * hw; rm.hw = hw; rm.w = (uint32_t)p.Wd;
+        rm.row0 = ((int64_t)(bi - ph * (uint32_t)p.B) * (2 * p.H) + (ph >> 1)) * (2 * p.Wd) + (ph & 1);
+        rm.rcp_hw = 1.f / (float)hw; rm.rcp_w = 1.f / (float)p.Wd;
+        epilogue_rounded<EPI, NB>(p, acc, stg, bias_lds, rowbias_lds, m0, n0, wm, wc, lane, rm);
+      } else if constexpr (EPI == EPI_GEGLU || !RES) {
+        epilogue_rounded<EPI, NB>(p, acc, stg, bias_lds, rowbias_lds, m0, n0, wm, wc, lane);
+      } else {
+        epilogue_residual<NB>(p, acc, stg, bias_lds, rowbias_lds, m0, n0, wm, wc, lane);
+      }
     }
     if (tnext >= ntiles) break;
     t = tnext;
@@ -396,5 +429,11 @@
 int A3D_FN(a3d_launch_gemm_pp)(int conv, int epi, int nb, hipStream_t stream, const GemmParams& p, int cus) {
   if (conv == 0) return launch_pp_conv<0>(epi, nb, stream, p, cus);
   if (conv == 1) return launch_pp_conv<1>(epi, nb, stream, p, cus);
+  if (conv == 3) {
+    if (epi != EPI_LINEAR || p.R || p.rowbias || p.ksplit > 1) return A3D_EUNSUPPORTED;
+    if (nb == 5) return launch_pp<3, EPI_LINEAR, 5, false>(stream, p, cus);
+    if (nb == 4) return launch_pp<3, EPI_LINEAR, 4, false>(stream, p, cus);
+    return A3D_EUNSUPPORTED;
+  }
   return launch_pp_conv<2>(epi, nb, stream, p, cus);
 }
diff --git a/animate3d_amd/hip_ops.py b/animate3d_amd/hip_ops.py
--- a/animate3d_amd/hip_ops.py
+++ b/animate3d_amd/hip_ops.py
@@ -52,6 +52,7 @@
     "a3d_conv3x3_bf16": (c_int, [c_vp, c_vp, c_vp, c_vp, c_vp, c_i64, c_vp, c_vp, c_int, c_int, c_int, c_int, c_int, c_int, c_int, c_int]),
     "a3d_conv3x3_ws_bf16": (c_int, [c_vp, c_vp, c_vp, c_vp, c_vp, c_i64, c_vp, c_vp, c_int, c_int, c_int, c_int, c_int, c_int, c_int, c_int,
                                     c_vp, c_i64, ctypes.POINTER(c_i64)]),
+    "a3d_conv3x3_up2x_folded_bf16": (c_int, [c_vp, c_vp, c_vp, c_vp, c_vp, c_int, c_int, c_int, c_int, c_int, c_int]),
     "a3d_flash_attn_bf16": (c_int, [c_vp, c_vp, c_vp, c_vp, c_vp, ctypes.POINTER(_RowMapC), ctypes.POINTER(_RowMapC), ctypes.POINTER(_RowMapC),
                                     c_int, c_int, c_int, c_i64, c_i64, c_f32, c_f32, c_int]),
     "a3d_flash_attn_counted_bf16": (c_int, [c_vp, c_vp, c_vp, c_vp, c_vp, ctypes.POINTER(_RowMapC), ctypes.POINTER(_RowMapC), ctypes.POINTER(_RowMapC),
@@ -329,12 +330,44 @@
         _check(rc, f"a3d_gemm_geglu_bf16 M={M} N2={N2} K={K}")
         return y
 
+    supports_folded_up2x = True
+
+    @staticmethod
+    def fold_up2x(w: torch.Tensor) -> torch.Tensor:
+        Cout, K9 = w.shape
+        Cin = K9 // 9
+        assert K9 == 9 * Cin
+        acc = torch.float32 if w.dtype in (torch.bfloat16, torch.float16) else w.dtype
+        w9 = w.reshape(Cout, 3, 3, Cin).to(acc)
+        taps = (((0,), (1, 2)), ((0, 1), (2,)))
+        wf = torch.zeros(4, Cout, 2, 2, Cin, dtype=acc, device=w.device)
+        for a in range(2):
+            for b in range(2):
+                for r in range(2):
+                    for s in range(2):
+                        for ky in taps[a][r]:
+                            for kx in taps[b][s]:
+                                wf[2 * a + b, :, r, s] += w9[:, ky, kx]
+        return wf.reshape(4, Cout, 4 * Cin).to(w.dtype).contiguous()
+
+    @staticmethod
+    def folded_up2x_applies(H: int, W: int, up2x: bool, up_size, folded) -> bool:
+        return bool(up2x) and folded is not None and (up_size is None or tuple(int(v) for v in up_size) == (2 * H, 2 * W))
+
     def conv3x3(self, x, B: int, H: int, W: int, w, bias, *, stride: int = 1, up2x: bool = False, rowbias=None, rb_div: int = 1, residual=None,
-                up_size=None, tile128: bool = False):
+                up_size=None, tile128: bool = False, folded=None):
         x, w = self._act(x, "conv.x"), self._act(w, "conv.w")
         Cin = x.shape[1]
         Cout = w.shape[0]
         assert x.is_contiguous() and w.is_contiguous() and x.shape[0] == B * H * W and w.shape[1] == 9 * Cin
+        if self.folded_up2x_applies(H, W, up2x, up_size, folded):
+            if stride != 1 or rowbias is not None or residual is not None:
+                raise ValueError("the folded up-sampling conv is stride 1 and takes a bias only")
+            assert folded.dtype == self.act_dtype and folded.is_cuda and folded.is_contiguous() and tuple(folded.shape) == (4, Cout, 4 * Cin)
+            y = self.empty(B * 4 * H * W, Cout)
+            rc = self.lib.a3d_conv3x3_up2x_folded_bf16(self._stream(), _p(x), _p(folded), _p(bias), _p(y), B, H, W, Cin, Cout, self._gemm_flags(tile128))
+            _check(rc, f"a3d_conv3x3_up2x_folded_bf16 B={B} H={H} W={W} Cin={Cin} Cout={Cout}")
+            return y, 2 * H, 2 * W
         He, We = (2 * H, 2 * W) if up2x else (H, W)
         up_code = 1 if up2x else 0
         if up_size is not None:
diff --git a/animate3d_amd/unet.py b/animate3d_amd/unet.py
--- a/animate3d_amd/unet.py
+++ b/animate3d_amd/unet.py
@@ -476,13 +476,19 @@
         out.ff = self._pack_ff(tb)
         return out
 
+    def _fold_up(self, w9: torch.Tensor) -> Optional[torch.Tensor]:
+        ops = self._base_ops()
+        return ops.fold_up2x(w9) if getattr(ops, "supports_folded_up2x", False) else None
+
     def _pack_block(self, blk: M.MotionBlock):
+        up = None if blk.upsamplers is None else (self._conv_w(blk.upsamplers[0].conv), self._f(blk.upsamplers[0].conv.bias))
         return SimpleNamespace(
+            upf=None if up is None else self._fold_up(up[0]),
             resnets=[self._pack_resnet(r) for r in blk.resnets],
             t2d=[self._pack_t2d(t) for t in blk.attentions] if blk.has_cross_attention else None,
             motion=[self._pack_motion(m) for m in blk.motion_modules],
             down=None if blk.downsamplers is None else (self._conv_w(blk.downsamplers[0].conv), self._f(blk.downsamplers[0].conv.bias)),
-            up=None if blk.upsamplers is None else (self._conv_w(blk.upsamplers[0].conv), self._f(blk.upsamplers[0].conv.bias)))
+            up=up)
 
     def _pack(self):
         cfg = self.config
@@ -1123,7 +1129,9 @@
                 x = layer((x, skip) if pair else ops.concat(x, skip), rp, pk.t2d[j] if pk.t2d is not None else None, pk.motion[j], h_, w_)
             if pk.up is not None:
                 lvl -= 1
-                x, h_, w_ = ops.conv3x3(x, B2, h_, w_, pk.up[0], pk.up[1], up2x=True, up_size=sizes[lvl])
+                fold = getattr(pk, "upf", None) if self._active_ops is None and getattr(ops, "supports_folded_up2x", False) else None
+                kw = {} if fold is None else {"folded": fold}
+                x, h_, w_ = ops.conv3x3(x, B2, h_, w_, pk.up[0], pk.up[1], up2x=True, up_size=sizes[lvl], **kw)
         x = ops.group_norm(x, B2, h_ * w_, P.norm_out[0], P.norm_out[1], cfg.norm_num_groups, cfg.norm_eps, True)
         x, _, _ = ops.conv3x3(x, B2, h_, w_, P.conv_out[0], P.conv_out[1])
         out_dtype = sample.dtype if sample.dtype in (torch.float32, torch.bfloat16, torch.float16) else torch.float32
diff --git a/animate3d_amd/vae.py b/animate3d_amd/vae.py
--- a/animate3d_amd/vae.py
+++ b/animate3d_amd/vae.py
@@ -244,6 +244,9 @@
             v=(self._w(a.to_v.weight), self._f(a.to_v.bias)), o=(self._w(a.to_out[0].weight), self._f(a.to_out[0].bias)))
         P.up = [SimpleNamespace(res=[self._pack_resnet(r) for r in b.resnets],
                                 up=None if b.upsamplers is None else self._conv_w(b.upsamplers[0].conv)) for b in d.up_blocks]
+        folds = getattr(self.ops, "supports_folded_up2x", False)
+        for blk in P.up:
+            blk.upf = self.ops.fold_up2x(blk.up[0]) if folds and blk.up is not None else None
         P.norm_out = (self._f(d.conv_norm_out.weight), self._f(d.conv_norm_out.bias))
         P.conv_out = self._conv_w(d.conv_out, pad_out_to=4)
         self._packed = P
@@ -264,7 +267,8 @@
             for r in blk.res:
                 x = self._resnet(x, B, H, W, r)
             if blk.up is not None:
-                x, H, W = ops.conv3x3(x, B, H, W, blk.up[0], blk.up[1], up2x=True)
+                kw = {"folded": blk.upf} if blk.upf is not None and getattr(ops, "supports_folded_up2x", False) else {}
+                x, H, W = ops.conv3x3(x, B, H, W, blk.up[0], blk.up[1], up2x=True, **kw)
         x = ops.group_norm(x, B, H * W, P.norm_out[0], P.norm_out[1], cfg.norm_num_groups, 1e-6, True)
         x, _, _ = ops.conv3x3(x, B, H, W, P.conv_out[0], P.conv_out[1])
         img = ops.unpack_out(x, B, 4, 1, H, W, torch.float32)
diff --git a/include/animate3d_hip.h b/include/animate3d_hip.h
--- a/include/animate3d_hip.h
+++ b/include/animate3d_hip.h
@@ -55,6 +55,9 @@
                         const void* rowbias, int64_t rb_div, const void* R, void* Y,
                         int B, int H, int W, int Cin, int Cout, int stride, int up2x, int flags,
                         void* ws, int64_t ws_bytes, int64_t* ws_needed);
+
+int a3d_conv3x3_up2x_folded_bf16(a3d_stream_t stream, const void* X, const void* Wf, const float* bias, void* Y,
+                                 int B, int H, int W, int Cin, int Cout, int flags);
 
 #define A3D_ATTN_ACCUMULATE 1
 #define A3D_ATTN_CAUSAL 2
@@ -280,6 +283,8 @@
                        const void* rowbias, int64_t rb_div, const void* R, void* Y,
                        int B, int H, int W, int Cin, int Cout, int stride, int up2x, int flags,
                        void* ws, int64_t ws_bytes, int64_t* ws_needed);
+int a3d_conv3x3_up2x_folded_f16(a3d_stream_t stream, const void* X, const void* Wf, const float* bias, void* Y,
+                                int B, int H, int W, int Cin, int Cout, int flags);
 int a3d_flash_attn_f16(a3d_stream_t stream, const void* Q, const void* K, const void* V, void* O,
                         const a3d_rowmap* qmap, const a3d_rowmap* kmap, const a3d_rowmap* omap,
                         int groups, int heads, int head_dim, int64_t q_len, int64_t kv_len,
```

Result: no change. 2.449 denoise-steps/s, median of 6 (+0.8%).
